# AjayAlluri/realtime-fraud-detection

Measured on AMD Instinct MI355X. Metric: scored transactions/sec (whole node), higher is better.
Workload: dtype f32 (features f64, forests f32/f64, blend f64)

## Files before the change

include/fdengine.h:

```cpp
#ifndef FDENGINE_H
#define FDENGINE_H

#include <stddef.h>
#include <stdint.h>

#ifdef __cplusplus
extern "C" {
#endif

#define FD_ABI_VERSION 15

enum fd_status {
  FD_OK = 0,
  FD_ERR_INVALID_ARG = 1,
  FD_ERR_HIP = 2,
  FD_ERR_NOT_LOADED = 3,
  FD_ERR_UNSUPPORTED = 4,
  FD_ERR_OOM = 5,
  FD_ERR_IO = 6,
};

enum fd_forest_kind {
  FD_FOREST_XGB_BINARY_LOGISTIC = 1,
  FD_FOREST_SKLEARN_IFOREST = 2,
  FD_FOREST_SKLEARN_PROBA = 3,
};

typedef struct fd_engine fd_engine;

typedef struct {
  int32_t n_trees;
  const int64_t* tree_offsets;
  const int32_t* left;
  const int32_t* right;
  const int32_t* feature;
  const double* threshold;
  const uint8_t* default_left;
  const double* leaf_value;
} fd_tree_arrays;

typedef struct {
  int32_t kind;
  int32_t num_feature;
  double base_score;
  double if_offset;
  double if_denominator;
} fd_forest_params;

#define FD_MAX_MODELS 8
enum fd_blend_strategy { FD_BLEND_WEIGHTED_AVERAGE = 0, FD_BLEND_VOTING = 1, FD_BLEND_STACKING = 2 };
enum fd_decision { FD_APPROVE = 0, FD_REVIEW = 1, FD_DECLINE = 2, FD_APPROVE_WITH_MONITORING = 3 };
enum fd_risk { FD_VERY_LOW = 0, FD_LOW = 1, FD_MEDIUM = 2, FD_HIGH = 3, FD_CRITICAL = 4 };
typedef struct {
  int32_t n_models;
  int32_t strategy;
  double weight[FD_MAX_MODELS];
  double conf_mult[FD_MAX_MODELS];
  double fraud_threshold;
  double confidence_threshold;
} fd_blend_params;

const char* fd_last_error(void);
int fd_abi_version(void);
const char* fd_build_id(void);
int fd_device_count(int* out);
int fd_engine_create(int device, fd_engine** out);
int fd_engine_destroy(fd_engine* eng);
int fd_engine_set_stream(fd_engine* eng, void* hip_stream);
int fd_engine_reset_stream(fd_engine* eng);
int fd_engine_sync(fd_engine* eng);

int fd_load_forest(fd_engine* eng, int slot, const fd_forest_params* params, const fd_tree_arrays* trees);
int fd_unload_forest(fd_engine* eng, int slot);

int fd_load_xgboost_json(fd_engine* eng, int slot, const char* path);

int fd_xgboost_json_read(const char* path, fd_forest_params* params, int32_t* n_trees, int64_t* n_nodes,
                         fd_tree_arrays* trees);
int fd_forest_info(fd_engine* eng, int slot, int32_t* n_trees, int32_t* depth, int32_t* num_feature);

int fd_forest_predict_device(fd_engine* eng, int slot, const float* d_X, int64_t n, int32_t ld,
                             double* d_prob, double* d_raw, int32_t* d_leaf);
int fd_forest_predict_host(fd_engine* eng, int slot, const float* X, int64_t n, int32_t ld,
                           double* prob, double* raw, int32_t* leaf);

typedef struct {
  int32_t n_trees;
  int32_t n_chunks;
  int32_t chunk;
  int32_t depth;
  int64_t tree_bytes;
  int64_t chunk_stride;
  int64_t blob_bytes;
  int64_t n_leaf_ids;
  float base_margin;
  int32_t layout;
  int64_t n_thresholds;
  int32_t bin_steps;
} fd_pack_info;
int fd_pack_forest_host(const fd_forest_params* params, const fd_tree_arrays* trees, void* blob,
                        int64_t blob_cap, int32_t* leaf_ids, int64_t ids_cap, fd_pack_info* info);
int fd_pack_forest_binned_host(const fd_forest_params* params, const fd_tree_arrays* trees, void* blob,
                               int64_t blob_cap, float* thresholds, int64_t thr_cap, int32_t* offsets,
                               fd_pack_info* info);

int fd_contract_forest_host(const fd_forest_params* params, const fd_tree_arrays* trees, int64_t* n_nodes,
                            fd_tree_arrays* out, int32_t* depths, int64_t* n_pruned);

typedef struct {
  int32_t kind;
  int32_t n_trees;
  int32_t depth;
  int32_t leaf_bytes;
  int64_t n_nodes;
  int64_t n_leaves;
  float base_margin;
  int32_t pad;
} fd_sparse_info;
int fd_pack_forest_sparse_host(const fd_forest_params* params, const fd_tree_arrays* trees, void* nodes,
                               int64_t nodes_cap, void* leaf_values, int64_t values_cap, int32_t* leaf_ids,
                               int64_t ids_cap, fd_sparse_info* info);

int fd_blend_device(fd_engine* eng, const fd_blend_params* params, int64_t n,
                    const double* const* d_probs, const uint8_t* present,
                    double* d_fraud_prob, double* d_confidence, uint8_t* d_decision, uint8_t* d_risk);
int fd_blend_host(fd_engine* eng, const fd_blend_params* params, int64_t n,
                  const double* const* probs, const uint8_t* present,
                  double* fraud_prob, double* confidence, uint8_t* decision, uint8_t* risk);

enum fd_window_mode {
  FD_WINDOW_REDIS_COMPAT = 0,
  FD_WINDOW_SLIDING = 1
};
#define FD_RAW_FEATURES 16
#define FD_VECTOR_WIDTH 64
#define FD_MAX_SEQ_LEN 16
typedef struct {
  int64_t capacity;
  int32_t window_mode;
  int32_t ring_k;
  int32_t seq_len;
} fd_state_params;
int fd_state_init(fd_engine* eng, const fd_state_params* params);
int fd_state_clear(fd_engine* eng);
int fd_state_info(fd_engine* eng, int64_t* capacity, int64_t* cards);
typedef struct {
  int64_t n;
  const uint64_t* key;
  const double* avg_amount;
  const int32_t* account_age_days;
  const uint64_t* device_fp;
} fd_users;
int fd_state_load_users_host(fd_engine* eng, const fd_users* users);
typedef struct {
  int64_t n;
  const double* fraud_rate;
  const double* risk_multiplier;
} fd_merchants;
int fd_load_merchants_host(fd_engine* eng, const fd_merchants* merchants);
typedef struct {
  const uint64_t* card_key;
  const int64_t* ts_ms;
  const int64_t* amount_cents;
  const int32_t* merchant;
  const uint64_t* device_fp;
  const uint8_t* ip_class;
  const uint8_t* hour;
  const uint8_t* weekend;
} fd_txn_batch;
int fd_features_device(fd_engine* eng, const fd_txn_batch* txns, int64_t n, float* d_vectors, double* d_raw);
int fd_features_host(fd_engine* eng, const fd_txn_batch* txns, int64_t n, float* vectors, double* raw);

#define FD_FEATURE_MAP_WIDTH 64
#define FD_CODE_UNKNOWN 254
typedef struct {
  const double* geo_lat;
  const double* geo_lon;
  const double* merchant_lat;
  const double* merchant_lon;
  const uint8_t* payment_method;
  const uint8_t* transaction_type;
  const uint8_t* card_type;
  const uint8_t* user_agent_flag;
  const double* fraud_score;
} fd_txn_context;
typedef struct {
  double tp_score;
  double fe_score;
  uint8_t tp_decision;
  uint8_t tp_risk;
  uint8_t fe_decision;
  uint8_t fe_risk;
  uint8_t pad[4];
} fd_rule_scores;
typedef struct {
  int64_t n;
  const uint64_t* key;
  const double* risk_score;
  const uint8_t* kyc_status;
  const uint8_t* verified;
  const int8_t* pref_start;
  const int8_t* pref_end;
  const double* weekend_activity;
  const double* online_preference;
  const double* intl_preference;
  const int32_t* txn_frequency;
  const uint8_t* has_patterns;
} fd_users_ext;
typedef struct {
  int64_t n;
  const double* avg_amount;
  const uint8_t* risk_level;
  const uint8_t* blacklisted;
  const uint8_t* category;
  const uint8_t* high_risk_category;
  const uint8_t* open_hour;
  const uint8_t* close_hour;
  const uint8_t* suspicious_name;
} fd_merchants_ext;
int fd_state_load_users_ext_host(fd_engine* eng, const fd_users_ext* users);
int fd_load_merchants_ext_host(fd_engine* eng, const fd_merchants_ext* merchants);
int fd_load_vocab_host(fd_engine* eng, const uint8_t* payment_high_risk, const uint8_t* type_is_refund);
int fd_features_full_device(fd_engine* eng, const fd_txn_batch* txns, const fd_txn_context* ctx, int64_t n,
                            float* d_vectors, double* d_raw, double* d_fmap, fd_rule_scores* d_rules);

typedef struct {
  int32_t input_size;
  int32_t hidden;
  int32_t n_out;
  const float* w_ih;
  const float* w_hh;
  const float* b_ih;
  const float* b_hh;
  const float* w_out;
  const float* b_out;
} fd_lstm_params;
int fd_load_lstm(fd_engine* eng, const fd_lstm_params* params);
int fd_unload_lstm(fd_engine* eng);
int fd_lstm_predict_device(fd_engine* eng, const float* d_seq, int64_t n, int32_t T, double* d_prob);
int fd_lstm_predict_host(fd_engine* eng, const float* seq, int64_t n, int32_t T, double* prob);
#define FD_SLOT_LSTM 64
int fd_features_seq_device(fd_engine* eng, const fd_txn_batch* txns, int64_t n, float* d_vectors, double* d_raw,
                           float* d_seq);

typedef struct {
  int32_t n_layers;
  int32_t dims[9];
  const float* weight[8];
  const float* bias[8];
} fd_mlp_params;
int fd_load_mlp(fd_engine* eng, const fd_mlp_params* params);
int fd_unload_mlp(fd_engine* eng);
int fd_mlp_info(fd_engine* eng, int32_t* n_layers, int32_t* in_dim, int32_t* hidden);
int fd_mlp_predict_device(fd_engine* eng, const float* d_X, int64_t n, int32_t ld, double* d_prob);
int fd_mlp_predict_host(fd_engine* eng, const float* X, int64_t n, int32_t ld, double* prob);
int fd_pack_mlp_host(const fd_mlp_params* params, void* blob, int64_t cap, int64_t* bytes);
#define FD_SLOT_MLP 65

#define FD_GRAPH_FEATURES 5
typedef struct {
// ... 249 lines not shown
```

realtime-fraud-detection_amd/csrc/engine.hip:

```cpp
#include <algorithm>
#include <chrono>
#include <mutex>
#include <cstring>
#include <string>

#include "blend_row.h"
#include "abtest_row.h"
#include "fd_internal.h"
#include "graph_row.h"
#include "host_stage.h"
#include "ingest_parse.h"
#include "text_row.h"

namespace fd {

static thread_local std::string g_last_error;

void set_error(const std::string& msg) { g_last_error = msg; }

Engine::Timed* Engine::next_event_pair(int kind) {
  if (timing_every > 1 && kind >= 0 && kind < 16 && (timing_seq[kind]++ % (unsigned)timing_every) != 0)
    return nullptr;
  if (events_used == events.size()) {
    hipEvent_t a, b;
// ... 367 lines not shown
    for (auto* b : {&f.split.bins, &f.split.nan, &f.split.leaves}) b->release();
    f.blob.release();
    f.leaf_ids.release();
    f.b_blob.release();
    f.b_thr.release();
    f.b_thr_off.release();
  }
  e.stage.release();
  e.scratch_probs.release();
  e.feat_vec.release();
  fd::windows_release(e);
  fd::sink_release(e);
  fd::graph_release(e);
  fd::text_release(e);
  fd::ab_release(e);
  for (auto* b : {&e.route_blk, &e.route_blk_stream, &e.route_out, &e.route_err, &e.seq_buf, &e.seq_desc, &e.lstm.wpk, &e.lstm.wpk4, &e.lstm.bias,
                  &e.lstm.wout, &e.lstm.bout, &e.state.seq, &e.mlp.blob})
    b->release();
  if (e.aux_stream) {
    (void)hipStreamSynchronize(e.aux_stream);
    (void)hipStreamDestroy(e.aux_stream);
    (void)hipEventDestroy(e.fork_ev);
    (void)hipEventDestroy(e.join_ev);
  }
  if (e.aux2_stream) {
    (void)hipStreamSynchronize(e.aux2_stream);
    (void)hipStreamDestroy(e.aux2_stream);
    (void)hipEventDestroy(e.join2_ev);
  }
  try {
    fd::comm_destroy(e);
  } catch (...) {
  }
  for (hipStream_t st : e.pipe_stream)
    if (st) {
      (void)hipStreamSynchronize(st);
      (void)hipStreamDestroy(st);
    }
  if (e.pipe_slot_stream) {
    (void)hipStreamSynchronize(e.pipe_slot_stream);
    (void)hipStreamDestroy(e.pipe_slot_stream);
  }
  if (e.pipe_entry_ev) (void)hipEventDestroy(e.pipe_entry_ev);
  for (int k = 0; k < Engine::kPipeSlots; ++k) {
    if (e.pipe_slot_ev[k]) (void)hipEventDestroy(e.pipe_slot_ev[k]);
    if (e.pipe_feat_ev[k]) (void)hipEventDestroy(e.pipe_feat_ev[k]);
    if (e.pipe_copy_ev[k]) (void)hipEventDestroy(e.pipe_copy_ev[k]);
    e.pipe_vec[k].release();
    e.pipe_out[k].release();
    e.pipe_seq[k].release();
  }
  for (int k = 0; k < Engine::kSplitRing; ++k) {
    if (e.pipe_done_ev[k]) (void)hipEventDestroy(e.pipe_done_ev[k]);
    e.pipe_split[k].release();
  }
  for (auto* b : {&e.state.uext, &e.state.mext, &e.state.vocab, &e.feat_ext}) b->release();
  for (auto& P1 : e.ens1)
    for (auto* b : {&P1.nodes[0], &P1.nodes[1], &P1.thr}) b->release();
  for (auto* b : {&e.ens.nodes[0], &e.ens.nodes[1], &e.ens.thr})
    b->release();
  {
    fd::IngestTables& t = e.ingest;
    for (auto* b : {&t.mkeys, &t.mvals}) b->release();
    for (int w = 0; w < 3; ++w) {
      t.vkeys[w].release();
      t.vvals[w].release();
    }
  }
  for (auto* b : {&e.state.pages, &e.state.keys, &e.state.merchants, &e.state.err, &e.state.sat,
                  &e.state.bucket_scr})
    b->release();
  for (auto& g : e.state.gs)
    for (auto* b : {&g.slot, &g.bucket_fill, &g.pairs, &g.ovf_cnt, &g.ovf_key, &g.ovf_b, &g.prep}) b->release();
  for (auto& ev : e.events) {
    (void)hipEventDestroy(ev.a);
    (void)hipEventDestroy(ev.b);
    if (ev.c) (void)hipEventDestroy(ev.c);
    if (ev.d) (void)hipEventDestroy(ev.d);
  }
  if (e.own_stream) (void)hipStreamDestroy(e.own_stream);
  delete eng;
  FD_API_END
}

static void rebind_stream(Engine& e, hipStream_t s) {
  for (int k = 0; k < Engine::kDoneRing; ++k)
    if (e.pipe_done_live[k] && s != e.stream) FD_HIP(hipStreamWaitEvent(s, e.pipe_done_ev[k], 0));
  e.stream = s;
}

int fd_engine_set_stream(fd_engine* eng, void* hip_stream) {
  FD_API_BEGIN
  FD_ENGINE_LOCK(eng);
  Engine& e = E(eng);
  rebind_stream(e, static_cast<hipStream_t>(hip_stream));
  FD_API_END
}

int fd_engine_reset_stream(fd_engine* eng) {
  FD_API_BEGIN
  FD_ENGINE_LOCK(eng);
  Engine& e = E(eng);
  rebind_stream(e, e.own_stream);
  FD_API_END
}

int fd_engine_sync(fd_engine* eng) {
  FD_API_BEGIN
  FD_ENGINE_LOCK(eng);
  Engine& e = E(eng);
  if (e.comm.aborted) {
    bool ok = fd::comm_sync_stream(e, e.comm.x_fwd);
    ok = fd::comm_sync_stream(e, e.stream) && ok;
    for (hipStream_t st : e.pipe_stream) ok = fd::comm_sync_stream(e, st) && ok;
    for (hipStream_t st : {e.pipe_slot_stream, e.aux_stream, e.aux2_stream}) ok = fd::comm_sync_stream(e, st) && ok;
    FD_REQUIRE(ok, FD_ERR_HIP, "streams still busy " + std::to_string(e.comm.timeout_ms) +
                                   " ms after the communicators were aborted (" + e.comm.abort_reason + ")");
  }
  FD_HIP(hipStreamSynchronize(e.stream));
  if (e.comm.x_fwd) FD_HIP(hipStreamSynchronize(e.comm.x_fwd));
  for (hipStream_t st : e.pipe_stream)
    if (st) FD_HIP(hipStreamSynchronize(st));
  if (e.pipe_slot_stream) FD_HIP(hipStreamSynchronize(e.pipe_slot_stream));
  if (e.aux_stream) FD_HIP(hipStreamSynchronize(e.aux_stream));
  if (e.aux2_stream) FD_HIP(hipStreamSynchronize(e.aux2_stream));
  fd::route_check(e);
  FD_API_END
}

int fd_engine_set_timing(fd_engine* eng, int enable) {
  FD_API_BEGIN
  FD_ENGINE_LOCK(eng);
  Engine& e = E_quiet(eng);
  e.timing = enable != 0;
  FD_API_END
}

int fd_engine_get_counter(fd_engine* eng, const char* key, int64_t* value) {
  FD_API_BEGIN
  FD_ENGINE_LOCK(eng);
  Engine& e = E_quiet(eng);
  FD_REQUIRE(key && value, FD_ERR_INVALID_ARG, "null key/value");
  const std::string k(key);
  if (k == "pipelined_batches") {
    *value = (int64_t)e.pipe_iter_total;
  } else if (k == "ensemble_single_launches") {
    *value = (int64_t)e.ens_single_total;
  } else if (k == "ensemble_contracted_launches") {
    *value = (int64_t)e.ens_contract_total;
  } else if (k == "ensemble_nodes_pruned") {
    *value = e.ens.valid ? (int64_t)e.ens.nodes_pruned : 0;
  } else if (k == "ensemble_node_steps_per_txn") {
    *value = (int64_t)e.ens_steps_last;
  } else if (k == "forest_sparse_launches") {
    *value = (int64_t)e.sparse_total;
  } else if (k == "mlp_launches") {
    *value = (int64_t)e.mlp_total;
  } else if (k == "graph_steps") {
    *value = (int64_t)e.graph.steps;
  } else if (k == "text_calls") {
    *value = (int64_t)e.text.calls;
  } else if (k == "text_nonascii_rows") {
    *value = fd::text_nonascii_rows(e);
  } else if (k == "latency_prebinned_batches") {
    *value = (int64_t)e.prebin_total;
  } else if (k == "pipelined_split_batches") {
    *value = (int64_t)e.pipe_split_total;
  } else if (k == "pipelined_compact_batches") {
    *value = (int64_t)e.pipe_compact_total;
  } else if (k == "pipelined_host_ns") {
    *value = (int64_t)e.pipe_host_ns;
  } else if (k == "pipelined_slot_stream_batches") {
    *value = (int64_t)e.pipe_slot_stream_total;
  } else if (k == "window_saturated") {
    FD_REQUIRE(e.state.ready, FD_ERR_NOT_LOADED, "card state not initialised (fd_state_init)");
    FD_HIP(hipStreamSynchronize(e.stream));
    for (hipStream_t st : e.pipe_stream)
      if (st) FD_HIP(hipStreamSynchronize(st));
    unsigned long long v = 0;
    FD_HIP(hipMemcpy(&v, e.state.sat.ptr, 8, hipMemcpyDeviceToHost));
    *value = (int64_t)v;
  } else if (k == "sharded_steps") {
    *value = (int64_t)e.comm.steps.load();
  } else if (k == "rccl_ops") {
    *value = (int64_t)e.comm.ops.load();
  } else if (k.rfind("sharded_host_ns_", 0) == 0) {
    int i = 0;
    while (i < fd::ShardComm::kHostPhases && k.compare(16, std::string::npos, fd::kShardHostPhase[i]) != 0) ++i;
    FD_REQUIRE(i < fd::ShardComm::kHostPhases, FD_ERR_INVALID_ARG, "unknown counter: " + k);
    *value = (int64_t)e.comm.host_ns[i].load();
  } else {
    FD_REQUIRE(false, FD_ERR_INVALID_ARG, "unknown counter: " + k);
  }
  FD_API_END
}

int fd_engine_set_option(fd_engine* eng, const char* key, int64_t value) {
  FD_API_BEGIN
  FD_ENGINE_LOCK(eng);
  Engine& e = E_quiet(eng);
  FD_REQUIRE(key, FD_ERR_INVALID_ARG, "null key");
  const std::string k(key);
  if (k == "forest_kernel") {
    FD_REQUIRE(value == 0 || value == 1 || value == 2 || value == 3 || value == 6 || value == 8 || value == 11,
               FD_ERR_INVALID_ARG, "forest_kernel must be 0, 1, 2, 3, 6, 8 or 11");
    e.forest_variant = (int)value;
  } else if (k == "ensemble") {
    FD_REQUIRE(value == 0 || value == 1, FD_ERR_INVALID_ARG, "ensemble must be 0 or 1");
    e.ensemble_on = value != 0;
  } else if (k == "ensemble_owner") {
    FD_REQUIRE(value == 0 || value == 1, FD_ERR_INVALID_ARG, "ensemble_owner must be 0 or 1");
    e.ens_owner_fixed = value != 0;
  } else if (k == "ensemble_prio") {
    FD_REQUIRE(value == 0 || value == 1, FD_ERR_INVALID_ARG, "ensemble_prio must be 0 or 1");
    e.ens_prio = value != 0;
  } else if (k == "ensemble_chunks") {
    FD_REQUIRE(value >= 0 && value <= 2, FD_ERR_INVALID_ARG, "ensemble_chunks must be 0, 1 or 2");
    e.ens_chunks = (int)value;
  } else if (k == "ensemble_contract") {
    FD_REQUIRE(value >= 0 && value <= 2, FD_ERR_INVALID_ARG, "ensemble_contract must be 0, 1 or 2");
    if ((int)value != e.ens_contract) {
      e.activate();
      FD_HIP(hipDeviceSynchronize());
    }
    e.ens_contract = (int)value;
  } else if (k == "compact_vectors") {
    FD_REQUIRE(value >= 0 && value <= 2, FD_ERR_INVALID_ARG, "compact_vectors must be 0, 1 or 2");
    e.compact_vectors = (int)value;
  } else if (k == "latency_fused") {
    FD_REQUIRE(value == 0 || value == 1, FD_ERR_INVALID_ARG, "latency_fused must be 0 or 1");
    e.latency_fused = value != 0;
  } else if (k == "pipeline_lean") {
    FD_REQUIRE(value == 0 || value == 1, FD_ERR_INVALID_ARG, "pipeline_lean must be 0 or 1");
    e.pipe_lean = value != 0;
  } else if (k == "pipeline_gather") {
    FD_REQUIRE(value == 0 || value == 1, FD_ERR_INVALID_ARG, "pipeline_gather must be 0 or 1");
    e.pipe_gather = value != 0;
  } else if (k == "latency_prebin") {
    FD_REQUIRE(value >= 0 && value <= 3, FD_ERR_INVALID_ARG, "latency_prebin must be 0, 1, 2 or 3");
    e.latency_prebin = value != 0;
    if (value) e.latency_prebin_mode = (int)value;
  } else if (k == "small_streams") {
    FD_REQUIRE(value >= 0 && value <= 2, FD_ERR_INVALID_ARG, "small_streams must be 0, 1 or 2");
    e.small_streams = (int)value;
  } else if (k == "count_exchange") {
    FD_REQUIRE(value >= -1 && value <= 1, FD_ERR_INVALID_ARG, "count_exchange must be -1, 0 or 1");
    FD_REQUIRE(!e.comm.pending, FD_ERR_INVALID_ARG, "count_exchange: a prefetched batch's counts are in flight");
    e.comm.count_mode = (int)value;
    e.comm.count_gather = value == 1 || (value < 0 && e.comm.world >= 4);
  } else if (k == "comm_timeout_ms") {
    FD_REQUIRE(value >= 1, FD_ERR_INVALID_ARG, "comm_timeout_ms must be >= 1");
    e.comm.timeout_ms = value;
  } else if (k == "stream_priority") {
    FD_REQUIRE(value >= 0 && value <= 3, FD_ERR_INVALID_ARG, "stream_priority must be in 0..3");
    FD_REQUIRE(!e.pipe_stream[0] && !e.comm.x_fwd, FD_ERR_INVALID_ARG,
               "stream_priority: set before the first pipelined call and fd_comm_init");
    e.stream_prio = (int)value;
  } else if (k == "bucket_keys") {
    FD_REQUIRE(value == 0 || (value >= 8 && value <= 512 && (value & (value - 1)) == 0), FD_ERR_INVALID_ARG,
               "bucket_keys must be 0 or a power of two in 8..512");
    e.state.bucket_keys = (int)value;
  } else if (k == "ensemble_bin_global") {
    FD_REQUIRE(value == 0 || value == 1, FD_ERR_INVALID_ARG, "ensemble_bin_global must be 0 or 1");
    e.ens_bin_global = value != 0;
  } else if (k == "lean_group") {
    FD_REQUIRE(value >= 0 && value <= 2, FD_ERR_INVALID_ARG, "lean_group must be 0, 1 or 2");
    e.state.lean_group = (int)value;
  } else if (k == "slot_gather") {
    FD_REQUIRE(value == 0 || value == 1, FD_ERR_INVALID_ARG, "slot_gather must be 0 or 1");
    e.state.slot_gather = value != 0;
  } else if (k == "slot_stream") {
    FD_REQUIRE(value >= -1 && value <= 2, FD_ERR_INVALID_ARG, "slot_stream must be -1, 0, 1 or 2");
    FD_REQUIRE(!e.pipe_slot_stream || (int)value == e.pipe_slot_mode, FD_ERR_INVALID_ARG,
               "slot_stream: set before the first pipelined call");
    e.pipe_slot_mode = (int)value;
  } else if (k == "slot_prio") {
    FD_REQUIRE(value == 0 || value == 1, FD_ERR_INVALID_ARG, "slot_prio must be 0 or 1");
    e.state.slot_prio = value != 0;
  } else if (k == "feature_prio") {
    FD_REQUIRE(value == 0 || value == 1, FD_ERR_INVALID_ARG, "feature_prio must be 0 or 1");
    e.state.feat_prio = value != 0;
  } else if (k == "bucket_spread") {
    FD_REQUIRE(value == 0 || value == 1, FD_ERR_INVALID_ARG, "bucket_spread must be 0 or 1");
    e.state.bucket_spread = value != 0;
  } else if (k == "timing_every") {
    FD_REQUIRE(value >= 1 && value <= 1000000, FD_ERR_INVALID_ARG, "timing_every must be >= 1");
    e.timing_every = (int)value;
    for (auto& q : e.timing_seq) q = 0;
  } else if (k == "seq_ring_lstm") {
    FD_REQUIRE(value == 0 || value == 1, FD_ERR_INVALID_ARG, "seq_ring_lstm must be 0 or 1");
    e.seq_ring_lstm = value != 0;
  } else if (k == "lstm_rows") {
    FD_REQUIRE(value == 0 || value == 4 || value == 16, FD_ERR_INVALID_ARG, "lstm_rows must be 0, 4 or 16");
    e.lstm_rows = (int)value;
  } else if (k == "mlp_form") {
    FD_REQUIRE(value == 0 || value == 1, FD_ERR_INVALID_ARG, "mlp_form must be 0 or 1");
    e.mlp_form = (int)value;
  } else if (k == "mlp_wgs_per_cu") {
    FD_REQUIRE(value >= 0 && value <= 8, FD_ERR_INVALID_ARG, "mlp_wgs_per_cu must be in 0..8");
    e.mlp_wgs_per_cu = (int)value;
  } else if (k == "ingest_stop_after") {
    FD_REQUIRE(value >= 0 && value <= 3, FD_ERR_INVALID_ARG, "ingest_stop_after must be in 0..3");
    e.ingest.stop_after = (int)value;
  } else if (k == "rule_fraud_threshold_permille") {
    FD_REQUIRE(value >= 0 && value <= 1000, FD_ERR_INVALID_ARG, "rule_fraud_threshold_permille must be in 0..1000");
    e.state.tp_threshold = (double)value / 1000.0;
  } else {
    throw fd::Error(FD_ERR_INVALID_ARG, "unknown option: " + k);
  }
  FD_API_END
}

int fd_timing_read(fd_engine* eng, int kind, double* total_ms, int64_t* launches) {
  FD_API_BEGIN
  FD_ENGINE_LOCK(eng);
  Engine& e = E_quiet(eng);
  double tot = 0.0;
  int64_t cnt = 0;
  for (size_t i = 0; i < e.events_used; ++i) {
    if (kind >= 0 && e.events[i].kind != kind) continue;
    FD_HIP(hipEventSynchronize(e.events[i].b));
    float ms = 0.f;
    FD_HIP(hipEventElapsedTime(&ms, e.events[i].a, e.events[i].b));
    tot += ms;
    if (e.events[i].split) {
      FD_HIP(hipEventSynchronize(e.events[i].d));
      FD_HIP(hipEventElapsedTime(&ms, e.events[i].c, e.events[i].d));
      tot += ms;
    }
    ++cnt;
  }
  if (total_ms) *total_ms = tot;
  if (launches) *launches = cnt;
  FD_API_END
}

int fd_timing_reset(fd_engine* eng) {
  FD_API_BEGIN
  FD_ENGINE_LOCK(eng);
  Engine& e = E_quiet(eng);
  for (size_t i = 0; i < e.events_used; ++i) {
    FD_HIP(hipEventSynchronize(e.events[i].b));
    if (e.events[i].split) FD_HIP(hipEventSynchronize(e.events[i].d));
  }
  e.events_used = 0;
  FD_API_END
}

int fd_load_forest(fd_engine* eng, int slot, const fd_forest_params* params, const fd_tree_arrays* trees) {
  FD_API_BEGIN
  FD_ENGINE_LOCK(eng);
  Engine& e = E(eng);
  FD_REQUIRE(params && trees, FD_ERR_INVALID_ARG, "null params/trees");
  fd::PackedForest& pf = slot_of(e, slot);
  FD_HIP(hipStreamSynchronize(e.stream));
  pf.loaded = false;
  fd::repack_forest(pf, *params, *trees);
  FD_API_END
}

int fd_pack_forest_host(const fd_forest_params* params, const fd_tree_arrays* trees, void* blob,
                        int64_t blob_cap, int32_t* leaf_ids, int64_t ids_cap, fd_pack_info* info) {
  FD_API_BEGIN
  FD_REQUIRE(params && trees && info, FD_ERR_INVALID_ARG, "null params/trees/info");
  const fd::HostPack hp = fd::pack_forest_host(*params, *trees);
  info->n_trees = hp.n_trees;
  info->n_chunks = hp.n_chunks;
  info->chunk = hp.chunk;
  info->depth = hp.depth;
  info->tree_bytes = (int64_t)hp.tree_bytes;
  info->chunk_stride = (int64_t)hp.chunk_stride;
  info->blob_bytes = (int64_t)hp.blob.size();
  info->n_leaf_ids = (int64_t)hp.leaf_ids.size();
  info->base_margin = hp.base_margin;
  info->layout = 0;
  info->n_thresholds = (int64_t)hp.b_thr.size();
  info->bin_steps = hp.bin_steps;
  if (blob) {
    FD_REQUIRE(blob_cap >= (int64_t)hp.blob.size(), FD_ERR_INVALID_ARG, "blob buffer too small");
    std::memcpy(blob, hp.blob.data(), hp.blob.size());
  }
  if (leaf_ids) {
    FD_REQUIRE(ids_cap >= (int64_t)hp.leaf_ids.size(), FD_ERR_INVALID_ARG, "leaf id buffer too small");
    std::memcpy(leaf_ids, hp.leaf_ids.data(), hp.leaf_ids.size() * sizeof(int32_t));
  }
  FD_API_END
}

int fd_contract_forest_host(const fd_forest_params* params, const fd_tree_arrays* trees, int64_t* n_nodes,
                            fd_tree_arrays* out, int32_t* depths, int64_t* n_pruned) {
  FD_API_BEGIN
  FD_REQUIRE(params && trees, FD_ERR_INVALID_ARG, "null params/trees");
  const fd::ContractedForest c = fd::contract_forest_host(*params, *trees);
  const int32_t T = (int32_t)c.off.size() - 1;
  const int64_t M = (int64_t)c.left.size();
  if (n_nodes) *n_nodes = M;
  if (n_pruned) *n_pruned = (int64_t)c.pruned;
  if (depths) std::memcpy(depths, c.depth.data(), (size_t)T * 4);
  if (out) {
    FD_REQUIRE(out->tree_offsets && out->left && out->right && out->feature && out->threshold && out->default_left &&
                   out->leaf_value,
               FD_ERR_INVALID_ARG, "incomplete output arrays");
    out->n_trees = T;
    std::memcpy(const_cast<int64_t*>(out->tree_offsets), c.off.data(), (size_t)(T + 1) * 8);
    std::memcpy(const_cast<int32_t*>(out->left), c.left.data(), (size_t)M * 4);
    std::memcpy(const_cast<int32_t*>(out->right), c.right.data(), (size_t)M * 4);
    std::memcpy(const_cast<int32_t*>(out->feature), c.feature.data(), (size_t)M * 4);
    std::memcpy(const_cast<double*>(out->threshold), c.threshold.data(), (size_t)M * 8);
    std::memcpy(const_cast<uint8_t*>(out->default_left), c.dleft.data(), (size_t)M);
    std::memcpy(const_cast<double*>(out->leaf_value), c.leaf.data(), (size_t)M * 8);
  }
  FD_API_END
}

int fd_pack_forest_binned_host(const fd_forest_params* params, const fd_tree_arrays* trees, void* blob,
                               int64_t blob_cap, float* thresholds, int64_t thr_cap, int32_t* offsets,
                               fd_pack_info* info) {
  FD_API_BEGIN
  FD_REQUIRE(params && trees && info, FD_ERR_INVALID_ARG, "null params/trees/info");
  const fd::HostPack hp = fd::pack_forest_host(*params, *trees);
  FD_REQUIRE(hp.binned, FD_ERR_UNSUPPORTED,
             "forest has no binned layout (depth > 8 or > 65534 distinct thresholds in a feature)");
  info->n_trees = hp.n_trees;
  info->n_chunks = hp.b_n_chunks;
  info->chunk = hp.b_chunk;
  info->depth = hp.depth;
  info->tree_bytes = (int64_t)hp.b_tree_bytes;
  info->chunk_stride = (int64_t)hp.b_chunk_stride;
  info->blob_bytes = (int64_t)hp.b_blob.size();
  info->n_leaf_ids = (int64_t)hp.leaf_ids.size();
  info->base_margin = hp.base_margin;
  info->layout = 1;
  info->n_thresholds = (int64_t)hp.b_thr.size();
  info->bin_steps = hp.bin_steps;
  if (blob) {
    FD_REQUIRE(blob_cap >= (int64_t)hp.b_blob.size(), FD_ERR_INVALID_ARG, "blob buffer too small");
    std::memcpy(blob, hp.b_blob.data(), hp.b_blob.size());
  }
  if (thresholds) {
    FD_REQUIRE(thr_cap >= (int64_t)hp.b_thr.size(), FD_ERR_INVALID_ARG, "threshold buffer too small");
    std::memcpy(thresholds, hp.b_thr.data(), hp.b_thr.size() * sizeof(float));
  }
  if (offsets) std::memcpy(offsets, hp.b_thr_off.data(), hp.b_thr_off.size() * sizeof(int32_t));
  FD_API_END
}

int fd_pack_forest_sparse_host(const fd_forest_params* params, const fd_tree_arrays* trees, void* nodes,
                               int64_t nodes_cap, void* leaf_values, int64_t values_cap, int32_t* leaf_ids,
                               int64_t ids_cap, fd_sparse_info* info) {
  FD_API_BEGIN
  FD_REQUIRE(params && trees && info, FD_ERR_INVALID_ARG, "null params/trees/info");
  const fd::SparsePack sp = fd::pack_forest_sparse_host(*params, *trees);
  *info = fd_sparse_info{};
  info->kind = sp.kind;
  info->n_trees = sp.n_trees;
  info->depth = sp.depth;
  info->leaf_bytes = sp.leaf_bytes;
  info->n_nodes = sp.n_nodes;
  info->n_leaves = sp.n_leaves;
  info->base_margin = sp.base_margin;
  if (nodes) {
    FD_REQUIRE(nodes_cap >= sp.n_nodes, FD_ERR_INVALID_ARG, "node buffer too small");
    std::memcpy(nodes, sp.nodes.data(), sp.nodes.size() * sizeof(uint32_t));
  }
  if (leaf_values) {
    FD_REQUIRE(values_cap >= sp.n_leaves, FD_ERR_INVALID_ARG, "leaf value buffer too small");
    std::memcpy(leaf_values, sp.leaf_val.data(), sp.leaf_val.size());
  }
  if (leaf_ids) {
    FD_REQUIRE(ids_cap >= sp.n_leaves, FD_ERR_INVALID_ARG, "leaf id buffer too small");
    std::memcpy(leaf_ids, sp.leaf_ids.data(), sp.leaf_ids.size() * sizeof(int32_t));
  }
  FD_API_END
}

int fd_load_xgboost_json(fd_engine* eng, int slot, const char* path) {
  FD_API_BEGIN
  FD_ENGINE_LOCK(eng);
  Engine& e = E(eng);
  fd::PackedForest& pf = slot_of(e, slot);
  fd::XgbModel m;
  fd::read_xgboost_json(path, m);
  fd_forest_params p{};
  p.kind = FD_FOREST_XGB_BINARY_LOGISTIC;
  p.num_feature = m.num_feature;
  p.base_score = m.base_score;
  fd_tree_arrays t{};
  t.n_trees = (int32_t)(m.offsets.size() - 1);
  t.tree_offsets = m.offsets.data();
  t.left = m.left.data();
  t.right = m.right.data();
  t.feature = m.feature.data();
  t.threshold = m.threshold.data();
  t.default_left = m.default_left.data();
  t.leaf_value = m.leaf_value.data();
  FD_REQUIRE(t.n_trees > 0, FD_ERR_INVALID_ARG, "xgboost json: no trees");
  FD_HIP(hipStreamSynchronize(e.stream));
  pf.loaded = false;
  fd::repack_forest(pf, p, t);
  FD_API_END
}

int fd_xgboost_json_read(const char* path, fd_forest_params* params, int32_t* n_trees, int64_t* n_nodes,
                         fd_tree_arrays* trees) {
  FD_API_BEGIN
  fd::XgbModel m;
  fd::read_xgboost_json(path, m);
  const int32_t T = (int32_t)(m.offsets.size() - 1);
  const int64_t M = (int64_t)m.left.size();
  if (params) {
    *params = fd_forest_params{};
    params->kind = FD_FOREST_XGB_BINARY_LOGISTIC;
    params->num_feature = m.num_feature;
    params->base_score = m.base_score;
  }
  if (n_trees) *n_trees = T;
  if (n_nodes) *n_nodes = M;
  if (trees) {
    FD_REQUIRE(trees->tree_offsets && trees->left && trees->right && trees->feature && trees->threshold &&
                   trees->default_left && trees->leaf_value,
               FD_ERR_INVALID_ARG, "incomplete output arrays");
    trees->n_trees = T;
    std::memcpy(const_cast<int64_t*>(trees->tree_offsets), m.offsets.data(), (size_t)(T + 1) * 8);
    std::memcpy(const_cast<int32_t*>(trees->left), m.left.data(), (size_t)M * 4);
    std::memcpy(const_cast<int32_t*>(trees->right), m.right.data(), (size_t)M * 4);
    std::memcpy(const_cast<int32_t*>(trees->feature), m.feature.data(), (size_t)M * 4);
    std::memcpy(const_cast<double*>(trees->threshold), m.threshold.data(), (size_t)M * 8);
    std::memcpy(const_cast<uint8_t*>(trees->default_left), m.default_left.data(), (size_t)M);
    std::memcpy(const_cast<double*>(trees->leaf_value), m.leaf_value.data(), (size_t)M * 8);
  }
  FD_API_END
}

int fd_unload_forest(fd_engine* eng, int slot) {
  FD_API_BEGIN
  FD_ENGINE_LOCK(eng);
  Engine& e = E(eng);
  fd::PackedForest& pf = slot_of(e, slot);
  FD_HIP(hipStreamSynchronize(e.stream));
  pf.blob.release();
  pf.leaf_ids.release();
  pf.b_blob.release();
  pf.b_thr.release();
  pf.b_thr_off.release();
  for (auto* b : {&pf.split.bins, &pf.split.nan, &pf.split.leaves}) b->release();
  for (auto* b : {&pf.sp.nodes, &pf.sp.leaf_val, &pf.sp.leaf_ids}) b->release();
  pf.sp.gen = 0;
  pf.sparse_only = false;
  pf.binned = false;
  pf.loaded = false;
  pf.gen = 0;
  FD_API_END
}

int fd_forest_info(fd_engine* eng, int slot, int32_t* n_trees, int32_t* depth, int32_t* num_feature) {
  FD_API_BEGIN
  FD_ENGINE_LOCK(eng);
  Engine& e = E(eng);
  fd::PackedForest& pf = slot_of(e, slot);
  FD_REQUIRE(pf.loaded, FD_ERR_NOT_LOADED, "Model in slot " + std::to_string(slot) + " not loaded");
  if (n_trees) *n_trees = pf.n_trees;
  if (depth) *depth = pf.depth;
  if (num_feature) *num_feature = pf.num_feature;
  FD_API_END
}

int fd_forest_predict_device(fd_engine* eng, int slot, const float* d_X, int64_t n, int32_t ld,
// ... 1375 lines not shown
```

realtime-fraud-detection_amd/csrc/ensemble.hip:

```cpp
#include <algorithm>
#include <atomic>
#include <cstring>

#include "blend_row.h"
#include "walk_common.h"

namespace fd {

static std::atomic<uint64_t> g_forest_gen{0};

void forest_loaded(PackedForest& pf, const fd_forest_params& p, const fd_tree_arrays& t) {
  pf.gen = ++g_forest_gen;
  pf.params = p;
  const int64_t m = t.tree_offsets[t.n_trees];
  pf.t_off.assign(t.tree_offsets, t.tree_offsets + t.n_trees + 1);
  pf.t_left.assign(t.left, t.left + m);
  pf.t_right.assign(t.right, t.right + m);
  pf.t_feature.assign(t.feature, t.feature + m);
  pf.t_threshold.assign(t.threshold, t.threshold + m);
  pf.t_leaf.assign(t.leaf_value, t.leaf_value + m);
  if (t.default_left)
    pf.t_dleft.assign(t.default_left, t.default_left + m);
  else
    pf.t_dleft.assign((size_t)m, 0);
}

ContractedForest contract_forest_host(const fd_forest_params& p, const fd_tree_arrays& t) {
  FD_REQUIRE(p.kind == FD_FOREST_XGB_BINARY_LOGISTIC || p.kind == FD_FOREST_SKLEARN_IFOREST, FD_ERR_INVALID_ARG,
             "contraction: XGBoost binary:logistic or IsolationForest trees");
  FD_REQUIRE(p.num_feature > 0 && p.num_feature <= kMaxFeatures, FD_ERR_UNSUPPORTED, "num_feature must be in [1, 64]");
  FD_REQUIRE(forest_depth_probe(t) >= 0, FD_ERR_INVALID_ARG, "incomplete tree arrays or a tree that is not a tree");
  const bool xgb = p.kind == FD_FOREST_XGB_BINARY_LOGISTIC;
  ContractedForest c;
  c.off.push_back(0);
  struct Item {
    int32_t o, lo, ro;
    int depth;
  };
  std::vector<Item> st, keep;
  std::vector<int32_t> remap;
  for (int i = 0; i < t.n_trees; ++i) {
    const int64_t a = t.tree_offsets[i], m = t.tree_offsets[i + 1] - a;
    const int32_t *L = t.left + a, *R = t.right + a, *F = t.feature + a;
    auto resolve = [&](int32_t o) {
      while (L[o] >= 0) {
        FD_REQUIRE(F[o] >= 0 && F[o] < p.num_feature, FD_ERR_INVALID_ARG, "split feature outside [0, num_feature)");
        const int src = compact_src(F[o]);
        if (src >= 0) break;
        const float val = src == -2 ? 0.5f : 0.0f;
        const float thr = xgb ? (float)t.threshold[a + o] : sklearn_threshold_to_lt(t.threshold[a + o]);
        o = val < thr ? L[o] : R[o];
      }
      return o;
    };
    const int64_t base = (int64_t)c.left.size();
    auto emit = [&](int32_t l, int32_t r, int32_t f, double thr, uint8_t dl, double leaf) {
      c.left.push_back(l);
      c.right.push_back(r);
      c.feature.push_back(f);
      c.threshold.push_back(thr);
      c.dleft.push_back(dl);
      c.leaf.push_back(leaf);
      return (int32_t)((int64_t)c.left.size() - 1 - base);
    };
    int64_t splits_in = 0, splits_out = 0;
    for (int64_t o = 0; o < m; ++o) splits_in += L[o] >= 0 ? 1 : 0;
    int depth = 0;
    const int32_t root = resolve(0);
    if (L[root] < 0 && L[0] >= 0) {
      emit(1, 2, 0, 0.0, 0, 0.0);
      emit(-1, -1, 0, 0.0, 0, t.leaf_value[a + root]);
      emit(-1, -1, 0, 0.0, 0, t.leaf_value[a + root]);
      depth = 1;
    } else {
      st.clear();
      st.push_back({root, 0, 0});
      keep.clear();
      while (!st.empty()) {
        Item it = st.back();
        st.pop_back();
        depth = std::max(depth, it.depth);
        if (L[it.o] >= 0) {
          it.lo = resolve(L[it.o]);
          it.ro = resolve(R[it.o]);
          st.push_back({it.ro, 0, 0, it.depth + 1});
          st.push_back({it.lo, 0, 0, it.depth + 1});
        }
        keep.push_back(it);
      }
      std::sort(keep.begin() + 1, keep.end(), [](const Item& x, const Item& y) { return x.o < y.o; });
      remap.assign((size_t)m, -1);
      for (size_t k = 0; k < keep.size(); ++k) remap[(size_t)keep[k].o] = (int32_t)k;
      for (const Item& it : keep) {
        const int32_t o = it.o;
        if (L[o] < 0) {
          emit(-1, -1, F[o], t.threshold[a + o], t.default_left ? t.default_left[a + o] : 0, t.leaf_value[a + o]);
        } else {
          ++splits_out;
          emit(remap[(size_t)it.lo], remap[(size_t)it.ro], F[o], t.threshold[a + o],
               t.default_left ? t.default_left[a + o] : 0, t.leaf_value[a + o]);
        }
      }
    }
    c.pruned += splits_in - splits_out;
    c.depth.push_back(std::max(depth, 1));
    c.off.push_back((int64_t)c.left.size());
  }
  return c;
}

namespace {

constexpr int kEnsWG = 1024;
constexpr int kMaxPass = 64;

template <bool WIDE>
struct EnsCfg {
  static constexpr int CHA = WIDE ? 24 : 20;
  static constexpr int CHB = WIDE ? 16 : 12;
  static constexpr uint32_t BUF = (uint32_t)(CHA * (1024 + 256 * 4) > CHB * (1024 + 256 * 8) ? CHA * (1024 + 256 * 4)
                                                                                             : CHB * (1024 + 256 * 8));
};
inline uint32_t ens_buf(bool wide) { return wide ? EnsCfg<true>::BUF : EnsCfg<false>::BUF; }
constexpr uint32_t kEnsTile = 4u * kTile * 8u;

__host__ __device__ constexpr uint32_t ens_xs_bytes(int nf) { return (uint32_t)((nf + 1) / 2) * 1024u; }

size_t ens_lds(int nf, bool wide) {
  return (size_t)ens_xs_bytes(nf) + 2 * (size_t)ens_buf(wide) + 2 * (size_t)kEnsTile + kTile * 4 + kTile * 8 + 128 +
         1024;
}

struct EnsArgs {
  const float* X;
  int64_t n;
  int ld, nf;
  const float* thr;
  int vec4;
  int compact;
  int owner_fixed;
  int prio;
  int n_pass;
  int ldepth;
  unsigned long long pass_global;
  const char* img;
  const char* nodes[2];
  int n_chunks[2];
  int stride[2];
  float base_margin;
  int pad1;
  double if_offset, if_denom;
  int pos[2];
  int mcol[2];
  double* mp;
  double* fp;
  double* conf;
  uint8_t* dec;
  uint8_t* risk;
  const RouteRecord* rec;
  ResultRecord* res;
  int pass_f[kMaxPass + 1];
  int img_off[kMaxPass + 1];
  int thr_off[kMaxFeatures + 1];
  uint16_t cbin[kMaxFeatures];
  alignas(4) uint16_t lut[8 * 32];
  BlendConsts blend;
#ifdef FD_FOREST_PROFILE
  int prof_slot;
  int clk_slot;
#endif
};

constexpr uint32_t kLinkMask = 0x3F8u;

template <int D, int TPG, bool NAN_AWARE>
__device__ __forceinline__ void walk_ens(uint32_t buf, int t0, uint32_t lane4, uint32_t (&leaf)[TPG]) {
  uint32_t tb[TPG], node[TPG], kl[TPG], kr[TPG], xw[TPG];
#pragma unroll
  for (int j = 0; j < TPG; ++j) {
    tb[j] = buf + (uint32_t)(t0 + j) * 1024u;
    asm volatile("" : "+v"(tb[j]));
    node[j] = lds_load<uint32_t>(tb[j] + 4u);
  }
#pragma unroll
  for (int j = 0; j < TPG; ++j) {
    xw[j] = lds_load<uint16_t>((node[j] & 0xFC02u) | lane4);
    if (D > 1) {
      const u32x2 k = lds_load<u32x2>(tb[j] + 8u);
      kl[j] = k.x;
      kr[j] = k.y;
    }
  }
#pragma unroll
  for (int l = 0; l < D; ++l) {
#pragma unroll
    for (int j = 0; j < TPG; ++j) {
      bool right = xw[j] > (node[j] >> 16);
      if (NAN_AWARE) {
        if (xw[j] == 0xFFFFu) right = (node[j] & 1u) == 0u;
      }
      if (l + 1 < D) {
        uint32_t a = kl[j], b = kr[j];
        asm volatile("" : "+v"(a), "+v"(b));
        node[j] = right ? b : a;
        xw[j] = lds_load<uint16_t>((node[j] & 0xFC02u) | lane4);
        if (l + 2 < D) {
          const u32x2 k = lds_load<u32x2>((node[j] & kLinkMask) | tb[j]);
          kl[j] = k.x;
          kr[j] = k.y;
        }
      } else {
        leaf[j] = ((node[j] & kLinkMask) >> 2) + (right ? 1u : 0u);
      }
    }
  }
}

template <int D, int TPG>
__device__ __forceinline__ unsigned long long walk_pack(uint32_t cur, int gg, uint32_t lane4, bool tile_nan) {
  static_assert(TPG <= 8, "a byte per tree in a u64");
  uint32_t leaf[TPG];
  if (tile_nan)
    walk_ens<D, TPG, true>(cur, gg * TPG, lane4, leaf);
  else
    walk_ens<D, TPG, false>(cur, gg * TPG, lane4, leaf);
  uint32_t lo = 0, hi = 0;
#pragma unroll
  for (int j = 0; j < TPG; ++j) {
    if (j < 4) lo |= leaf[j] << (8 * j);
    else hi |= leaf[j] << (8 * (j - 4));
  }
  return ((unsigned long long)hi << 32) | lo;
}

template <int TPG, bool NAN_AWARE>
__device__ __forceinline__ void walk_ens_var(uint32_t buf, int t0, uint32_t lane4, const int (&d)[TPG],
                                             uint32_t (&leaf)[TPG]) {
  uint32_t tb[TPG], node[TPG], kl[TPG], kr[TPG], xw[TPG];
  int dw = 1;
#pragma unroll
  for (int j = 0; j < TPG; ++j) {
    tb[j] = buf + (uint32_t)(t0 + j) * 1024u;
    asm volatile("" : "+v"(tb[j]));
    node[j] = lds_load<uint32_t>(tb[j] + 4u);
    dw = max(dw, d[j]);
    leaf[j] = 0u;
  }
#pragma unroll
  for (int j = 0; j < TPG; ++j) {
    xw[j] = lds_load<uint16_t>((node[j] & 0xFC02u) | lane4);
    const u32x2 k = lds_load<u32x2>(tb[j] + 8u);
    kl[j] = k.x;
    kr[j] = k.y;
  }
#pragma unroll
  for (int l = 0; l < 8; ++l) {
    if (l >= dw) break;
#pragma unroll
    for (int j = 0; j < TPG; ++j) {
      bool right = xw[j] > (node[j] >> 16);
      if (NAN_AWARE) {
        if (xw[j] == 0xFFFFu) right = (node[j] & 1u) == 0u;
      }
      const uint32_t at = ((node[j] & kLinkMask) >> 2) + (right ? 1u : 0u);
      leaf[j] = (l + 1 == d[j]) ? at : leaf[j];
      node[j] = right ? kr[j] : kl[j];
    }
    if (l + 1 >= dw) break;
#pragma unroll
    for (int j = 0; j < TPG; ++j) {
      if (l + 1 < d[j]) {
        xw[j] = lds_load<uint16_t>((node[j] & 0xFC02u) | lane4);
        if (l + 2 < d[j]) {
          const u32x2 k = lds_load<u32x2>((node[j] & kLinkMask) | tb[j]);
          kl[j] = k.x;
          kr[j] = k.y;
        }
      }
    }
  }
}

template <int VD, int TPG>
__device__ __forceinline__ unsigned long long walk_pack_var(uint32_t cur, int gg, uint32_t lane4, bool tile_nan) {
  static_assert(TPG <= 8, "a byte per tree in a u64");
  uint32_t leaf[TPG];
  int d[TPG];
#pragma unroll
  for (int j = 0; j < TPG; ++j)
    d[j] = __builtin_amdgcn_readfirstlane((int)lds_load<uint32_t>(cur + (uint32_t)(gg * TPG + j) * 1024u)) & 0xFF;
  if (VD == 1) {
    if (tile_nan)
      walk_ens_var<TPG, true>(cur, gg * TPG, lane4, d, leaf);
    else
      walk_ens_var<TPG, false>(cur, gg * TPG, lane4, d, leaf);
  } else {
#define FD_WALK_DEPTH(K)                                          \
  case K:                                                         \
    if (tile_nan)                                                 \
      walk_ens<K, TPG, true>(cur, gg * TPG, lane4, leaf);         \
    else                                                          \
      walk_ens<K, TPG, false>(cur, gg * TPG, lane4, leaf);        \
    break;
    switch (d[0]) {
      FD_WALK_DEPTH(1)
      FD_WALK_DEPTH(2)
      FD_WALK_DEPTH(3)
      FD_WALK_DEPTH(4)
      FD_WALK_DEPTH(5)
      FD_WALK_DEPTH(6)
      FD_WALK_DEPTH(7)
      default:
        if (tile_nan)
          walk_ens<8, TPG, true>(cur, gg * TPG, lane4, leaf);
        else
          walk_ens<8, TPG, false>(cur, gg * TPG, lane4, leaf);
        break;
    }
#undef FD_WALK_DEPTH
  }
  uint32_t lo = 0, hi = 0;
#pragma unroll
  for (int j = 0; j < TPG; ++j) {
    if (j < 4) lo |= leaf[j] << (8 * j);
    else hi |= leaf[j] << (8 * (j - 4));
  }
  return ((unsigned long long)hi << 32) | lo;
}

template <int D, int TPG, int CH, typename LeafT>
__device__ __forceinline__ void owner_sum(uint32_t buf, uint32_t tile, uint32_t acc, int txn, const int NL = 1 << D) {
  unsigned long long w[4];
#pragma unroll
  for (int q = 0; q < 4; ++q) w[q] = lds_load<unsigned long long>(tile + (uint32_t)(q * kTile + txn) * 8u);
  LeafT v[CH];
#pragma unroll
  for (int t = 0; t < CH; ++t) {
    const uint32_t idx = (uint32_t)(w[t / TPG] >> (8 * (t % TPG))) & 0xFFu;
    v[t] = lds_load<LeafT>(buf + (uint32_t)(CH * 1024) + ((uint32_t)(t * NL) + idx) * (uint32_t)sizeof(LeafT));
  }
  LeafT s = lds_load<LeafT>(acc + (uint32_t)txn * (uint32_t)sizeof(LeafT));
#pragma unroll
  for (int t = 0; t < CH; ++t) s += v[t];
  lds_store<LeafT>(acc + (uint32_t)txn * (uint32_t)sizeof(LeafT), s);
}

__device__ __forceinline__ void stage_pieces(const char* __restrict__ src, uint32_t dst, int bytes, int nparts,
                                             int part) {
  const int lane = threadIdx.x & 63;
  const int pieces = bytes >> 10;
  for (int p = part; p < pieces; p += nparts) {
    const char* g = src + (p << 10) + lane * 16;
    const uint32_t m0 = __builtin_amdgcn_readfirstlane(dst + ((uint32_t)p << 10));
    asm volatile(
        "s_mov_b32 m0, %0\n\t"
        "s_nop 0\n\t"
        "global_load_lds_dwordx4 %1, off"
        :
        : "s"(m0), "v"(g)
        : "memory", "m0");
  }
}

__host__ __device__ __forceinline__ int thr_pad(int g) { return g + (g >> 5); }

#ifdef FD_FOREST_PROFILE
constexpr int kEprofSlots = 4;
__device__ unsigned long long g_eprof[kEprofSlots * 256 * 16 * 16];
static int g_eprof_next = 0;
constexpr int kEclkSlots = 1024;
__device__ unsigned long long g_eclk[kEclkSlots * 4 * 4];
static int g_eclk_next = 0;
#define FD_ESTAMP(var) const unsigned long long var = __builtin_amdgcn_s_memtime()
#else
#define FD_ESTAMP(var)
#endif

template <int L>
__device__ __forceinline__ void search_lockstep(const float (&vv)[L], const int (&o)[L], const int (&cnt)[L],
                                                int (&pos)[L], int steps, bool glob, uint32_t tl, int o0,
                                                const float* __restrict__ thr) {
  if (!glob) {
    for (int st = steps; st > 0; st >>= 1) {
      float t[L];
#pragma unroll
      for (int k = 0; k < L; ++k) {
        const int np = pos[k] + st;
        const int idx = np <= cnt[k] ? np - 1 : 0;
        t[k] = lds_load<float>(tl + (uint32_t)thr_pad(o[k] - o0 + idx) * 4u);
      }
#pragma unroll
      for (int k = 0; k < L; ++k) {
        const int np = pos[k] + st;
        pos[k] = (np <= cnt[k] && t[k] <= vv[k]) ? np : pos[k];
      }
    }
  } else {
    for (int st = steps; st > 0; st >>= 1) {
      float t[L];
#pragma unroll
      for (int k = 0; k < L; ++k) {
        const int np = pos[k] + st;
        t[k] = thr[o[k] + (np <= cnt[k] ? np - 1 : 0)];
      }
#pragma unroll
      for (int k = 0; k < L; ++k) {
        const int np = pos[k] + st;
        pos[k] = (np <= cnt[k] && t[k] <= vv[k]) ? np : pos[k];
      }
    }
  }
}

template <int Q>
__device__ __forceinline__ void bin_compact_constants(const EnsArgs& a, uint16_t* Xs, int txn) {
  uint32_t* X32 = reinterpret_cast<uint32_t*>(Xs);
#pragma unroll
  for (int j = Q; j < kMaxFeatures / 2; j += 4) {
    const int f = 2 * j;
    const bool c0 = compact_src(f) < 0 && f < a.nf, c1 = compact_src(f + 1) < 0 && f + 1 < a.nf;
    if (c0 && c1)
      X32[j * 256 + txn] = (uint32_t)a.cbin[f] | ((uint32_t)a.cbin[f + 1] << 16);
    else if (c0)
      Xs[j * 512 + txn * 2] = a.cbin[f];
    else if (c1)
      Xs[j * 512 + txn * 2 + 1] = a.cbin[f + 1];
  }
}

constexpr int kLutN = 32;
static_assert(kIntSlots * kLutN == 8 * 32, "EnsArgs::lut");
constexpr int kIntOf[4][6] = {{-1, 2, -1, 6, -1, -1}, {-1, 3, 5, -1, -1, -1}, {0, 4, -1, -1, -1, -1},
                              {1, -1, -1, 7, -1, -1}};
constexpr int kNSearched[4] = {4, 4, 3, 3};
constexpr int kSearched[4][4] = {{0, 2, 4, 5}, {0, 3, 4, 5}, {2, 3, 4, 0}, {1, 2, 4, 0}};
constexpr bool int_tables_agree() {
  for (int q = 0; q < 4; ++q) {
    int ns = 0;
    for (int i = 0; i < 6; ++i) {
      const int ci = q + 4 * i;
      const int want = ci < kCompactSlots ? int_slot(ci) : -1;
      if (kIntOf[q][i] != want) return false;
      if (ci < kCompactSlots && want < 0) {
        if (ns >= 4 || kSearched[q][ns] != i) return false;
        ++ns;
      }
    }
    if (ns != kNSearched[q]) return false;
  }
  return true;
}
static_assert(int_tables_agree(), "kIntOf / kSearched must follow kIntCompact and kCompactSlot");

template <int Q>
__device__ __forceinline__ void load_compact(const float* __restrict__ xr, float (&v)[16]) {
  const unsigned long long ib = *reinterpret_cast<const unsigned long long*>(xr + 14);
#pragma unroll
  for (int i = 0; i < 6; ++i) {
    const int ci = Q + 4 * i;
    if (ci >= kCompactSlots) {
      v[i] = 0.f;
    } else if (int_slot(ci) >= 0) {
      v[i] = (float)(unsigned)((ib >> (8 * int_slot(ci))) & 0xFFull);
    } else {
      v[i] = xr[compact_word(ci)];
    }
  }
}

template <int Q>
__device__ __forceinline__ void load_split(const uint4* __restrict__ ra, const uint4* __restrict__ rb,
                                           float (&v)[16]) {
  const uint4 a0 = ra[0], a1 = ra[1], b0 = rb[0], b1 = rb[1];
  const unsigned fa = a1.w >> 24;
  const int na = (fa & 1u) ? 1 : 0;
  const int nu = ((b1.z >> 8) & 1u) ? 1 : 0;
  const int nc = ((b1.y >> 8) & 0xFFu) ? 1 : 0;
  const int n2 = na + nu + nc;
  auto byte = [](unsigned w, int k) { return (float)((w >> (8 * k)) & 0xFFu); };
#pragma unroll
  for (int i = 0; i < 6; ++i) {
    const int ci = Q + 4 * i;
    float x = 0.f;
    switch (ci) {
      case 0: x = __uint_as_float(a0.x); break;
      case 1: x = __uint_as_float(a0.y); break;
      case 2: x = byte(a1.w, 0); break;
      case 3: x = byte(a1.w, 1); break;
      case 4: x = byte(a1.w, 2); break;
      case 5: x = byte(b1.y, 0); break;
      case 6: x = byte(b1.y, 1); break;
      case 7: x = __uint_as_float(b0.x); break;
      case 8: x = __uint_as_float(b0.y); break;
      case 9: x = byte(b1.y, 2); break;
      case 10: x = __uint_as_float(a0.w); break;
      case 11: x = __uint_as_float(a1.x); break;
      case 12: x = byte(b1.y, 3); break;
      case 13: x = __uint_as_float(a1.y); break;
      case 14: x = __uint_as_float(b0.z); break;
      case 15: x = byte(b1.z, 0); break;
      default:
        if (ci < kCompactSlots) {
          const int k = ci - 16;
          const float first = (na && k == 0) ? __uint_as_float(a0.z)
                                             : ((nu && k == na) ? __uint_as_float(b0.w) : __uint_as_float(b1.x));
          const int t = k - n2;
          x = k < n2 ? first
                     : (t == 0 ? __uint_as_float(a1.z)
                               : (t == 1 ? ((fa & 2u) ? 1.f : 0.f) : (t == 2 ? ((fa & 4u) ? 1.f : 0.f) : 0.f)));
        }
        break;
    }
    v[i] = x;
  }
}

template <int Q, int L, bool LUT>
__device__ __forceinline__ void bin_compact_pass(const EnsArgs& a, const float (&v)[16], uint16_t* Xs,
                                                 int txn, int f0, int f1, bool glob, uint32_t tl, int o0,
                                                 int& anynan, uint32_t lut) {
  constexpr int NV = (kCompactSlots - Q + 3) / 4;
  constexpr int NS = LUT ? kNSearched[Q] : NV;
#pragma unroll
  for (int i = 0; i < NV; ++i) {
    const int ks = LUT ? kIntOf[Q][i] : -1;
    if (ks < 0) continue;
    const int f = kCompactSlot[Q + 4 * i];
    if (!(f >= f0 && f < f1 && f < a.nf)) continue;
    const float x = v[i];
    uint16_t bin;
    if (x != x) {
      anynan = 1;
      bin = (uint16_t)0xFFFFu;
    } else if (x >= 0.f && x < (float)kLutN && x == truncf(x)) {
      bin = lds_load<uint16_t>(lut + (uint32_t)(ks * kLutN + (int)x) * 2u);
    } else {
      const int o = a.thr_off[f], cnt = a.thr_off[f + 1] - o;
      int pos = 0;
#pragma unroll
      for (int st = 1 << 15; st > 0; st >>= 1)
        if (pos + st <= cnt && a.thr[o + pos + st - 1] <= x) pos += st;
      bin = (uint16_t)pos;
    }
    Xs[(f >> 1) * 512 + txn * 2 + (f & 1)] = bin;
  }
#pragma unroll
  for (int g0 = 0; g0 < NS; g0 += L) {
    float vv[L];
    int o[L], cnt[L], pos[L];
    bool act[L];
    int steps = 0;
#pragma unroll
    for (int k = 0; k < L; ++k) {
      const int i = LUT ? kSearched[Q][g0 + k < NS ? g0 + k : 0] : (g0 + k < NS ? g0 + k : 0);
      const int f = kCompactSlot[Q + 4 * i];
      act[k] = g0 + k < NS && f >= f0 && f < f1 && f < a.nf;
      vv[k] = act[k] ? v[i] : 0.f;
      o[k] = act[k] ? a.thr_off[f] : o0;
      cnt[k] = act[k] ? a.thr_off[f + 1] - o[k] : 0;
      pos[k] = 0;
      steps = max(steps, lift_steps(cnt[k]));
    }
    search_lockstep<L>(vv, o, cnt, pos, steps, glob, tl, o0, a.thr);
#pragma unroll
    for (int k = 0; k < L; ++k) {
      const int i = LUT ? kSearched[Q][g0 + k < NS ? g0 + k : 0] : (g0 + k < NS ? g0 + k : 0);
      const int f = kCompactSlot[Q + 4 * i];
      if (act[k]) {
        const bool nan = vv[k] != vv[k];
        anynan |= nan ? 1 : 0;
        Xs[(f >> 1) * 512 + txn * 2 + (f & 1)] = nan ? (uint16_t)0xFFFFu : (uint16_t)pos[k];
      }
    }
  }
}

template <int D, int OUT, bool WIDE, bool LUT = true, int VD = 0>
__global__ void __launch_bounds__(kEnsWG) ensemble_kernel(EnsArgs a) {
  constexpr int kCHA = EnsCfg<WIDE>::CHA, kCHB = EnsCfg<WIDE>::CHB;
  constexpr uint32_t kEnsBuf = EnsCfg<WIDE>::BUF;
  constexpr int TPGA = kCHA / 4, TPGB = kCHB / 4;
  extern __shared__ __attribute__((aligned(16))) char smem[];
  const uint32_t sdyn = (uint32_t)(size_t)((lds_char*)smem);
  const uint32_t s0 = (sdyn + 1023u) & ~1023u;
  char* const lbase = smem + (s0 - sdyn);
  const int tid = threadIdx.x, wave = tid >> 6, lane = tid & 63;
  const int gg = __builtin_amdgcn_readfirstlane(wave >> 2);
  const int txn = ((wave & 3) << 6) + lane;
  const uint32_t lane4 = s0 + (uint32_t)txn * 4u;
  const uint32_t bufA = s0 + ens_xs_bytes(a.nf), bufB = bufA + kEnsBuf;
  const uint32_t tile0 = bufB + kEnsBuf, tile1 = tile0 + kEnsTile;
  const uint32_t accA = tile1 + kEnsTile, accB = accA + kTile * 4;
  const uint32_t flags = accB + kTile * 8, owner_cnt = flags + 64;
  const int64_t row = (int64_t)blockIdx.x * kTile + txn;
  const bool valid = row < a.n;
  const int nA = a.n_chunks[0], G = nA + a.n_chunks[1];
  const int NL = VD ? 1 << a.ldepth : 1 << D;

#ifdef FD_FOREST_PROFILE
  unsigned long long pr_top = 0, pr_walk = 0, pr_sync = 0, pr_dma = 0, pr_st[8] = {0, 0, 0, 0, 0, 0, 0, 0};
#endif
  FD_ESTAMP(pr_t0);
#ifdef FD_FOREST_PROFILE
  const unsigned long long pr_rt0 = __builtin_amdgcn_s_memrealtime();
#endif
  {
    const int k_prio = a.prio, k_compact = a.compact, k_npass = a.n_pass, k_vec4 = a.vec4, k_ld = a.ld;
    const unsigned long long k_pg = a.pass_global;
    const float* k_x = a.X;
    const char* k_img = a.img;
    const int k_i0 = a.img_off[0], k_i1 = a.img_off[1], k_f1 = a.pass_f[1];
    asm volatile("" ::"s"(k_prio), "s"(k_compact), "s"(k_npass), "s"(k_vec4), "s"(k_ld), "s"(k_pg), "s"(k_x),
                 "s"(k_img), "s"(k_i0), "s"(k_i1), "s"(k_f1), "s"(nA), "s"(G), "s"(a.n));
  }
  if (a.prio) __builtin_amdgcn_s_setprio(2);
  int anynan = 0;
  const bool early0 = G > 0 && a.n_pass == 1 && (a.pass_global & 1ull) != 0;
  {
    uint16_t* Xs = reinterpret_cast<uint16_t*>(lbase);
    const int q = __builtin_amdgcn_readfirstlane(tid >> 8);
    const int fq = q * 16;
    float v[16];
    if (valid && a.compact == 2) {
      const uint4* ra = reinterpret_cast<const uint4*>(a.X) + 2 * row;
      const uint4* rb = reinterpret_cast<const uint4*>(a.X) + 2 * (a.n + row);
      switch (q) {
        case 0: load_split<0>(ra, rb, v); bin_compact_constants<0>(a, Xs, txn); break;
        case 1: load_split<1>(ra, rb, v); bin_compact_constants<1>(a, Xs, txn); break;
        case 2: load_split<2>(ra, rb, v); bin_compact_constants<2>(a, Xs, txn); break;
        default: load_split<3>(ra, rb, v); bin_compact_constants<3>(a, Xs, txn); break;
      }
    } else if (valid && a.compact) {
      const float* xr = a.X + row * (int64_t)kCompactWidth;
      switch (q) {
        case 0: load_compact<0>(xr, v); bin_compact_constants<0>(a, Xs, txn); break;
        case 1: load_compact<1>(xr, v); bin_compact_constants<1>(a, Xs, txn); break;
        case 2: load_compact<2>(xr, v); bin_compact_constants<2>(a, Xs, txn); break;
        default: load_compact<3>(xr, v); bin_compact_constants<3>(a, Xs, txn); break;
      }
    } else if (valid) {
      const float* xr = a.X + row * (int64_t)a.ld;
      const int ncopy = a.ld < a.nf ? a.ld : a.nf;
      if (a.vec4 && fq + 16 <= ncopy) {
        const float4* x4 = reinterpret_cast<const float4*>(xr + fq);
#pragma unroll
        for (int k = 0; k < 4; ++k) {
          const float4 t = x4[k];
          v[4 * k] = t.x;
          v[4 * k + 1] = t.y;
          v[4 * k + 2] = t.z;
          v[4 * k + 3] = t.w;
        }
      } else {
#pragma unroll
        for (int k = 0; k < 16; ++k) v[k] = fq + k < ncopy ? xr[fq + k] : __builtin_nanf("");
      }
    }
    if (a.n_pass > 0 && !(a.pass_global & 1ull))
      stage_pieces(a.img + a.img_off[0], bufA, a.img_off[1] - a.img_off[0], kEnsWG / 64, wave);
    if (early0) stage_chunk_asm(nA > 0 ? a.nodes[0] : a.nodes[1], bufA, nA > 0 ? a.stride[0] : a.stride[1], kEnsWG / 64);
#ifdef FD_FOREST_PROFILE
    pr_st[0] = __builtin_amdgcn_s_memtime();
#endif
    if (LUT && a.compact && tid < kIntSlots * kLutN / 2)
      lds_store<uint32_t>(accA + (uint32_t)tid * 4u, reinterpret_cast<const uint32_t*>(a.lut)[tid]);
    constexpr int kLock = 4;
    for (int p = 0; p < a.n_pass; ++p) {
      const int f0 = a.pass_f[p], f1 = a.pass_f[p + 1];
      const bool glob = (a.pass_global >> p) & 1ull;
      const int o0 = a.thr_off[f0];
      const uint32_t tl = bufA;
      if (!glob) {
        if (p > 0)
          stage_pieces(a.img + a.img_off[p], bufA, a.img_off[p + 1] - a.img_off[p], kEnsWG / 64, wave);
        dma_wait();
        __syncthreads();
      } else if (LUT && a.compact && p == 0) {
        __syncthreads();
      }
#ifdef FD_FOREST_PROFILE
      if (p < 3) pr_st[1 + 2 * p] = __builtin_amdgcn_s_memtime();
#endif
      if (LUT && valid && a.compact) {
        switch (q) {
          case 0: bin_compact_pass<0, kLock, true>(a, v, Xs, txn, f0, f1, glob, tl, o0, anynan, accA); break;
          case 1: bin_compact_pass<1, kLock, true>(a, v, Xs, txn, f0, f1, glob, tl, o0, anynan, accA); break;
          case 2: bin_compact_pass<2, kLock, true>(a, v, Xs, txn, f0, f1, glob, tl, o0, anynan, accA); break;
          default: bin_compact_pass<3, kLock, true>(a, v, Xs, txn, f0, f1, glob, tl, o0, anynan, accA); break;
        }
      } else if (valid && a.compact) {
        switch (q) {
          case 0: bin_compact_pass<0, kLock, false>(a, v, Xs, txn, f0, f1, glob, tl, o0, anynan, accA); break;
          case 1: bin_compact_pass<1, kLock, false>(a, v, Xs, txn, f0, f1, glob, tl, o0, anynan, accA); break;
          case 2: bin_compact_pass<2, kLock, false>(a, v, Xs, txn, f0, f1, glob, tl, o0, anynan, accA); break;
          default: bin_compact_pass<3, kLock, false>(a, v, Xs, txn, f0, f1, glob, tl, o0, anynan, accA); break;
        }
      } else if (valid) {
#pragma unroll
        for (int kk = 0; kk < 16; kk += kLock) {
          const int fb = fq + kk;
          if (fb + kLock - 1 < f0 || fb >= f1) continue;
          float vv[kLock];
          int o[kLock], cnt[kLock], pos[kLock];
          bool act[kLock];
          int steps = 0;
#pragma unroll
          for (int k = 0; k < kLock; ++k) {
            const int f = fb + k;
            act[k] = f >= f0 && f < f1;
            vv[k] = act[k] ? v[kk + k] : 0.f;
            o[k] = act[k] ? a.thr_off[f] : o0;
            cnt[k] = act[k] ? a.thr_off[f + 1] - o[k] : 0;
            pos[k] = 0;
            steps = max(steps, lift_steps(cnt[k]));
          }
          if (!glob) {
            for (int st = steps; st > 0; st >>= 1) {
              float t[kLock];
#pragma unroll
              for (int k = 0; k < kLock; ++k) {
                const int np = pos[k] + st;
                const int idx = np <= cnt[k] ? np - 1 : 0;
                t[k] = lds_load<float>(tl + (uint32_t)thr_pad(o[k] - o0 + idx) * 4u);
              }
#pragma unroll
              for (int k = 0; k < kLock; ++k) {
                const int np = pos[k] + st;
                pos[k] = (np <= cnt[k] && t[k] <= vv[k]) ? np : pos[k];
              }
            }
          } else {
            for (int st = steps; st > 0; st >>= 1) {
              float t[kLock];
#pragma unroll
              for (int k = 0; k < kLock; ++k) {
                const int np = pos[k] + st;
                t[k] = a.thr[o[k] + (np <= cnt[k] ? np - 1 : 0)];
              }
#pragma unroll
              for (int k = 0; k < kLock; ++k) {
                const int np = pos[k] + st;
                pos[k] = (np <= cnt[k] && t[k] <= vv[k]) ? np : pos[k];
              }
            }
          }
#pragma unroll
          for (int k = 0; k < kLock; ++k) {
            const int f = fb + k;
            if (act[k]) {
              const bool nan = vv[k] != vv[k];
              anynan |= nan ? 1 : 0;
              Xs[(f >> 1) * 512 + txn * 2 + (f & 1)] = nan ? (uint16_t)0xFFFFu : (uint16_t)pos[k];
            }
          }
        }
      }
      __syncthreads();
#ifdef FD_FOREST_PROFILE
      if (p < 3) pr_st[2 + 2 * p] = __builtin_amdgcn_s_memtime();
#endif
    }
  }
  if (G > 0 && !early0)
    stage_pieces(nA > 0 ? a.nodes[0] : a.nodes[1], bufA, nA > 0 ? a.stride[0] : a.stride[1], kEnsWG / 64, wave);
  if (gg == 0) {
    lds_store<float>(accA + txn * 4, a.base_margin);
    lds_store<double>(accB + txn * 8, 0.0);
  }
  if (tid == 0) lds_store<uint32_t>(owner_cnt, 0u);
  dma_wait();
  const bool tile_nan = tile_any(anynan, reinterpret_cast<uint32_t*>(lbase + (flags - s0)), kEnsWG / 64);

  FD_ESTAMP(pr_t1);
  for (int g = 0; g < G; ++g) {
    FD_ESTAMP(q0);
    const bool owner = gg == (a.owner_fixed ? 0 : ((g - 1) & 3));
    if (owner) {
      if (g > 0) {
        const int c = g - 1;
        const uint32_t bp = (c & 1) ? bufB : bufA, tp = (c & 1) ? tile1 : tile0;
        if (c < nA) owner_sum<D, TPGA, kCHA, float>(bp, tp, accA, txn, NL);
        else owner_sum<D, TPGB, kCHB, double>(bp, tp, accB, txn, NL);
        if (lane == 0)
          __hip_atomic_fetch_add(reinterpret_cast<uint32_t*>(lbase + (owner_cnt - s0)), 1u, __ATOMIC_RELAXED,
                                 __HIP_MEMORY_SCOPE_WORKGROUP);
        while (__hip_atomic_load(reinterpret_cast<uint32_t*>(lbase + (owner_cnt - s0)), __ATOMIC_RELAXED,
                                 __HIP_MEMORY_SCOPE_WORKGROUP) < 4u * (uint32_t)g)
          __builtin_amdgcn_s_sleep(1);
      }
      if (g + 1 < G) {
        const int h = g + 1, fb = h >= nA ? 1 : 0;
        stage_pieces(a.nodes[fb] + (size_t)(fb ? h - nA : h) * a.stride[fb], (g & 1) ? bufA : bufB, a.stride[fb], 4,
                  wave & 3);
      }
    }
    const uint32_t cur = (g & 1) ? bufB : bufA, tw = (g & 1) ? tile1 : tile0;
    FD_ESTAMP(q1);
    unsigned long long w;
    if (VD)
      w = g < nA ? walk_pack_var<VD, TPGA>(cur, gg, lane4, tile_nan) : walk_pack_var<VD, TPGB>(cur, gg, lane4, tile_nan);
    else
      w = g < nA ? walk_pack<D, TPGA>(cur, gg, lane4, tile_nan) : walk_pack<D, TPGB>(cur, gg, lane4, tile_nan);
    lds_store<unsigned long long>(tw + (uint32_t)(gg * kTile + txn) * 8u, w);
    FD_ESTAMP(q2);
    if (owner) dma_wait();
#ifdef FD_FOREST_PROFILE
    const unsigned long long q2d = __builtin_amdgcn_s_memtime();
#endif
    __syncthreads();
#ifdef FD_FOREST_PROFILE
    const unsigned long long q3 = __builtin_amdgcn_s_memtime();
    pr_top += q1 - q0;
    pr_walk += q2 - q1;
    pr_dma += q2d - q2;
    pr_sync += q3 - q2;
#endif
  }
  if (G > 0 && gg == (a.owner_fixed ? 0 : ((G - 1) & 3))) {
    const int c = G - 1;
    const uint32_t bp = (c & 1) ? bufB : bufA, tp = (c & 1) ? tile1 : tile0;
    if (c < nA) owner_sum<D, TPGA, kCHA, float>(bp, tp, accA, txn, NL);
    else owner_sum<D, TPGB, kCHB, double>(bp, tp, accB, txn, NL);
  }
  __syncthreads();
#ifdef FD_FOREST_PROFILE
  if (lane == 0 && blockIdx.x < 256) {
    unsigned long long* o = g_eprof + (size_t)a.prof_slot * 256 * 16 * 16 + ((size_t)blockIdx.x * 16 + wave) * 16;
    for (int k = 0; k < 7; ++k) o[6 + k] = pr_st[k] ? pr_st[k] - pr_t0 : 0;
    o[0] = pr_t1 - pr_t0;
    o[1] = pr_top;
    o[2] = pr_walk;
    o[3] = pr_sync;
    o[13] = pr_dma;
    o[4] = pr_t0;
    o[5] = __builtin_amdgcn_s_memtime();
    o[14] = pr_rt0;
    o[15] = __builtin_amdgcn_s_memrealtime();
    if (wave == 0 && (blockIdx.x & 63) == 0) {
      unsigned long long* c = g_eclk + ((size_t)a.clk_slot * 4 + (blockIdx.x >> 6)) * 4;
      c[0] = pr_t0;
      c[1] = o[5];
      c[2] = pr_rt0;
      c[3] = o[15];
    }
  }
#endif
  if (gg != 0 || !valid) return;

  double pa, pb;
  {
    const float mg = lds_load<float>(accA + txn * 4);
    const float xm = fminf(-mg, 88.7f);
    const float denom = expf(xm) + 1.0f + 1e-16f;
    pa = (double)(1.0f / denom);
  }
  {
    const double d = lds_load<double>(accB + txn * 8);
    const double qd = (a.if_denom != 0.0) ? d / a.if_denom : 1.0;
    const double score = pow(2.0, -qd);
    const double decision = -score - a.if_offset;
    pb = 1.0 / (1.0 + exp(decision));
  }
  if (OUT == 2) {
    a.fp[row] = nA > 0 ? pa : pb;
    if (a.mp) a.mp[row] = nA > 0 ? (double)lds_load<float>(accA + txn * 4) : lds_load<double>(accB + txn * 8);
    return;
  }
  double raw[FD_MAX_MODELS];
#pragma unroll
  for (int m = 0; m < FD_MAX_MODELS; ++m) raw[m] = m == a.pos[0] ? pa : (m == a.pos[1] ? pb : 0.0);
  if (a.mp) {
    a.mp[(size_t)a.mcol[0] * a.n + row] = pa;
    a.mp[(size_t)a.mcol[1] * a.n + row] = pb;
  }
  double fp, conf;
  uint8_t dec, risk;
  blend_row(a.blend, raw, fp, conf, dec, risk);
  if (OUT == 0) {
    a.fp[row] = fp;
    if (a.conf) a.conf[row] = conf;
    if (a.dec) a.dec[row] = dec;
    if (a.risk) a.risk[row] = risk;
  } else {
    ResultRecord r;
    r.fraud_prob = fp;
    r.confidence = conf;
    r.seq = a.rec[row].seq;
    r.decision = dec;
    r.risk = risk;
    r.pad = 0;
    a.res[row] = r;
  }
}

template <int OUT, bool WIDE>
const void* pick_ensemble(int D) {
  switch (D) {
    case 1: return (const void*)ensemble_kernel<1, OUT, WIDE>;
    case 2: return (const void*)ensemble_kernel<2, OUT, WIDE>;
    case 3: return (const void*)ensemble_kernel<3, OUT, WIDE>;
    case 4: return (const void*)ensemble_kernel<4, OUT, WIDE>;
    case 5: return (const void*)ensemble_kernel<5, OUT, WIDE>;
    case 6: return (const void*)ensemble_kernel<6, OUT, WIDE>;
    case 7: return (const void*)ensemble_kernel<7, OUT, WIDE>;
    case 8: return (const void*)ensemble_kernel<8, OUT, WIDE>;
    default: return nullptr;
  }
}

const void* pick_ensemble(int out, bool wide, int D) {
  if (wide) return out == 1 ? pick_ensemble<1, true>(D) : out == 2 ? pick_ensemble<2, true>(D) : pick_ensemble<0, true>(D);
  return out == 1 ? pick_ensemble<1, false>(D) : out == 2 ? pick_ensemble<2, false>(D) : pick_ensemble<0, false>(D);
}

const void* pick_ensemble_var(int out, bool wide, int vd) {
  if (vd == 2) {
    if (wide) return out == 1 ? (const void*)ensemble_kernel<8, 1, true, true, 2> : (const void*)ensemble_kernel<8, 0, true, true, 2>;
    return out == 1 ? (const void*)ensemble_kernel<8, 1, false, true, 2> : (const void*)ensemble_kernel<8, 0, false, true, 2>;
  }
  if (wide) return out == 1 ? (const void*)ensemble_kernel<8, 1, true, true, 1> : (const void*)ensemble_kernel<8, 0, true, true, 1>;
  return out == 1 ? (const void*)ensemble_kernel<8, 1, false, true, 1> : (const void*)ensemble_kernel<8, 0, false, true, 1>;
}

fd_tree_arrays arrays_of(const PackedForest& f) {
  fd_tree_arrays t{};
  t.n_trees = f.n_trees;
  t.tree_offsets = f.t_off.data();
  t.left = f.t_left.data();
  t.right = f.t_right.data();
  t.feature = f.t_feature.data();
  t.threshold = f.t_threshold.data();
  t.default_left = f.t_dleft.data();
  t.leaf_value = f.t_leaf.data();
  return t;
}

void plan_passes(const std::vector<float>& thr, const std::vector<int32_t>& off, int nf, bool wide, EnsPassSet& ps,
                 std::vector<float>& img) {
  const size_t stage_floats = (2 * (size_t)ens_buf(wide) + 2 * (size_t)kEnsTile) / 4;
  ps = EnsPassSet{};
  ps.f.push_back(0);
  ps.img_off.push_back((int)(img.size() * 4));
  int f = 0;
  while (f < nf) {
    int g = f;
    while (g < nf && (size_t)(off[g + 1] - off[f]) + (size_t)(off[g + 1] - off[f]) / 32 + 1 <= stage_floats) ++g;
    const int np = (int)ps.f.size() - 1;
    FD_REQUIRE(np < kMaxPass, FD_ERR_UNSUPPORTED, "ensemble binning plan too long");
    if (g == f) {
      ps.glob |= 1ull << np;
      g = f + 1;
    } else {
      const int cnt = off[g] - off[f];
      const size_t words = cnt > 0 ? (size_t)thr_pad(cnt - 1) + 1 : 0;
      const size_t base = img.size();
      img.resize(base + (words + 255) / 256 * 256, 0.f);
      for (int i = 0; i < cnt; ++i) img[base + (size_t)thr_pad(i)] = thr[(size_t)off[f] + i];
    }
    ps.f.push_back(g);
    ps.img_off.push_back((int)(img.size() * 4));
    f = g;
  }
}

bool build_plan(Engine& e, EnsemblePlan& P, int sa, int sb, bool wide, int contract = 0) {
  P.valid = false;
  const PackedForest* F[2] = {sa >= 0 ? &e.forests[sa] : nullptr, sb >= 0 ? &e.forests[sb] : nullptr};
  if (!F[0] && !F[1]) return false;
  int D = 0, nf = -1;
  for (const PackedForest* f : F) {
    if (!f) continue;
    if (f->sparse_only || !f->binned || f->t_off.empty() || (nf >= 0 && f->num_feature != nf)) return false;
    nf = f->num_feature;
    D = std::max(D, f->depth);
  }
  if (D > 8) return false;
  if (ens_lds(nf, wide) > kLdsBudget) return false;
  HostPack hp[2];
  for (int k = 0; k < 2; ++k) {
    if (!F[k]) continue;
    hp[k] = pack_forest_host(F[k]->params, arrays_of(*F[k]), D);
    if (!hp[k].binned || hp[k].depth != D) return false;
  }
  std::vector<std::vector<float>> merged(nf);
  for (int f = 0; f < nf; ++f) {
    for (int k = 0; k < 2; ++k) {
      if (!F[k]) continue;
      const HostPack& h = hp[k];
      merged[f].insert(merged[f].end(), h.b_thr.begin() + h.b_thr_off[f], h.b_thr.begin() + h.b_thr_off[f + 1]);
    }
    std::sort(merged[f].begin(), merged[f].end());
    merged[f].erase(std::unique(merged[f].begin(), merged[f].end()), merged[f].end());
    if (merged[f].size() > (size_t)kMaxBins) return false;
  }
  std::vector<float> thr;
  std::vector<int32_t> off(nf + 1, 0);
  int maxc = 0;
  for (int f = 0; f < nf; ++f) {
    thr.insert(thr.end(), merged[f].begin(), merged[f].end());
    off[f + 1] = (int32_t)thr.size();
    maxc = std::max(maxc, (int)merged[f].size());
  }
  const int NL = 1 << D;
  const int CH[2] = {wide ? EnsCfg<true>::CHA : EnsCfg<false>::CHA, wide ? EnsCfg<true>::CHB : EnsCfg<false>::CHB};
  const size_t leaf_sz[2] = {sizeof(float), sizeof(double)};
  for (int k = 0; k < 2; ++k) {
    if (!F[k]) {
      P.n_trees[k] = P.n_chunks[k] = 0;
      P.CH[k] = CH[k];
      P.stride[k] = 0;
      continue;
    }
    const HostPack& h = hp[k];
    const int T = h.n_trees, nc = (T + CH[k] - 1) / CH[k];
    const size_t leaf_bytes = (size_t)CH[k] * NL * leaf_sz[k];
    const size_t stride = ((size_t)CH[k] * 1024 + leaf_bytes + 1023) / 1024 * 1024;
    FD_REQUIRE(stride <= ens_buf(wide), FD_ERR_UNSUPPORTED, "ensemble chunk exceeds its LDS buffer");
    std::vector<char> blob((size_t)nc * stride, 0);
    for (int i = 0; i < T; ++i) {
      const char* src = h.b_blob.data() + (size_t)(i / h.b_chunk) * h.b_chunk_stride + (size_t)(i % h.b_chunk) *
                                                                                          h.b_tree_bytes;
      char* chunk = blob.data() + (size_t)(i / CH[k]) * stride;
      uint32_t* dst = reinterpret_cast<uint32_t*>(chunk + (size_t)(i % CH[k]) * 1024);
      for (int s = 1; s < NL; ++s) {
        uint32_t w;
        std::memcpy(&w, src + (size_t)s * 4, 4);
        const uint32_t f = (w >> 10) & 63u;
        if (!h.pad[(size_t)i * NL + s]) {
          const int j = (int)(w >> 16);
          const float t = h.b_thr[h.b_thr_off[f] + j];
          const uint32_t jm = (uint32_t)(std::lower_bound(merged[f].begin(), merged[f].end(), t) - merged[f].begin());
          w = (jm << 16) | (w & 0xFFFFu);
        }
        const uint32_t link = s < (NL >> 1) ? (uint32_t)s : (uint32_t)(s - (NL >> 1));
        dst[s] = (w & 0xFFFF0001u) | ((f >> 1) << 10) | (link << 3) | ((f & 1u) << 1);
      }
      std::memcpy(chunk + (size_t)CH[k] * 1024 + (size_t)(i % CH[k]) * NL * leaf_sz[k], src + (size_t)NL * 4,
                  (size_t)NL * leaf_sz[k]);
    }
    P.nodes[k].ensure(blob.size());
    FD_HIP(hipMemcpy(P.nodes[k].ptr, blob.data(), blob.size(), hipMemcpyHostToDevice));
    P.n_trees[k] = T;
    P.CH[k] = CH[k];
    P.n_chunks[k] = nc;
    P.stride[k] = stride;
  }
  P.contract = contract;
  P.contracted = false;
  P.nodes_pruned = 0;
  P.steps_full = P.steps_c = 0;
  for (int k = 0; k < 2 && contract; ++k) {
    if (!F[k]) continue;
    const bool xgb = F[k]->params.kind == FD_FOREST_XGB_BINARY_LOGISTIC;
    const ContractedForest c = contract_forest_host(F[k]->params, arrays_of(*F[k]));
    const int T = hp[k].n_trees, nc = P.n_chunks[k], ch = CH[k], tpg = ch / 4;
    const size_t nb = (size_t)nc * ch;
    std::vector<int> dw(nb, 1);
    for (int i = 0; i < T; ++i) dw[i] = std::min(c.depth[i], D);
    if (contract == 1)
      for (size_t g0 = 0; g0 < nb; g0 += tpg) {
        const int mx = *std::max_element(dw.begin() + g0, dw.begin() + g0 + tpg);
        std::fill(dw.begin() + g0, dw.begin() + g0 + tpg, mx);
      }
    std::vector<char> blob((size_t)nc * P.stride[k], 0);
    std::vector<int32_t> cur(2 * NL);
    for (size_t i = 0; i < nb; ++i) {
      char* chunk = blob.data() + (i / ch) * P.stride[k];
      uint32_t* dst = reinterpret_cast<uint32_t*>(chunk + (i % ch) * 1024);
      dst[0] = (uint32_t)dw[i];
      const int nl = 1 << dw[i];
      if ((int)i >= T) {
        for (int s = 1; s < nl; ++s) dst[s] = (s < (nl >> 1) ? (uint32_t)s : (uint32_t)(s - (nl >> 1))) << 3;
        continue;
      }
      P.steps_c += dw[i];
      const int64_t a = c.off[i];
      cur[1] = 0;
      for (int s = 1; s < nl; ++s) {
        const int32_t o = cur[s];
        const uint32_t link = s < (nl >> 1) ? (uint32_t)s : (uint32_t)(s - (nl >> 1));
        if (c.left[a + o] < 0) {
          dst[s] = link << 3;
          cur[2 * s] = cur[2 * s + 1] = o;
          continue;
        }
        const uint32_t f = (uint32_t)c.feature[a + o];
        const float thr = xgb ? (float)c.threshold[a + o] : sklearn_threshold_to_lt(c.threshold[a + o]);
        const uint32_t jm = (uint32_t)(std::lower_bound(merged[f].begin(), merged[f].end(), thr) - merged[f].begin());
        dst[s] = (jm << 16) | ((f >> 1) << 10) | (link << 3) | ((f & 1u) << 1) | (c.dleft[a + o] ? 1u : 0u);
        cur[2 * s] = c.left[a + o];
        cur[2 * s + 1] = c.right[a + o];
      }
      char* leaves = chunk + (size_t)ch * 1024 + (i % ch) * NL * leaf_sz[k];
      for (int s = 0; s < nl; ++s) {
        const double v = c.leaf[a + cur[nl + s]];
        if (k == 0) {
          const float vf = (float)v;
          std::memcpy(leaves + (size_t)s * 4, &vf, 4);
        } else {
          std::memcpy(leaves + (size_t)s * 8, &v, 8);
        }
      }
    }
    P.nodes_c[k].ensure(blob.size());
    FD_HIP(hipMemcpy(P.nodes_c[k].ptr, blob.data(), blob.size(), hipMemcpyHostToDevice));
    P.nodes_pruned += c.pruned;
  }
  for (int k = 0; k < 2; ++k) P.steps_full += F[k] ? (long long)hp[k].n_trees * D : 0;
  P.contracted = contract != 0 && P.steps_c < P.steps_full;
  P.thr.ensure(std::max<size_t>(4, thr.size() * sizeof(float)));
  if (!thr.empty()) FD_HIP(hipMemcpy(P.thr.ptr, thr.data(), thr.size() * sizeof(float), hipMemcpyHostToDevice));
  P.h_thr_off = off;
  P.h_cbin.assign(kMaxFeatures, 0);
  for (int f = 0; f < nf && f < kMaxFeatures; ++f) {
    const int src = compact_src(f);
    if (src >= 0) continue;
    const float val = src == -2 ? 0.5f : 0.0f;
    P.h_cbin[f] = (uint16_t)(std::upper_bound(merged[f].begin(), merged[f].end(), val) - merged[f].begin());
  }
  {
    std::vector<uint16_t> lut((size_t)kIntSlots * kLutN, 0);
    for (int k = 0; k < kIntSlots; ++k) {
      const int f = kCompactSlot[kIntCompact[k]];
      if (f >= nf) continue;
      for (int x = 0; x < kLutN; ++x)
        lut[(size_t)k * kLutN + x] =
            (uint16_t)(std::upper_bound(merged[f].begin(), merged[f].end(), (float)x) - merged[f].begin());
    }
    P.h_lut = lut;
  }
  {
    std::vector<float> img;
    plan_passes(thr, off, nf, wide, P.passes, img);
    P.img.ensure(std::max<size_t>(1024, img.size() * sizeof(float)));
    if (!img.empty()) FD_HIP(hipMemcpy(P.img.ptr, img.data(), img.size() * sizeof(float), hipMemcpyHostToDevice));
  }
  P.max_feature_thr = maxc;
  P.slot[0] = sa;
  P.slot[1] = sb;
  P.gen[0] = F[0] ? F[0]->gen : 0;
  P.gen[1] = F[1] ? F[1]->gen : 0;
  P.n_forests = (F[0] ? 1 : 0) + (F[1] ? 1 : 0);
  P.D = D;
  P.nf = nf;
  P.wide = wide;
  P.kind[0] = FD_FOREST_XGB_BINARY_LOGISTIC;
  P.kind[1] = FD_FOREST_SKLEARN_IFOREST;
  P.base_margin = F[0] ? hp[0].base_margin : 0.f;
  P.if_offset = F[1] ? F[1]->if_offset : 0.0;
  P.if_denominator = F[1] ? F[1]->if_denominator : 0.0;
  P.valid = true;
  return true;
}

bool plan_current(const Engine& e, const EnsemblePlan& P, int sa, int sb, bool wide, int contract = 0) {
  return P.valid && P.wide == wide && P.contract == contract && P.slot[0] == sa && P.slot[1] == sb &&
         P.gen[0] == (sa >= 0 ? e.forests[sa].gen : 0) && P.gen[1] == (sb >= 0 ? e.forests[sb].gen : 0);
}

bool want_wide(const Engine& e) { return e.ens_chunks == 1 || (e.ens_chunks == 0 && !e.comm.ready); }

}

#ifdef FD_FOREST_PROFILE
extern "C" __attribute__((visibility("default"))) int fd_debug_ens_profile(unsigned long long* out, int n) {
  return (int)hipMemcpyFromSymbol(out, HIP_SYMBOL(g_eprof), sizeof(unsigned long long) * (size_t)n);
}
extern "C" __attribute__((visibility("default"))) int fd_debug_ens_profile_next(void) { return g_eprof_next; }
extern "C" __attribute__((visibility("default"))) int fd_debug_ens_clock(unsigned long long* out, int n) {
  return (int)hipMemcpyFromSymbol(out, HIP_SYMBOL(g_eclk), sizeof(unsigned long long) * (size_t)n);
}
extern "C" __attribute__((visibility("default"))) int fd_debug_ens_clock_next(void) { return g_eclk_next; }
#endif

namespace {
struct Pair {
  int sa = -1, sb = -1, pa = -1, pb = -1, ma = -1, mb = -1;
};

bool select_pair(Engine& e, const fd_blend_params& p, const int32_t* slots, const uint8_t* present, int64_t n,
                 Pair& q) {
  if (!e.ensemble_on || e.forest_variant != 0 || n <= 0) return false;
  if ((n + kTile - 1) / kTile < kSplitTiles) return false;
  int k = 0;
  for (int m = 0; m < p.n_models; ++m) {
    if (present && !present[m]) continue;
    const int s = slots[m];
    if (s < 0 || s >= kMaxSlots || !e.forests[s].loaded || e.forests[s].sparse_only) return false;
    const int kind = e.forests[s].kind;
    if (kind == FD_FOREST_XGB_BINARY_LOGISTIC && q.sa < 0) {
      q.sa = s;
      q.pa = k;
      q.ma = m;
    } else if (kind == FD_FOREST_SKLEARN_IFOREST && q.sb < 0) {
      q.sb = s;
      q.pb = k;
      q.mb = m;
    } else {
      return false;
    }
    ++k;
  }
  if (q.sa < 0 || q.sb < 0) return false;
  const bool wide = want_wide(e);
  if (!plan_current(e, e.ens, q.sa, q.sb, wide, e.ens_contract) &&
      !build_plan(e, e.ens, q.sa, q.sb, wide, e.ens_contract))
    return false;
  return true;
}
}

namespace {
void plan_args(const EnsemblePlan& P, const float* dX, int64_t n, int32_t ld, bool owner_fixed, EnsArgs& a) {
  a.X = dX;
  a.n = n;
  a.ld = ld;
  a.nf = P.nf;
  a.thr = P.thr.as<const float>();
  FD_REQUIRE(P.nf <= kMaxFeatures, FD_ERR_UNSUPPORTED, "ensemble: more than 64 features");
  for (int f = 0; f <= P.nf; ++f) a.thr_off[f] = P.h_thr_off[f];
  a.owner_fixed = owner_fixed ? 1 : 0;
  for (int f = 0; f < kMaxFeatures; ++f) a.cbin[f] = f < (int)P.h_cbin.size() ? P.h_cbin[f] : 0;
  for (size_t k = 0; k < P.h_lut.size() && k < sizeof(a.lut) / sizeof(a.lut[0]); ++k) a.lut[k] = P.h_lut[k];
  a.vec4 = (ld % 4 == 0 && (reinterpret_cast<uintptr_t>(dX) & 15u) == 0) ? 1 : 0;
  const EnsPassSet& ps = P.passes;
  a.n_pass = (int)ps.f.size() - 1;
  for (int p = 0; p <= a.n_pass; ++p) {
    a.pass_f[p] = ps.f[p];
    a.img_off[p] = ps.img_off[p];
  }
  a.pass_global = ps.glob;
  a.img = P.img.as<const char>();
  for (int q = 0; q < 2; ++q) {
    a.nodes[q] = P.nodes[q].as<const char>();
    a.n_chunks[q] = P.n_chunks[q];
    a.stride[q] = (int)P.stride[q];
  }
  a.base_margin = P.base_margin;
  a.if_offset = P.if_offset;
  a.if_denom = P.if_denominator;
}

bool run_plan(Engine& e, const EnsemblePlan& P, EnsArgs& a, int out, int timing_kind, int vd = 0) {
  const void* fn = vd && out != 2 ? pick_ensemble_var(out, P.wide, vd) : pick_ensemble(out, P.wide, P.D);
  if (!fn) return false;
  const size_t lds = ens_lds(P.nf, P.wide);
  FD_HIP(hipFuncSetAttribute(fn, hipFuncAttributeMaxDynamicSharedMemorySize, (int)lds));
  const int64_t blocks = (a.n + kTile - 1) / kTile;
  Engine::Timed* ev = e.timing ? e.next_event_pair(timing_kind) : nullptr;
  if (ev) FD_HIP(hipEventRecord(ev->a, e.stream));
#ifdef FD_FOREST_PROFILE
  a.prof_slot = g_eprof_next;
  g_eprof_next = (g_eprof_next + 1) % kEprofSlots;
  a.clk_slot = g_eclk_next;
  g_eclk_next = (g_eclk_next + 1) % kEclkSlots;
#endif
  void* args[] = {&a};
  FD_HIP(hipLaunchKernel(fn, dim3((unsigned)blocks), dim3(kEnsWG), args, lds, e.stream));
  if (ev) FD_HIP(hipEventRecord(ev->b, e.stream));
  return true;
}
}

bool ensemble_applies(Engine& e, const fd_blend_params& p, const int32_t* slots, const uint8_t* present, int64_t n) {
  Pair q;
  return select_pair(e, p, slots, present, n, q);
}

bool launch_ensemble(Engine& e, const fd_blend_params& p, const int32_t* slots, const uint8_t* present,
                     const float* dX, int64_t n, int32_t ld, double* dMP, double* dfp, double* dconf, uint8_t* ddec,
                     uint8_t* drisk, const RouteRecord* records, ResultRecord* results, int compact) {
  Pair q;
  if (!select_pair(e, p, slots, present, n, q)) return false;
  const int pa = q.pa, pb = q.pb, ma = q.ma, mb = q.mb;
  EnsArgs a{};
  plan_args(e.ens, dX, n, compact ? kCompactWidth : ld, e.ens_owner_fixed, a);
  a.compact = compact;
  if (compact && e.ens_bin_global) {
    a.n_pass = 1;
    a.pass_f[0] = 0;
    a.pass_f[1] = e.ens.nf;
    a.pass_global = 1ull;
  }
  a.prio = e.ens_prio ? 1 : 0;
  a.pos[0] = pa;
  a.pos[1] = pb;
  a.mcol[0] = ma;
  a.mcol[1] = mb;
  a.blend = blend_consts(p, present);
  a.mp = dMP;
  a.fp = dfp;
  a.conf = dconf;
  a.dec = ddec;
  a.risk = drisk;
  a.rec = records;
  a.res = results;
  const int out = results ? 1 : 0;
  FD_REQUIRE(out == 1 || dfp != nullptr, FD_ERR_INVALID_ARG, "null output");
  const int vd = (compact && e.ens.contracted) ? (e.ens.contract == 1 ? 2 : 1) : 0;
  if (vd) {
    for (int k = 0; k < 2; ++k) a.nodes[k] = e.ens.nodes_c[k].as<const char>();
    a.ldepth = e.ens.D;
  }
  if (!run_plan(e, e.ens, a, out, FD_TIMING_ENSEMBLE, vd)) return false;
  if (vd) ++e.ens_contract_total;
  e.ens_steps_last = vd ? e.ens.steps_c : e.ens.steps_full;
  return true;
}

bool launch_ensemble_single(Engine& e, int slot, const float* dX, int64_t n, int32_t ld, double* dprob,
                            double* draw, hipStream_t stream) {
  if (!e.ensemble_on || e.forest_variant != 0 || n <= 0) return false;
  if ((n + kTile - 1) / kTile < kSplitTiles) return false;
  if (slot < 0 || slot >= kMaxSlots || !e.forests[slot].loaded || e.forests[slot].sparse_only) return false;
  const bool xgb = e.forests[slot].kind == FD_FOREST_XGB_BINARY_LOGISTIC;
  const int sa = xgb ? slot : -1, sb = xgb ? -1 : slot;
  EnsemblePlan& P = e.ens1[slot];
  const bool wide = want_wide(e);
  if (!plan_current(e, P, sa, sb, wide) && !build_plan(e, P, sa, sb, wide)) return false;
  EnsArgs a{};
  plan_args(P, dX, n, ld, e.ens_owner_fixed, a);
  a.prio = e.ens_prio ? 1 : 0;
  a.fp = dprob;
  a.mp = draw;
  const hipStream_t saved = e.stream;
  if (stream) e.stream = stream;
  bool ok = false;
  try {
    ok = run_plan(e, P, a, 2, xgb ? FD_TIMING_XGB : FD_TIMING_IFOREST);
  } catch (...) {
    e.stream = saved;
    throw;
  }
  e.stream = saved;
  if (ok) ++e.ens_single_total;
  return ok;
}


}
```

realtime-fraud-detection_amd/csrc/fd_internal.h:

```cpp
#pragma once

#include <hip/hip_runtime.h>

#include <atomic>
#include <chrono>
#include <condition_variable>
#include <cstddef>
#include <cstdint>
#include <mutex>
#include <stdexcept>
#include <string>
#include <thread>
#include <vector>

#include "fdengine.h"
#include "key_hash.h"

namespace fd {

constexpr int kMaxSlots = 8;
constexpr int kTile = 256;
constexpr int kGatherBatchMax = 4096;
constexpr int kMaxFeatures = 64;
constexpr int kCompactWidth = 16;
// ... 24 lines not shown
constexpr int64_t kSparseMaxNodes = 1ll << 24;
constexpr size_t kLdsBudget = 160 * 1024;
constexpr int kMaxBins = 65534;
constexpr int kSplitTiles = 128;
constexpr int kSeqInput = 16;
constexpr unsigned long long kSeqMaterialized = 1ull << 63;
constexpr int kLstmHidden = 128;

#ifdef FD_FOREST_PROFILE
constexpr int kTlKernels = 8;
#define FD_TL_BUF(name) __device__ unsigned long long name[fd::kTlKernels * 1024 * 4]
#define FD_TL(buf, kid, k)                                                                            \
  do {                                                                                                \
    const unsigned tl_b = blockIdx.x + blockIdx.y * gridDim.x;                                        \
    if (threadIdx.x == 0 && tl_b < 1024u) buf[((kid) * 1024 + tl_b) * 4 + (k)] = __builtin_amdgcn_s_memrealtime(); \
  } while (0)
#else
#define FD_TL(buf, kid, k) \
  do {                     \
  } while (0)
#endif

struct Error : std::runtime_error {
  int code;
  Error(int c, const std::string& m) : std::runtime_error(m), code(c) {}
};

void set_error(const std::string& msg);

#define FD_HIP(call)                                                                       \
  do {                                                                                     \
    hipError_t _e = (call);                                                                \
    if (_e != hipSuccess)                                                                  \
      throw ::fd::Error(FD_ERR_HIP, std::string(#call) + ": " + hipGetErrorString(_e));    \
  } while (0)

#define FD_REQUIRE(cond, code, msg)              \
  do {                                           \
    if (!(cond)) throw ::fd::Error((code), (msg)); \
  } while (0)


struct DeviceBuffer {
  void* ptr = nullptr;
  size_t bytes = 0;
  void ensure(size_t need) {
    if (need <= bytes) return;
    release();
    FD_HIP(hipMalloc(&ptr, need));
    bytes = need;
  }
  void ensure_headroom(size_t need) {
    if (need > bytes) ensure(need + need / 4);
  }
  void release() {
    if (ptr) (void)hipFree(ptr);
    ptr = nullptr;
    bytes = 0;
  }
  template <class T>
  T* as() const { return static_cast<T*>(ptr); }
};

struct SplitScratch {
  DeviceBuffer bins, nan, leaves;
};

struct PreBin {
  const float* thr[2] = {};
  const int32_t* thr_off[2] = {};
  uint32_t* bins[2] = {};
  uint32_t* nan[2] = {};
  int nf[2] = {};
  int64_t n = 0, n_pad = 0;
  int ld = 0;
  int steps[2] = {};
  bool thr_nonempty = false;
  const void* fx = nullptr;
  const void* ff = nullptr;
  const float* X = nullptr;
  bool want = false, done = false;
};

struct SparseImage {
  DeviceBuffer nodes, leaf_val, leaf_ids;
  int64_t n_nodes = 0, n_leaves = 0;
  uint64_t gen = 0;
};

struct PackedForest {
  bool loaded = false;
  bool sparse_only = false;
  mutable SparseImage sp;
  int kind = 0;
  int n_trees = 0;
  int n_chunks = 0;
  int chunk = 0;
  int depth = 0;
  int num_feature = 0;
  size_t tree_bytes = 0;
  size_t chunk_stride = 0;
  float base_margin = 0.f;
  double if_offset = 0.0;
  double if_denominator = 0.0;
  DeviceBuffer blob;
  DeviceBuffer leaf_ids;
  bool binned = false;
  int b_chunk = 0, b_n_chunks = 0, bin_steps = 0;
  size_t b_tree_bytes = 0, b_chunk_stride = 0;
  DeviceBuffer b_blob;
  DeviceBuffer b_thr;
  DeviceBuffer b_thr_off;
  int b_n_thr = 0;
  int n_chunk = 0, n_n_chunks = 0;
  size_t n_chunk_stride = 0;
  DeviceBuffer n_blob;
  DeviceBuffer n_leaves;
  mutable SplitScratch split;
  uint64_t gen = 0;
  fd_forest_params params{};
  std::vector<int64_t> t_off;
  std::vector<int32_t> t_left, t_right, t_feature;
  std::vector<double> t_threshold, t_leaf;
  std::vector<uint8_t> t_dleft;
};

struct EnsPassSet {
  std::vector<int> f, img_off;
  unsigned long long glob = 0;
};

struct EnsemblePlan {
  bool valid = false;
  bool wide = true;
  int slot[2] = {-1, -1};
  uint64_t gen[2] = {0, 0};
  int n_forests = 0, D = 0, nf = 0;
  int kind[2] = {0, 0}, n_trees[2] = {0, 0}, CH[2] = {0, 0}, n_chunks[2] = {0, 0};
  size_t stride[2] = {0, 0};
  float base_margin = 0.f;
  double if_offset = 0.0, if_denominator = 0.0;
  DeviceBuffer nodes[2], thr;
  std::vector<int32_t> h_thr_off;
  std::vector<uint16_t> h_cbin;
  std::vector<uint16_t> h_lut;
  DeviceBuffer img;
  EnsPassSet passes;
  int max_feature_thr = 0;
  DeviceBuffer nodes_c[2];
  int contract = 0;
  bool contracted = false;
  long long nodes_pruned = 0;
  long long steps_full = 0, steps_c = 0;
};

struct ContractedForest {
  std::vector<int64_t> off;
  std::vector<int32_t> left, right, feature, depth;
  std::vector<double> threshold, leaf;
  std::vector<uint8_t> dleft;
  long long pruned = 0;
  fd_tree_arrays arrays() const {
    fd_tree_arrays t{};
    t.n_trees = (int32_t)off.size() - 1;
    t.tree_offsets = off.data();
    t.left = left.data();
    t.right = right.data();
    t.feature = feature.data();
    t.threshold = threshold.data();
    t.default_left = dleft.data();
    t.leaf_value = leaf.data();
    return t;
  }
};
ContractedForest contract_forest_host(const fd_forest_params& p, const fd_tree_arrays& t);

struct __attribute__((aligned(16))) RouteRecord {
  unsigned long long key;
  long long ts;
  long long cents;
  unsigned long long dfp;
  int merchant;
  unsigned seq;
  unsigned char ipc, hour, wk;
  unsigned char pm;
  unsigned flags;
};
struct __attribute__((aligned(8))) ResultRecord {
  double fraud_prob;
  double confidence;
  unsigned seq;
  unsigned char decision, risk;
  unsigned short pad;
};

struct LstmModel {
  bool loaded = false;
  int input_size = 0, n_out = 0;
  DeviceBuffer wpk, wpk4, bias, wout, bout;
  bool hh_finite = false;
};

constexpr int kGraphChunk = 16384;
struct GraphState {
  bool ready = false;
  int H = 0;
  int cap = 0;
  int cur = 0;
  int64_t total = 0;
  int64_t base = 0;
  DeviceBuffer log[2];
  DeviceBuffer dm;
  unsigned long long steps = 0;
};

constexpr int kTextChunk = 65536;
struct TextState {
  DeviceBuffer acc;
  DeviceBuffer count;
  unsigned long long calls = 0;
};

struct AbTest {
  bool live = false;
  uint64_t salt = 0;
  double threshold = 0.0;
};
struct AbState {
  AbTest tests[FD_AB_MAX_TESTS];
  DeviceBuffer state;
  DeviceBuffer partials;
  DeviceBuffer part;
  DeviceBuffer index;
  DeviceBuffer rows;
};
struct AbScatter {
  const int32_t* idx;
  int64_t n;
  int64_t count[2];
  int models[2];
  int m_max;
  const double *p_fp, *p_conf;
  const uint8_t *p_dec, *p_risk;
  const double* p_mp[2];
  double *fp, *conf;
  uint8_t *dec, *risk;
  double* mp;
};

struct MlpModel {
  bool loaded = false;
  bool hot = false;
  int n_layers = 0;
  int dims[9] = {};
  int words = 0;
  int cus = 0, occ_ref = 1, occ_lds = 1;
  DeviceBuffer blob;
};

struct __attribute__((aligned(128))) CardHeader {
  long long last_ts;
  unsigned char ring_n, ring_head;
  unsigned char unsorted;
  unsigned char pad0;
  unsigned char wc[3], pad1;
  unsigned flags;
  int rc_cnt;
  long long ws[3];
  unsigned wod[3];
  unsigned pad2;
  unsigned long long key;
  double avg;
  int age;
  int pad3;
  unsigned long long fp[3];
  long long pad4[2];
};
static_assert(sizeof(CardHeader) == 128, "CardHeader must be one 128-B line");
static_assert(offsetof(CardHeader, key) == 64 && offsetof(CardHeader, wod) + sizeof(unsigned) * 3 <= 64,
              "the mutable fields in bytes 0-63, the key at 64 (snapshot.hip reads it there)");
constexpr int kCardHeaderBytes = (int)sizeof(CardHeader);

struct __attribute__((aligned(16))) RingEvent {
  long long ts;
  long long cents;
};

struct CardPages {
  char* base;
  long long stride;
  __host__ __device__ __forceinline__ CardHeader* hdr(long long s) const {
    return reinterpret_cast<CardHeader*>(base + s * stride);
  }
  __host__ __device__ __forceinline__ RingEvent* ring(long long s) const {
    return reinterpret_cast<RingEvent*>(base + s * stride + kCardHeaderBytes);
  }
};

#ifdef __HIP_DEVICE_COMPILE__
#define FD_CARD_SLOT_QUAL __device__ __forceinline__
#else
#define FD_CARD_SLOT_QUAL __device__ inline
#endif
FD_CARD_SLOT_QUAL long long card_slot(unsigned long long* keys, CardPages pg, long long mask, unsigned long long key) {
  if (key == 0ull) key = 1ull;
  long long h = (long long)(fmix64(key) & (unsigned long long)mask);
  if (mask >= 7) {
    long long g = h & ~7ll;
    int j0 = (int)(h & 7);
    for (long long p = 0; p <= mask + 8; p += 8) {
      const uint4* q = reinterpret_cast<const uint4*>(keys + g);
      uint4 w[4];
#pragma unroll
      for (int u = 0; u < 4; ++u) w[u] = q[u];
#pragma unroll
      for (int j = 0; j < 8; ++j) {
        if (j < j0) continue;
        const uint4 v = w[j >> 1];
        const unsigned long long k = (j & 1) ? (((unsigned long long)v.w << 32) | v.z)
                                             : (((unsigned long long)v.y << 32) | v.x);
        if (k == key) return g + j;
        if (k == 0ull) {
          const unsigned long long old = atomicCAS(&keys[g + j], 0ull, key);
          if (old == 0ull) {
            pg.hdr(g + j)->key = key;
            return g + j;
          }
          if (old == key) return g + j;
// ... 51 lines not shown
struct WindowState {
  bool ready = false;
  int64_t cap = 0, cand_cap = 0;
  int64_t ooo = 10000;
  int64_t wm = INT64_MIN;
  int64_t min_seen = INT64_MAX;
  int64_t max_seen = INT64_MIN;
  bool observed = false;
  DeviceBuffer ulog[2], mlog[2];
  int ucur = 0, mcur = 0;
  int64_t ucount = 0, mcount = 0;
  DeviceBuffer keys, vals, sort_tmp, uout, mout, scalars;
};

struct SinkState {
  bool ready = false;
  unsigned long long cap = 0, ucap = 0;
  DeviceBuffer table, users, err;
};

struct IngestTables {
  DeviceBuffer mkeys, mvals, vkeys[3], vvals[3];
  unsigned long long mmask = 0, vmask[3] = {0, 0, 0};
  bool mloaded = false, vloaded[3] = {false, false, false};
  int stop_after = 0;
};

struct ShardComm {
  bool ready = false;
  bool aborted = false;
  std::string abort_reason;
  int rank = 0, world = 1;
  const void* api = nullptr;
  void* fwd = nullptr;
  void* back = nullptr;
  hipStream_t x_fwd = nullptr;
  DeviceBuffer rec[2], cnt[2], back_buf;
  static constexpr int kInbox = 3;
  DeviceBuffer inbox[kInbox];
  DeviceBuffer res[kInbox];
  hipEvent_t in_ev[kInbox] = {}, inbox_ev[kInbox] = {};
  bool inbox_live[kInbox] = {};
  int inbox_next = 0;
  int inbox_of[2] = {0, 0};
  DeviceBuffer route_blk;
  int64_t* h_cnt[2] = {nullptr, nullptr};
  int64_t* d_hcnt[2] = {nullptr, nullptr};
  unsigned long long cnt_seq[2] = {0, 0};
  bool pending = false;
  unsigned long long pending_id = 0;
  int64_t pending_n = 0;
  int pending_slot = 0, next_slot = 0;
  int64_t split[2][2 * FD_MAX_SHARDS] = {};
  int64_t timeout_ms = 120000;
  int count_mode = -1;
  bool count_gather = false;
  int device = 0;
  static constexpr int kHostPhases = 8;
  std::atomic<unsigned long long> steps{0}, host_ns[kHostPhases] = {};
  std::atomic<unsigned long long> ops{0};
};
inline const char* const kShardHostPhase[ShardComm::kHostPhases] = {
    "wait", "partition", "counts", "count_copy", "records", "score", "back", "scatter"};
struct HostLaps {
  ShardComm& c;
  std::chrono::steady_clock::time_point t = std::chrono::steady_clock::now();
  void operator()(int ph) {
    const auto now = std::chrono::steady_clock::now();
    c.host_ns[ph].fetch_add((unsigned long long)std::chrono::duration_cast<std::chrono::nanoseconds>(now - t).count(),
                            std::memory_order_relaxed);
    t = now;
  }
};

inline int64_t floor_div_host(int64_t a, int64_t b) {
  int64_t q = a / b;
  if ((a % b != 0) && ((a < 0) != (b < 0))) --q;
  return q;
}

struct Engine {
  int device = 0;
  hipStream_t own_stream = nullptr;
  hipStream_t stream = nullptr;
  PackedForest forests[kMaxSlots];
  CardStore state;
  LstmModel lstm;
  MlpModel mlp;
  unsigned long long mlp_total = 0;
  GraphState graph;
  TextState text;
  AbState ab;
  WindowState windows;
  IngestTables ingest;
  SinkState sink;
  hipStream_t aux_stream = nullptr;
  hipEvent_t fork_ev = nullptr, join_ev = nullptr;
  hipStream_t aux2_stream = nullptr;
  hipEvent_t join2_ev = nullptr;
  DeviceBuffer seq_buf;
  DeviceBuffer seq_desc;
  DeviceBuffer feat_vec, feat_ext;
  static constexpr int kPipeSlots = 2;
  hipStream_t pipe_stream[2] = {nullptr, nullptr};
  static constexpr int kDoneRing = 4;
  hipEvent_t pipe_entry_ev = nullptr, pipe_feat_ev[kPipeSlots] = {}, pipe_done_ev[kDoneRing] = {};
  bool pipe_feat_live[kPipeSlots] = {}, pipe_done_live[kDoneRing] = {};
  bool pipe_dirty = true;
  int pipe_slot_mode = -1;
  hipStream_t pipe_slot_stream = nullptr;
  hipEvent_t pipe_slot_ev[kPipeSlots] = {};
  hipStream_t slot_pass_stream = nullptr;
  hipEvent_t slot_pass_ev = nullptr;
  unsigned long long pipe_iter = 0;
  unsigned long long pipe_iter_total = 0;
  unsigned long long sparse_total = 0;
  unsigned long long ens_single_total = 0;
  unsigned long long pipe_split_total = 0;
  unsigned long long pipe_compact_total = 0;
  unsigned long long pipe_host_ns = 0;
  unsigned long long pipe_slot_stream_total = 0;
  bool pipe_lean = true;
  bool pipe_gather = true;
  DeviceBuffer pipe_vec[kPipeSlots], pipe_seq[kPipeSlots];
  static constexpr int kSplitRing = 4;
  static_assert(kSplitRing == kDoneRing, "the split-row ring's buffers are released by the done events");
  DeviceBuffer pipe_split[kSplitRing];
  DeviceBuffer pipe_out[kPipeSlots];
  hipEvent_t pipe_copy_ev[kPipeSlots] = {};
  bool pipe_copy_live[kPipeSlots] = {};
  bool pipe_copy_vec[kPipeSlots] = {};
  int small_streams = 0;
  bool latency_fused = true;
  bool seq_ring_lstm = true;
  bool latency_prebin = true;
  int latency_prebin_mode = 3;
  PreBin prebin;
  unsigned long long prebin_total = 0;
  bool ens_prio = true;
  bool ens_bin_global = false;
  int compact_vectors = 2;
  int stream_prio = 3;
  DeviceBuffer stage;
  DeviceBuffer scratch_probs;
  DeviceBuffer route_blk, route_out, route_err;
  DeviceBuffer route_blk_stream;
  ShardComm comm;
  EnsemblePlan ens;
  EnsemblePlan ens1[kMaxSlots];
  bool route_err_live = false;
  int forest_variant = 0;
  bool ens_owner_fixed = true;
  int ens_chunks = 0;
  int ens_contract = 1;
  unsigned long long ens_contract_total = 0;
  long long ens_steps_last = 0;
  int mlp_form = 0;
  int mlp_wgs_per_cu = 0;
  int lstm_rows = 0;
  bool ensemble_on = true;
  bool timing = false;
  int timing_every = 1;
  unsigned long long timing_seq[16] = {};
  struct Timed {
    hipEvent_t a, b;
    int kind;
    hipEvent_t c = nullptr, d = nullptr;
    bool split = false;
  };
  std::vector<Timed> events;
  size_t events_used = 0;
  void activate() const { FD_HIP(hipSetDevice(device)); }
  Timed* next_event_pair(int kind);
};

struct HostPack {
  std::vector<char> blob;
  std::vector<int32_t> leaf_ids;
  int kind = 0, n_trees = 0, n_chunks = 0, chunk = 0, depth = 0, num_feature = 0;
  size_t tree_bytes = 0, chunk_stride = 0;
  float base_margin = 0.f;
  bool binned = false;
  std::vector<char> b_blob;
  std::vector<float> b_thr;
  std::vector<int32_t> b_thr_off;
  int b_chunk = 0, b_n_chunks = 0, bin_steps = 0;
  size_t b_tree_bytes = 0, b_chunk_stride = 0;
  std::vector<char> n_blob, n_leaves;
  int n_chunk = 0, n_n_chunks = 0;
  size_t n_chunk_stride = 0;
  std::vector<uint8_t> pad;
};
HostPack pack_forest_host(const fd_forest_params& p, const fd_tree_arrays& t, int min_depth = 0);
void repack_forest(PackedForest& pf, const fd_forest_params& p, const fd_tree_arrays& t);
float sklearn_threshold_to_lt(double thr);
struct SparsePack {
  std::vector<uint32_t> nodes;
  std::vector<char> leaf_val;
  std::vector<int32_t> leaf_ids;
  int kind = 0, n_trees = 0, depth = 0, num_feature = 0, leaf_bytes = 0;
  int64_t n_nodes = 0, n_leaves = 0;
  float base_margin = 0.f;
};
SparsePack pack_forest_sparse_host(const fd_forest_params& p, const fd_tree_arrays& t);
int forest_depth_probe(const fd_tree_arrays& t);
void load_forest_sparse(PackedForest& pf, const fd_forest_params& p, const fd_tree_arrays& t);
void launch_forest_sparse(Engine& e, const PackedForest& pf, const float* d_X, int64_t n, int32_t ld, double* d_prob,
                          double* d_raw, int32_t* d_leaf, hipStream_t stream);
bool launch_forest_pair(Engine& e, const PackedForest& pa, const PackedForest& pb, const float* d_X, int64_t n,
                        int32_t ld, double* d_prob_a, double* d_prob_b);
void launch_forest(Engine& e, const PackedForest& pf, const float* d_X, int64_t n, int32_t ld,
                   double* d_prob, double* d_raw, int32_t* d_leaf, hipStream_t stream = nullptr);
struct BlendConsts;
bool launch_forest_pair_blend(Engine& e, const PackedForest& p1, const PackedForest& p2, const float* d_X, int64_t n,
                              int32_t ld, const BlendConsts& bc, const double* const* cols, int pos1, int pos2,
                              double* dfp, double* dconf, uint8_t* ddec, uint8_t* drisk,
                              hipEvent_t before_blend = nullptr);
bool forest_pair_prebin(Engine& e, const PackedForest& p1, const PackedForest& p2, const float* d_X, int64_t n,
                        int32_t ld);
void windows_init(Engine& e, const fd_window_params& p);
void windows_step(Engine& e, const fd_txn_batch& t, const fd_window_inputs& in, int64_t n, bool flush,
                  fd_user_window* u_out, int64_t u_cap, int64_t* n_user, fd_merchant_window* m_out, int64_t m_cap,
                  int64_t* n_merch);
void windows_release(Engine& e);
void windows_observe(Engine& e, int64_t max_event_ts);
void merchant_windows_merge(const fd_merchant_window* p, int64_t n, fd_merchant_window* out, int64_t* n_out);
void ingest_set_vocab(Engine& e, int which, const uint8_t* bytes, const int64_t* offsets, int64_t n);
void ingest_set_merchants(Engine& e, const uint8_t* bytes, const int64_t* offsets, int64_t n);
void launch_ingest(Engine& e, const uint8_t* d_bytes, const int64_t* d_offsets, int64_t n, const fd_ingest_out& out);
void sink_init(Engine& e, const fd_sink_params& p);
void sink_update(Engine& e, const fd_txn_batch& t, const fd_window_inputs& in, int64_t n);
void sink_query(Engine& e, int kind, const int64_t* bucket, const int32_t* merchant, int64_t n, fd_aggregate* out);
void sink_evict_before(Engine& e, int64_t hour, int64_t* kept_entries, int64_t* kept_users);
void sink_release(Engine& e);
void state_snapshot(Engine& e, const char* path, int shard, int n_shards, int64_t* bytes_written);
void state_restore(Engine& e, const char* path, int shard, int n_shards, int flags, int64_t* cards_restored);
void state_init(Engine& e, const fd_state_params& p);
void state_clear(Engine& e);
int64_t state_count(Engine& e);
void load_users(Engine& e, const fd_users& u);
void load_merchants(Engine& e, const fd_merchants& m);
void launch_features(Engine& e, const fd_txn_batch& t, int64_t n, float* d_vec, double* d_raw,
                     float* d_seq = nullptr, double* d_vel5 = nullptr, hipStream_t stream = nullptr,
                     bool lean = false, int set = 0, hipEvent_t before_buckets = nullptr, int compact = 0,
                     unsigned long long* d_seq_desc = nullptr);
void launch_features_records(Engine& e, const void* d_records, int64_t n, float* d_vec, float* d_seq,
                             hipStream_t stream = nullptr, bool lean = false, int set = 0,
                             hipEvent_t before_buckets = nullptr, int compact = 0);
void load_users_ext(Engine& e, const fd_users_ext& u);
void load_merchants_ext(Engine& e, const fd_merchants_ext& m);
void load_vocab(Engine& e, const uint8_t* pay_high_risk, const uint8_t* type_refund);
void launch_features_full(Engine& e, const fd_txn_batch& t, const fd_txn_context& c, int64_t n, float* d_vec,
                          double* d_raw, double* d_fmap, fd_rule_scores* d_rules);
void features_check(Engine& e);
hipStream_t make_stream(int level);
unsigned shard_of_host(unsigned long long key, unsigned G);
void launch_route_partition(Engine& e, const fd_txn_batch& t, const fd_window_inputs* extra, int64_t n, int G,
                            void* d_records, int64_t* d_counts, hipStream_t stream = nullptr,
                            DeviceBuffer* scratch = nullptr, bool timed = true);
void launch_route_count(const fd_txn_batch& t, int64_t n, int G, int64_t* totals, hipStream_t st, DeviceBuffer& blk);
struct CountPublish {
  int64_t* cnt;
  int G;
  int gather_rank;
  int64_t* h;
  unsigned long long* h_seq;
  unsigned long long seq;
};
void launch_route_place(const fd_txn_batch& t, int64_t n, int G, void* d_records, hipStream_t st, DeviceBuffer& blk,
                        const CountPublish* pub = nullptr);
void launch_route_unpack(Engine& e, const void* d_records, const void* d_results, int64_t n, const fd_txn_batch& out,
                         uint8_t* pm, uint8_t* fraud, double* score);
void launch_result_pack(Engine& e, const double* fp, const double* conf, const uint8_t* dec, const uint8_t* risk,
                        const RouteRecord* records, int64_t n, void* d_results);
void launch_result_scatter(Engine& e, const void* d_results, int64_t n, double* fp, double* conf, uint8_t* dec,
                           uint8_t* risk);
void route_check(Engine& e);
void comm_unique_id(const char* rccl_path, uint8_t* out);
void comm_init(Engine& e, const char* rccl_path, int rank, int world, const uint8_t* id_fwd, const uint8_t* id_back);
void comm_destroy(Engine& e);
void comm_abort(Engine& e, const std::string& reason);
bool comm_sync_stream(Engine& e, hipStream_t st);
void comm_launch_counts(Engine& e, const fd_txn_batch& t, int64_t n, hipEvent_t ready, int slot, HostLaps& L);
void comm_wait_counts(Engine& e, int slot, int64_t n, HostLaps& L);
void comm_forward_group(Engine& e, int slot, const fd_txn_batch* next, int64_t next_n, hipEvent_t next_ready,
                        int next_slot, HostLaps& L);
void comm_exchange(Engine& e, bool back, hipStream_t st, const void* sendbuf, const int64_t* send, void* recvbuf,
                   const int64_t* recv, size_t elem);
void load_lstm(Engine& e, const fd_lstm_params& p);
void launch_lstm(Engine& e, hipStream_t stream, const float* d_seq, int64_t n, int T, double* d_prob,
                 const unsigned long long* d_desc = nullptr);
std::vector<uint32_t> pack_mlp_host(const fd_mlp_params& p);
void load_mlp(Engine& e, const fd_mlp_params& p);
void launch_mlp(Engine& e, hipStream_t stream, const float* d_X, int64_t n, int32_t ld, double* d_prob);
void graph_init(Engine& e, const fd_graph_params& p);
void graph_clear(Engine& e);
void graph_release(Engine& e);
void graph_info(Engine& e, int64_t* total, int64_t* held);
void graph_step(Engine& e, const fd_txn_batch& t, int64_t n, double* d_out);
void text_release(Engine& e);
int64_t text_nonascii_rows(Engine& e);
void text_features(Engine& e, const uint8_t* d_bytes, const int64_t* d_off, int64_t n, double* d_feat,
                   uint8_t* d_patterns, uint8_t* d_status);
const AbTest& ab_test(Engine& e, int id);
void ab_create(Engine& e, int id, const fd_ab_params& p);
void ab_destroy(Engine& e, int id);
void ab_clear(Engine& e, int id);
void ab_release(Engine& e);
// ... 29 lines not shown
```

realtime-fraud-detection_amd/fdengine/_native.py:

```python
from __future__ import annotations

import ctypes as C
import os
from pathlib import Path

PKG_ROOT = Path(__file__).resolve().parent.parent
REPO_ROOT = PKG_ROOT.parent
LIB_PATH = Path(os.environ.get("FDENGINE_LIB", PKG_ROOT / "lib" / "libfdengine.so"))

FD_OK = 0
FD_ERR_INVALID_ARG = 1
FD_ERR_HIP = 2
FD_ERR_NOT_LOADED = 3
FD_ERR_UNSUPPORTED = 4
FD_ERR_OOM = 5
FD_ERR_IO = 6
FD_RESTORE_SKIP_WINDOWS = 1
FD_RESTORE_SKIP_SINK = 2

FD_FOREST_XGB_BINARY_LOGISTIC = 1
FD_FOREST_SKLEARN_IFOREST = 2
FD_FOREST_SKLEARN_PROBA = 3

FD_MAX_MODELS = 8
FD_BLEND_WEIGHTED_AVERAGE = 0
FD_BLEND_VOTING = 1
FD_BLEND_STACKING = 2

DECISIONS = ("APPROVE", "REVIEW", "DECLINE", "APPROVE_WITH_MONITORING")
RISK_LEVELS = ("VERY_LOW", "LOW", "MEDIUM", "HIGH", "CRITICAL")


class fd_tree_arrays(C.Structure):
    _fields_ = [
        ("n_trees", C.c_int32),
        ("tree_offsets", C.POINTER(C.c_int64)),
        ("left", C.POINTER(C.c_int32)),
        ("right", C.POINTER(C.c_int32)),
        ("feature", C.POINTER(C.c_int32)),
        ("threshold", C.POINTER(C.c_double)),
        ("default_left", C.POINTER(C.c_uint8)),
        ("leaf_value", C.POINTER(C.c_double)),
    ]


class fd_forest_params(C.Structure):
    _fields_ = [
        ("kind", C.c_int32),
        ("num_feature", C.c_int32),
        ("base_score", C.c_double),
        ("if_offset", C.c_double),
        ("if_denominator", C.c_double),
    ]


class fd_blend_params(C.Structure):
    _fields_ = [
        ("n_models", C.c_int32),
        ("strategy", C.c_int32),
        ("weight", C.c_double * FD_MAX_MODELS),
        ("conf_mult", C.c_double * FD_MAX_MODELS),
        ("fraud_threshold", C.c_double),
        ("confidence_threshold", C.c_double),
    ]


class fd_pack_info(C.Structure):
    _fields_ = [
        ("n_trees", C.c_int32),
        ("n_chunks", C.c_int32),
        ("chunk", C.c_int32),
        ("depth", C.c_int32),
        ("tree_bytes", C.c_int64),
        ("chunk_stride", C.c_int64),
        ("blob_bytes", C.c_int64),
        ("n_leaf_ids", C.c_int64),
        ("base_margin", C.c_float),
        ("layout", C.c_int32),
        ("n_thresholds", C.c_int64),
        ("bin_steps", C.c_int32),
    ]


class fd_sparse_info(C.Structure):
    _fields_ = [
        ("kind", C.c_int32),
        ("n_trees", C.c_int32),
        ("depth", C.c_int32),
        ("leaf_bytes", C.c_int32),
        ("n_nodes", C.c_int64),
        ("n_leaves", C.c_int64),
        ("base_margin", C.c_float),
        ("pad", C.c_int32),
    ]


class fd_state_params(C.Structure):
    _fields_ = [("capacity", C.c_int64), ("window_mode", C.c_int32), ("ring_k", C.c_int32), ("seq_len", C.c_int32)]


class fd_txn_context(C.Structure):
    _fields_ = [("geo_lat", C.c_void_p), ("geo_lon", C.c_void_p), ("merchant_lat", C.c_void_p),
                ("merchant_lon", C.c_void_p), ("payment_method", C.c_void_p), ("transaction_type", C.c_void_p),
                ("card_type", C.c_void_p), ("user_agent_flag", C.c_void_p), ("fraud_score", C.c_void_p)]


class fd_users_ext(C.Structure):
    _fields_ = [("n", C.c_int64), ("key", C.c_void_p), ("risk_score", C.c_void_p), ("kyc_status", C.c_void_p),
                ("verified", C.c_void_p), ("pref_start", C.c_void_p), ("pref_end", C.c_void_p),
                ("weekend_activity", C.c_void_p), ("online_preference", C.c_void_p), ("intl_preference", C.c_void_p),
                ("txn_frequency", C.c_void_p), ("has_patterns", C.c_void_p)]


class fd_merchants_ext(C.Structure):
    _fields_ = [("n", C.c_int64), ("avg_amount", C.c_void_p), ("risk_level", C.c_void_p), ("blacklisted", C.c_void_p),
                ("category", C.c_void_p), ("high_risk_category", C.c_void_p), ("open_hour", C.c_void_p),
                ("close_hour", C.c_void_p), ("suspicious_name", C.c_void_p)]


CTX_FIELDS = ("geo_lat", "geo_lon", "merchant_lat", "merchant_lon", "payment_method", "transaction_type",
              "card_type", "user_agent_flag", "fraud_score")
USER_EXT_FIELDS = ("risk_score", "kyc_status", "verified", "pref_start", "pref_end", "weekend_activity",
                   "online_preference", "intl_preference", "txn_frequency", "has_patterns")
MERCHANT_EXT_FIELDS = ("avg_amount", "risk_level", "blacklisted", "category", "high_risk_category", "open_hour",
                       "close_hour", "suspicious_name")
FD_FEATURE_MAP_WIDTH = 64
FD_CODE_UNKNOWN = 254
RULE_DTYPE = [("tp_score", "<f8"), ("fe_score", "<f8"), ("tp_decision", "u1"), ("tp_risk", "u1"),
              ("fe_decision", "u1"), ("fe_risk", "u1"), ("pad", "u1", 4)]


class fd_lstm_params(C.Structure):
    _fields_ = [("input_size", C.c_int32), ("hidden", C.c_int32), ("n_out", C.c_int32), ("w_ih", C.c_void_p),
                ("w_hh", C.c_void_p), ("b_ih", C.c_void_p), ("b_hh", C.c_void_p), ("w_out", C.c_void_p),
                ("b_out", C.c_void_p)]


class fd_mlp_params(C.Structure):
    _fields_ = [("n_layers", C.c_int32), ("dims", C.c_int32 * 9), ("weight", C.c_void_p * 8),
                ("bias", C.c_void_p * 8)]


class fd_graph_params(C.Structure):
    _fields_ = [("max_history", C.c_int32)]


class fd_text_batch(C.Structure):
    _fields_ = [("bytes", C.c_void_p), ("off", C.c_void_p)]


class fd_ab_params(C.Structure):
    _fields_ = [("salt", C.c_uint64), ("threshold", C.c_double)]


class fd_ab_moments(C.Structure):
    _fields_ = [("sum_hi", C.c_double), ("sum_lo", C.c_double), ("m2_hi", C.c_double), ("m2_lo", C.c_double)]


class fd_ab_variant_state(C.Structure):
    _fields_ = [("rows", C.c_int64), ("decisions", C.c_int64 * 4), ("labeled", C.c_int64), ("tp", C.c_int64),
                ("fp", C.c_int64), ("tn", C.c_int64), ("fn", C.c_int64), ("prediction", fd_ab_moments),
                ("time_ms", fd_ab_moments)]


class fd_ab_state(C.Structure):
    _fields_ = [("variant", fd_ab_variant_state * 2)]


class fd_ab_model_set(C.Structure):
    _fields_ = [("params", C.c_void_p), ("slots", C.c_void_p), ("ext_probs", C.c_void_p), ("present", C.c_void_p)]


class fd_users(C.Structure):
    _fields_ = [("n", C.c_int64), ("key", C.c_void_p), ("avg_amount", C.c_void_p),
                ("account_age_days", C.c_void_p), ("device_fp", C.c_void_p)]


class fd_merchants(C.Structure):
    _fields_ = [("n", C.c_int64), ("fraud_rate", C.c_void_p), ("risk_multiplier", C.c_void_p)]


class fd_txn_batch(C.Structure):
    _fields_ = [("card_key", C.c_void_p), ("ts_ms", C.c_void_p), ("amount_cents", C.c_void_p),
                ("merchant", C.c_void_p), ("device_fp", C.c_void_p), ("ip_class", C.c_void_p),
                ("hour", C.c_void_p), ("weekend", C.c_void_p)]


FD_TIMING_ALL, FD_TIMING_XGB, FD_TIMING_IFOREST, FD_TIMING_FEATURES, FD_TIMING_BLEND = -1, 0, 1, 2, 3
FD_TIMING_ROUTE = 4
FD_TIMING_LSTM = 5
FD_TIMING_WINDOWS = 6
FD_TIMING_INGEST = 7
FD_TIMING_ENSEMBLE = 8
FD_TIMING_MLP = 9
FD_TIMING_GRAPH = 10
FD_TIMING_TEXT = 11
FD_TIMING_ABTEST = 12

INGEST_FIELDS = (("card_key", "<u8"), ("ts_ms", "<i8"), ("amount_cents", "<i8"), ("merchant", "<i4"),
                 ("device_fp", "<u8"), ("ip_class", "u1"), ("hour", "u1"), ("weekend", "u1"), ("geo_lat", "<f8"),
                 ("geo_lon", "<f8"), ("merchant_lat", "<f8"), ("merchant_lon", "<f8"), ("payment_method", "u1"),
                 ("transaction_type", "u1"), ("card_type", "u1"), ("user_agent_flag", "u1"),
                 ("fraud_score", "<f8"), ("is_fraud", "u1"), ("txn_hash", "<u8"), ("status", "u1"))
FD_VOCAB_OTHER = 254
FD_VOCAB_PAYMENT_METHOD, FD_VOCAB_TRANSACTION_TYPE, FD_VOCAB_CARD_TYPE = 0, 1, 2
FD_INGEST_MALFORMED, FD_INGEST_TOO_LONG, FD_INGEST_UNKNOWN_VOCAB, FD_INGEST_INEXACT, FD_INGEST_MISSING = 1, 2, 4, 8, 16
FD_INGEST_INVALID = FD_INGEST_MALFORMED | FD_INGEST_TOO_LONG | FD_INGEST_MISSING


class fd_sink_params(C.Structure):
    _fields_ = [("capacity", C.c_int64), ("user_capacity", C.c_int64)]


FD_AGG_HOURLY, FD_AGG_DAILY, FD_AGG_MERCHANT = 1, 2, 3
AGGREGATE_DTYPE = [("total_count", "<i8"), ("fraud_count", "<i8"), ("high_risk_count", "<i8"),
                   ("unique_user_count", "<i8"), ("total_amount", "<f8"), ("fraud_rate", "<f8"),
                   ("avg_amount", "<f8"), ("found", "<i4"), ("pad", "<i4")]
# ... 30 lines not shown
GRAPH_COLUMNS = ("user_centrality", "merchant_centrality", "clustering_coefficient", "path_length_anomaly",
                 "community_anomaly")
FD_TEXT_FIELDS = 4
FD_TEXT_PATTERNS = 5
FD_TEXT_FEATURES = 14
FD_TEXT_NONASCII = 1
TEXT_FIELDS = ("merchant_name", "description", "category", "location")
TEXT_COLUMNS = ("merchant_name_length", "description_length", "total_text_length", "merchant_name_unique_chars",
                "merchant_name_char_diversity", "numbers_in_merchant", "numbers_in_description", "total_numbers",
                "special_chars_merchant", "special_chars_description", "total_special_chars", "merchant_word_count",
                "description_word_count", "total_word_count")
TEXT_PATTERNS = ("crypto_keywords", "gift_card_keywords", "urgent_language", "suspicious_merchant",
                 "known_scam_patterns")
FD_AB_MAX_TESTS = 8
FD_AB_NO_LABEL = 255
FD_SEQ_INPUT = 16
FD_MAX_SHARDS = 64
FD_ROUTE_RECORD_BYTES = 48
FD_RESULT_RECORD_BYTES = 24
FD_WINDOW_REDIS_COMPAT = 0
FD_WINDOW_SLIDING = 1
FD_RAW_FEATURES = 16
FD_VECTOR_WIDTH = 64
TXN_FIELDS = ("card_key", "ts_ms", "amount_cents", "merchant", "device_fp", "ip_class", "hour", "weekend")

_vp = C.c_void_p
_i32 = C.c_int32
_i64 = C.c_int64
_dp = C.POINTER(C.c_double)

SIGNATURES = {
    "fd_last_error": (C.c_char_p, []),
    "fd_build_id": (C.c_char_p, []),
    "fd_abi_version": (C.c_int, []),
    "fd_device_count": (C.c_int, [C.POINTER(C.c_int)]),
    "fd_engine_create": (C.c_int, [C.c_int, C.POINTER(_vp)]),
    "fd_engine_destroy": (C.c_int, [_vp]),
    "fd_engine_set_stream": (C.c_int, [_vp, _vp]),
    "fd_engine_reset_stream": (C.c_int, [_vp]),
    "fd_engine_sync": (C.c_int, [_vp]),
    "fd_load_forest": (C.c_int, [_vp, C.c_int, C.POINTER(fd_forest_params), C.POINTER(fd_tree_arrays)]),
    "fd_unload_forest": (C.c_int, [_vp, C.c_int]),
    "fd_load_xgboost_json": (C.c_int, [_vp, C.c_int, C.c_char_p]),
    "fd_xgboost_json_read": (C.c_int, [C.c_char_p, C.POINTER(fd_forest_params), C.POINTER(_i32), C.POINTER(_i64),
                                       C.POINTER(fd_tree_arrays)]),
    "fd_forest_info": (C.c_int, [_vp, C.c_int, C.POINTER(_i32), C.POINTER(_i32), C.POINTER(_i32)]),
    "fd_forest_predict_device": (C.c_int, [_vp, C.c_int, _vp, _i64, _i32, _vp, _vp, _vp]),
    "fd_forest_predict_host": (C.c_int, [_vp, C.c_int, _vp, _i64, _i32, _vp, _vp, _vp]),
    "fd_blend_device": (C.c_int, [_vp, C.POINTER(fd_blend_params), _i64, C.POINTER(_vp), _vp, _vp, _vp, _vp, _vp]),
    "fd_blend_host": (C.c_int, [_vp, C.POINTER(fd_blend_params), _i64, C.POINTER(_vp), _vp, _vp, _vp, _vp, _vp]),
    "fd_score_matrix_device": (C.c_int, [_vp, C.POINTER(fd_blend_params), _vp, C.POINTER(_vp), _vp, _vp, _i64, _i32,
                                         _vp, _vp, _vp, _vp, _vp]),
    "fd_score_matrix_host": (C.c_int, [_vp, C.POINTER(fd_blend_params), _vp, C.POINTER(_vp), _vp, _vp, _i64, _i32,
                                       _vp, _vp, _vp, _vp, _vp]),
    "fd_state_init": (C.c_int, [_vp, C.POINTER(fd_state_params)]),
    "fd_state_clear": (C.c_int, [_vp]),
    "fd_state_info": (C.c_int, [_vp, C.POINTER(_i64), C.POINTER(_i64)]),
    "fd_state_load_users_host": (C.c_int, [_vp, C.POINTER(fd_users)]),
    "fd_load_merchants_host": (C.c_int, [_vp, C.POINTER(fd_merchants)]),
    "fd_features_device": (C.c_int, [_vp, C.POINTER(fd_txn_batch), _i64, _vp, _vp]),
    "fd_features_host": (C.c_int, [_vp, C.POINTER(fd_txn_batch), _i64, _vp, _vp]),
    "fd_score_batch_device": (C.c_int, [_vp, C.POINTER(fd_blend_params), _vp, C.POINTER(_vp), _vp,
                                        C.POINTER(fd_txn_batch), _i64, _vp, _vp, _vp, _vp, _vp, _vp]),
    "fd_score_batch_pipelined": (C.c_int, [_vp, C.POINTER(fd_blend_params), _vp, C.POINTER(_vp), _vp,
                                           C.POINTER(fd_txn_batch), _i64, _vp, _vp, _vp, _vp, _vp, _vp, _vp]),
    "fd_state_load_users_ext_host": (C.c_int, [_vp, C.POINTER(fd_users_ext)]),
    "fd_load_merchants_ext_host": (C.c_int, [_vp, C.POINTER(fd_merchants_ext)]),
    "fd_load_vocab_host": (C.c_int, [_vp, _vp, _vp]),
    "fd_features_full_device": (C.c_int, [_vp, C.POINTER(fd_txn_batch), C.POINTER(fd_txn_context), _i64, _vp, _vp,
                                          _vp, _vp]),
    "fd_load_lstm": (C.c_int, [_vp, C.POINTER(fd_lstm_params)]),
    "fd_unload_lstm": (C.c_int, [_vp]),
    "fd_lstm_predict_device": (C.c_int, [_vp, _vp, _i64, _i32, _vp]),
    "fd_lstm_predict_host": (C.c_int, [_vp, _vp, _i64, _i32, _vp]),
    "fd_load_mlp": (C.c_int, [_vp, C.POINTER(fd_mlp_params)]),
    "fd_unload_mlp": (C.c_int, [_vp]),
    "fd_mlp_info": (C.c_int, [_vp, C.POINTER(_i32), C.POINTER(_i32), C.POINTER(_i32)]),
    "fd_mlp_predict_device": (C.c_int, [_vp, _vp, _i64, _i32, _vp]),
    "fd_mlp_predict_host": (C.c_int, [_vp, _vp, _i64, _i32, _vp]),
    "fd_pack_mlp_host": (C.c_int, [C.POINTER(fd_mlp_params), _vp, _i64, C.POINTER(_i64)]),
    "fd_graph_init": (C.c_int, [_vp, C.POINTER(fd_graph_params)]),
    "fd_graph_clear": (C.c_int, [_vp]),
    "fd_graph_info": (C.c_int, [_vp, C.POINTER(_i64), C.POINTER(_i64)]),
    "fd_graph_step_device": (C.c_int, [_vp, C.POINTER(fd_txn_batch), _i64, _vp]),
    "fd_graph_step_host": (C.c_int, [_vp, C.POINTER(fd_txn_batch), _i64, _vp]),
    "fd_graph_features_host": (C.c_int, [_vp, _vp, _vp, _i64, _i32, _vp]),
    "fd_text_features_device": (C.c_int, [_vp, C.POINTER(fd_text_batch), _i64, _vp, _vp, _vp]),
    "fd_text_features_host": (C.c_int, [_vp, C.POINTER(fd_text_batch), _i64, _vp, _vp, _vp]),
    "fd_text_features_ref_host": (C.c_int, [_vp, _vp, _i64, _vp, _vp, _vp]),
    "fd_ab_create": (C.c_int, [_vp, _i32, C.POINTER(fd_ab_params)]),
    "fd_ab_destroy": (C.c_int, [_vp, _i32]),
    "fd_ab_clear": (C.c_int, [_vp, _i32]),
    "fd_ab_assign_device": (C.c_int, [_vp, _i32, _vp, _i64, _vp]),
    "fd_ab_assign_host": (C.c_int, [_vp, _i32, _vp, _i64, _vp]),
    "fd_ab_partition_device": (C.c_int, [_vp, _vp, _i64, _vp, _vp]),
    "fd_ab_partition_host": (C.c_int, [_vp, _vp, _i64, _vp, _vp]),
    "fd_ab_score_matrix_device": (C.c_int, [_vp, _i32, C.POINTER(fd_ab_model_set), C.POINTER(fd_ab_model_set), _vp,
                                            _vp, _i64, _i32, _vp, _vp, _vp, _vp, _vp, _vp]),
    "fd_ab_score_matrix_host": (C.c_int, [_vp, _i32, C.POINTER(fd_ab_model_set), C.POINTER(fd_ab_model_set), _vp,
                                          _vp, _i64, _i32, _vp, _vp, _vp, _vp, _vp, _vp]),
    "fd_ab_record_device": (C.c_int, [_vp, _i32, _vp, _vp, _vp, _vp, C.c_double, _vp, _i64]),
    "fd_ab_record_host": (C.c_int, [_vp, _i32, _vp, _vp, _vp, _vp, C.c_double, _vp, _i64]),
    "fd_ab_state_host": (C.c_int, [_vp, _i32, C.POINTER(fd_ab_state)]),
    "fd_ab_state_merge_host": (C.c_int, [C.POINTER(fd_ab_state), C.POINTER(fd_ab_state), C.POINTER(fd_ab_state)]),
    "fd_ab_bucket_host": (C.c_int, [_vp, _i64, C.c_uint64, _vp]),
    "fd_ab_record_ref_host": (C.c_int, [_vp, _vp, _vp, _vp, C.c_double, _vp, _i64, C.POINTER(fd_ab_state)]),
    "fd_features_seq_device": (C.c_int, [_vp, C.POINTER(fd_txn_batch), _i64, _vp, _vp, _vp]),
    "fd_shard_of_host": (C.c_int, [_vp, _i64, _i32, _vp]),
    "fd_route_partition_device": (C.c_int, [_vp, C.POINTER(fd_txn_batch), _i64, _i32, _vp, _vp]),
    "fd_route_partition_ex_device": (C.c_int, [_vp, C.POINTER(fd_txn_batch), C.POINTER(fd_window_inputs), _i64, _i32,
                                               _vp, _vp]),
    "fd_route_unpack_device": (C.c_int, [_vp, _vp, _vp, _i64, C.POINTER(fd_txn_batch), _vp, _vp, _vp]),
    "fd_windows_observe": (C.c_int, [_vp, _i64]),
    "fd_merchant_windows_merge": (C.c_int, [_vp, _i64, _vp, C.POINTER(_i64)]),
    "fd_score_records_device": (C.c_int, [_vp, C.POINTER(fd_blend_params), _vp, _vp, _vp, _i64, _vp]),
    "fd_score_records_pipelined": (C.c_int, [_vp, C.POINTER(fd_blend_params), _vp, _vp, _vp, _i64, _vp, _vp]),
    "fd_comm_unique_id": (C.c_int, [C.c_char_p, _vp]),
    "fd_comm_init": (C.c_int, [_vp, C.c_char_p, _i32, _i32, _vp, _vp]),
    "fd_comm_destroy": (C.c_int, [_vp]),
    "fd_sharded_step": (C.c_int, [_vp, C.POINTER(fd_blend_params), _vp, _vp, C.POINTER(fd_txn_batch), _i64,
                                  C.c_uint64, _vp, C.POINTER(fd_txn_batch), _i64, C.c_uint64, _vp, _vp, _vp, _vp, _vp,
                                  _vp]),
    "fd_route_partition_stream": (C.c_int, [_vp, C.POINTER(fd_txn_batch), C.POINTER(fd_window_inputs), _i64, _i32,
                                            _vp, _vp, _vp]),
    "fd_route_scatter_results_device": (C.c_int, [_vp, _vp, _i64, _vp, _vp, _vp, _vp]),
    "fd_windows_init": (C.c_int, [_vp, C.POINTER(fd_window_params)]),
    "fd_windows_step_device": (C.c_int, [_vp, C.POINTER(fd_txn_batch), C.POINTER(fd_window_inputs), _i64, C.c_int,
                                         _vp, _i64, C.POINTER(_i64), _vp, _i64, C.POINTER(_i64)]),
    "fd_windows_step_host": (C.c_int, [_vp, C.POINTER(fd_txn_batch), C.POINTER(fd_window_inputs), _i64, C.c_int,
                                       _vp, _i64, C.POINTER(_i64), _vp, _i64, C.POINTER(_i64)]),
    "fd_windows_stats": (C.c_int, [_vp, C.POINTER(_i64), C.POINTER(_i64), C.POINTER(_i64)]),
    "fd_state_snapshot": (C.c_int, [_vp, C.c_char_p, _i32, _i32, C.POINTER(_i64)]),
    "fd_state_restore": (C.c_int, [_vp, C.c_char_p, _i32, _i32, _i32, C.POINTER(_i64)]),
    "fd_hash64": (C.c_int, [_vp, _i64, C.POINTER(C.c_uint64)]),
    "fd_sink_init": (C.c_int, [_vp, C.POINTER(fd_sink_params)]),
    "fd_sink_update_device": (C.c_int, [_vp, C.POINTER(fd_txn_batch), C.POINTER(fd_window_inputs), _i64]),
    "fd_sink_update_host": (C.c_int, [_vp, C.POINTER(fd_txn_batch), C.POINTER(fd_window_inputs), _i64]),
    "fd_sink_query_host": (C.c_int, [_vp, _i32, _vp, _vp, _i64, _vp]),
    "fd_sink_evict_before": (C.c_int, [_vp, _i64, C.POINTER(_i64), C.POINTER(_i64)]),
    "fd_ingest_set_vocab": (C.c_int, [_vp, _i32, _vp, _vp, _i64]),
    "fd_ingest_set_merchants": (C.c_int, [_vp, _vp, _vp, _i64]),
    "fd_ingest_json_device": (C.c_int, [_vp, _vp, _vp, _i64, C.POINTER(fd_ingest_out)]),
    "fd_ingest_json_host": (C.c_int, [_vp, _vp, _vp, _i64, C.POINTER(fd_ingest_out)]),
    "fd_ingest_scalar_host": (C.c_int, [_i32, _vp, _i32, _dp, C.POINTER(_i64), C.POINTER(_i32)]),
    "fd_engine_set_timing": (C.c_int, [_vp, C.c_int]),
    "fd_engine_set_option": (C.c_int, [_vp, C.c_char_p, _i64]),
    "fd_engine_get_counter": (C.c_int, [_vp, C.c_char_p, C.POINTER(_i64)]),
    "fd_timing_read": (C.c_int, [_vp, C.c_int, _dp, C.POINTER(_i64)]),
    "fd_timing_reset": (C.c_int, [_vp]),
    "fd_pack_forest_host": (C.c_int, [C.POINTER(fd_forest_params), C.POINTER(fd_tree_arrays), _vp, _i64, _vp, _i64,
                                      C.POINTER(fd_pack_info)]),
    "fd_contract_forest_host": (C.c_int, [C.POINTER(fd_forest_params), C.POINTER(fd_tree_arrays), C.POINTER(_i64),
                                          C.POINTER(fd_tree_arrays), C.POINTER(C.c_int32), C.POINTER(_i64)]),
    "fd_pack_forest_binned_host": (C.c_int, [C.POINTER(fd_forest_params), C.POINTER(fd_tree_arrays), _vp, _i64,
                                             _vp, _i64, _vp, C.POINTER(fd_pack_info)]),
    "fd_pack_forest_sparse_host": (C.c_int, [C.POINTER(fd_forest_params), C.POINTER(fd_tree_arrays), _vp, _i64,
                                             _vp, _i64, _vp, _i64, C.POINTER(fd_sparse_info)]),
}


class NativeError(RuntimeError):
    def __init__(self, code: int, fn: str, msg: str):
        super().__init__(f"{fn} failed ({code}): {msg}")
        self.code = code


def _preload_hip_runtime() -> None:
    if os.environ.get("FDENGINE_HIP_RUNTIME", "") == "system":
        return
    import importlib.util
    try:
        spec = importlib.util.find_spec("torch")
    except (ImportError, ValueError):
        spec = None
    if spec is None or not spec.origin:
        return
    cand = Path(spec.origin).parent / "lib" / "libamdhip64.so"
    if cand.exists():
        C.CDLL(str(cand), mode=C.RTLD_GLOBAL)


def _load() -> C.CDLL:
    _preload_hip_runtime()
    if not LIB_PATH.exists():
        raise ImportError(
            f"libfdengine.so not found at {LIB_PATH}. Build it with "
            "`python -c 'import __graft_entry__ as g; g.build()'` (hipcc --offload-arch=gfx950). "
            "There is no CPU fallback for the scoring path.")
    lib = C.CDLL(str(LIB_PATH))
    for name, (res, args) in SIGNATURES.items():
        fn = getattr(lib, name)
        fn.restype = res
        fn.argtypes = args
    from . import _buildid
    src_pkg = Path(os.environ.get("FDENGINE_SRC_ROOT", PKG_ROOT))
    src_repo = Path(os.environ.get("FDENGINE_SRC_REPO", src_pkg.parent))
    if (src_pkg / "csrc").is_dir():
        _buildid.check(lib.fd_build_id().decode(), src_pkg, src_repo)
    return lib


lib = _load()


def check(code: int, fn: str) -> None:
    if code != FD_OK:
        msg = lib.fd_last_error().decode("utf-8", "replace")
        if code == FD_ERR_NOT_LOADED:
            raise ValueError(msg)
        raise NativeError(code, fn, msg)


def call(fn: str, *args) -> None:
    check(getattr(lib, fn)(*args), fn)
```

realtime-fraud-detection_amd/fdengine/engine.py:

```python
from __future__ import annotations

import ctypes as C
import os
from typing import Dict, Optional, Sequence

import numpy as np

from . import _native as N
from .forest import ForestArrays


def _ptr(a: Optional[np.ndarray]):
    return None if a is None else C.c_void_p(a.ctypes.data)


class FraudEngine:
    def __init__(self, device: int = 0):
        h = C.c_void_p()
        N.call("fd_engine_create", int(device), C.byref(h))
        self._h = h
        self.device = int(device)
        self.forests: Dict[int, dict] = {}

    def close(self) -> None:
# ... 551 lines not shown
        wi = N.fd_window_inputs(*[int(extra_ptrs[f]) if extra_ptrs and extra_ptrs.get(f) else None
                                  for f in ("payment_method", "is_fraud")], None)
        N.call("fd_route_partition_stream", self._h, C.byref(b), C.byref(wi), int(n), int(n_shards),
               C.c_void_p(records_ptr) if records_ptr else None, C.c_void_p(counts_ptr),
               C.c_void_p(int(stream_ptr)) if stream_ptr else None)

    def route_unpack_device(self, records_ptr: int, results_ptr: int, n: int, out_ptrs: dict, pm_ptr: int = 0,
                            fraud_ptr: int = 0, score_ptr: int = 0) -> None:
        opt = lambda p: C.c_void_p(p) if p else None
        b = N.fd_txn_batch(*[int(out_ptrs.get(f) or 0) or None for f in N.TXN_FIELDS])
        N.call("fd_route_unpack_device", self._h, opt(records_ptr), opt(results_ptr), int(n), C.byref(b),
               opt(pm_ptr), opt(fraud_ptr), opt(score_ptr))

    def score_records_device(self, params: N.fd_blend_params, slots: Sequence[int], records_ptr: int, n: int,
                             results_ptr: int, present: Optional[Sequence[int]] = None) -> None:
        M = params.n_models
        sl = np.array(list(slots) + [-1] * (N.FD_MAX_MODELS - len(slots)), np.int32)
        pres = np.array([1] * M if present is None else list(present), np.uint8)
        N.call("fd_score_records_device", self._h, C.byref(params), _ptr(sl), _ptr(pres),
               C.c_void_p(records_ptr) if records_ptr else None, int(n),
               C.c_void_p(results_ptr) if results_ptr else None)

    def score_records_pipelined(self, params: N.fd_blend_params, slots: Sequence[int], records_ptr: int, n: int,
                                results_ptr: int, input_ready: int = 0, present: Optional[Sequence[int]] = None) -> None:
        M = params.n_models
        sl = np.array(list(slots) + [-1] * (N.FD_MAX_MODELS - len(slots)), np.int32)
        pres = np.array([1] * M if present is None else list(present), np.uint8)
        N.call("fd_score_records_pipelined", self._h, C.byref(params), _ptr(sl), _ptr(pres),
               C.c_void_p(records_ptr) if records_ptr else None, int(n),
               C.c_void_p(results_ptr) if results_ptr else None, C.c_void_p(input_ready) if input_ready else None)

    @staticmethod
    def comm_unique_id(rccl_path: str) -> bytes:
        buf = (C.c_uint8 * 128)()
        N.call("fd_comm_unique_id", os.fsencode(rccl_path), C.cast(buf, C.c_void_p))
        return bytes(buf)

    def comm_init(self, rccl_path: str, rank: int, world: int, id_fwd: bytes, id_back: bytes) -> None:
        a = (C.c_uint8 * 128).from_buffer_copy(id_fwd)
        b = (C.c_uint8 * 128).from_buffer_copy(id_back)
        N.call("fd_comm_init", self._h, os.fsencode(rccl_path), int(rank), int(world), C.cast(a, C.c_void_p),
               C.cast(b, C.c_void_p))

    def comm_destroy(self) -> None:
        N.call("fd_comm_destroy", self._h)

    def sharded_scorer(self, params: N.fd_blend_params, slots: Sequence[int],
                       present: Optional[Sequence[int]] = None) -> "ShardedStep":
        return ShardedStep(self, params, slots, present)

    def route_scatter_results_device(self, results_ptr: int, n: int, fp_ptr: int, conf_ptr: int = 0,
                                     dec_ptr: int = 0, risk_ptr: int = 0) -> None:
        opt = lambda p: C.c_void_p(p) if p else None
        N.call("fd_route_scatter_results_device", self._h, opt(results_ptr), int(n), opt(fp_ptr), opt(conf_ptr),
               opt(dec_ptr), opt(risk_ptr))

    @staticmethod
    def blend_params(weights: Sequence[float], conf_mult: Sequence[float], strategy: int = 0,
                     fraud_threshold: float = 0.5, confidence_threshold: float = 0.7) -> N.fd_blend_params:
        p = N.fd_blend_params()
        p.n_models = len(weights)
        p.strategy = int(strategy)
        for i, (w, m) in enumerate(zip(weights, conf_mult)):
            p.weight[i] = float(w)
            p.conf_mult[i] = float(m)
        p.fraud_threshold = float(fraud_threshold)
        p.confidence_threshold = float(confidence_threshold)
        return p

    def blend(self, params: N.fd_blend_params, probs: Sequence[Optional[np.ndarray]]):
        M = params.n_models
        assert len(probs) == M
        n = next((len(p) for p in probs if p is not None), 0)
        cols = [None if p is None else np.ascontiguousarray(p, dtype=np.float64) for p in probs]
        present = np.array([0 if c is None else 1 for c in cols], np.uint8)
        arr = (C.c_void_p * N.FD_MAX_MODELS)()
        for i, c in enumerate(cols):
            arr[i] = None if c is None else c.ctypes.data
        fp = np.empty(n, np.float64)
        conf = np.empty(n, np.float64)
        dec = np.empty(n, np.uint8)
        risk = np.empty(n, np.uint8)
        N.call("fd_blend_host", self._h, C.byref(params), n, arr, _ptr(present), _ptr(fp), _ptr(conf),
               _ptr(dec), _ptr(risk))
        return fp, conf, dec, risk

    def score_matrix(self, params: N.fd_blend_params, slots: Sequence[int], X: np.ndarray,
                     ext_probs: Optional[Sequence[Optional[np.ndarray]]] = None,
                     present: Optional[Sequence[int]] = None):
        X = np.ascontiguousarray(np.asarray(X, dtype=np.float32))
        n, ld = X.shape
        M = params.n_models
        sl = np.array(list(slots) + [-1] * (N.FD_MAX_MODELS - len(slots)), np.int32)
        pres = np.array([1] * M if present is None else list(present), np.uint8)
        ext = (C.c_void_p * N.FD_MAX_MODELS)()
        keep = []
        for m in range(M):
            if sl[m] < 0 and pres[m]:
                col = np.ascontiguousarray(ext_probs[m], dtype=np.float64)
                keep.append(col)
                ext[m] = col.ctypes.data
        mp = np.empty((M, n), np.float64)
        fp = np.empty(n, np.float64)
        conf = np.empty(n, np.float64)
        dec = np.empty(n, np.uint8)
        risk = np.empty(n, np.uint8)
        N.call("fd_score_matrix_host", self._h, C.byref(params), _ptr(sl), ext, _ptr(pres), _ptr(X), n, ld,
               _ptr(mp), _ptr(fp), _ptr(conf), _ptr(dec), _ptr(risk))
        return mp, fp, conf, dec, risk

    def blend_device(self, params: N.fd_blend_params, n: int, prob_ptrs: Sequence[Optional[int]],
                     fp_ptr: int, conf_ptr: int = 0, dec_ptr: int = 0, risk_ptr: int = 0) -> None:
        present = np.array([0 if p is None else 1 for p in prob_ptrs], np.uint8)
        arr = (C.c_void_p * N.FD_MAX_MODELS)()
        for i, p in enumerate(prob_ptrs):
            arr[i] = p if p else None
        N.call("fd_blend_device", self._h, C.byref(params), int(n), arr, _ptr(present), C.c_void_p(fp_ptr),
               C.c_void_p(conf_ptr) if conf_ptr else None, C.c_void_p(dec_ptr) if dec_ptr else None,
               C.c_void_p(risk_ptr) if risk_ptr else None)


def pack_forest_host(fa: ForestArrays):
    p, t, keep = fa.c_structs()
    info = N.fd_pack_info()
    N.call("fd_pack_forest_host", C.byref(p), C.byref(t), None, 0, None, 0, C.byref(info))
    blob = np.empty(info.blob_bytes, np.uint8)
    ids = np.empty(info.n_leaf_ids, np.int32)
    N.call("fd_pack_forest_host", C.byref(p), C.byref(t), C.c_void_p(blob.ctypes.data), info.blob_bytes,
           C.c_void_p(ids.ctypes.data), info.n_leaf_ids, C.byref(info))
    del keep
    return blob.tobytes(), ids, info


def contract_forest_host(fa: ForestArrays):
    p, t, keep = fa.c_structs()
    nn, pruned = C.c_int64(), C.c_int64()
    N.call("fd_contract_forest_host", C.byref(p), C.byref(t), C.byref(nn), None, None, None)
    T, M = fa.n_trees, nn.value
    out = ForestArrays(kind=fa.kind, num_feature=fa.num_feature, offsets=np.zeros(T + 1, np.int64),
                       left=np.zeros(M, np.int32), right=np.zeros(M, np.int32), feature=np.zeros(M, np.int32),
                       threshold=np.zeros(M, np.float64), default_left=np.zeros(M, np.uint8),
                       leaf_value=np.zeros(M, np.float64), base_score=fa.base_score, if_offset=fa.if_offset,
                       if_denominator=fa.if_denominator)
    _, to, ko = out.c_structs()
    depths = np.zeros(T, np.int32)
    N.call("fd_contract_forest_host", C.byref(p), C.byref(t), C.byref(nn), C.byref(to),
           depths.ctypes.data_as(C.POINTER(C.c_int32)), C.byref(pruned))
    del keep
    for name in ("offsets", "left", "right", "feature", "threshold", "default_left", "leaf_value"):
        setattr(out, name, ko[name])
    return out, depths, pruned.value


def pack_forest_binned_host(fa: ForestArrays):
    p, t, keep = fa.c_structs()
    info = N.fd_pack_info()
    N.call("fd_pack_forest_binned_host", C.byref(p), C.byref(t), None, 0, None, 0, None, C.byref(info))
    blob = np.empty(info.blob_bytes, np.uint8)
    thr = np.empty(info.n_thresholds, np.float32)
    off = np.empty(fa.num_feature + 1, np.int32)
    N.call("fd_pack_forest_binned_host", C.byref(p), C.byref(t), C.c_void_p(blob.ctypes.data), info.blob_bytes,
           C.c_void_p(thr.ctypes.data), info.n_thresholds, C.c_void_p(off.ctypes.data), C.byref(info))
    del keep
    return blob.tobytes(), thr, off, info


def pack_forest_sparse_host(fa: ForestArrays):
    p, t, keep = fa.c_structs()
    info = N.fd_sparse_info()
    N.call("fd_pack_forest_sparse_host", C.byref(p), C.byref(t), None, 0, None, 0, None, 0, C.byref(info))
    nodes = np.empty((info.n_nodes, 2), np.uint32)
    vals = np.empty(info.n_leaves, np.float32 if info.leaf_bytes == 4 else np.float64)
    ids = np.empty(info.n_leaves, np.int32)
    N.call("fd_pack_forest_sparse_host", C.byref(p), C.byref(t), C.c_void_p(nodes.ctypes.data), info.n_nodes,
           C.c_void_p(vals.ctypes.data), info.n_leaves, C.c_void_p(ids.ctypes.data), info.n_leaves, C.byref(info))
    del keep
    return nodes, vals, ids, info


def read_xgboost_json_native(path) -> ForestArrays:
    p = N.fd_forest_params()
    nt, nn = C.c_int32(), C.c_int64()
    N.call("fd_xgboost_json_read", os.fsencode(str(path)), C.byref(p), C.byref(nt), C.byref(nn), None)
    T, M = nt.value, nn.value
    fa = ForestArrays(kind=p.kind, num_feature=p.num_feature, offsets=np.zeros(T + 1, np.int64),
                      left=np.zeros(M, np.int32), right=np.zeros(M, np.int32), feature=np.zeros(M, np.int32),
                      threshold=np.zeros(M, np.float64), default_left=np.zeros(M, np.uint8),
                      leaf_value=np.zeros(M, np.float64), base_score=p.base_score)
    _, t, keep = fa.c_structs()
    N.call("fd_xgboost_json_read", os.fsencode(str(path)), C.byref(p), C.byref(nt), C.byref(nn), C.byref(t))
    out = ForestArrays(kind=fa.kind, num_feature=fa.num_feature, offsets=keep["offsets"], left=keep["left"],
                       right=keep["right"], feature=keep["feature"], threshold=keep["threshold"],
                       default_left=keep["default_left"], leaf_value=keep["leaf_value"], base_score=p.base_score)
    return out


def shard_of(keys, n_shards: int) -> np.ndarray:
    k = np.ascontiguousarray(keys, np.uint64)
    out = np.empty(len(k), np.int32)
    N.call("fd_shard_of_host", _ptr(k), len(k), int(n_shards), _ptr(out))
    return out


def device_count() -> int:
    c = C.c_int()
    rc = N.lib.fd_device_count(C.byref(c))
    return c.value if rc == N.FD_OK else 0


def merge_merchant_windows(parts) -> np.ndarray:
    a = np.concatenate([np.asarray(p, N.MERCHANT_WINDOW_DTYPE) for p in parts]) if len(parts) else \
        np.zeros(0, N.MERCHANT_WINDOW_DTYPE)
    a = np.ascontiguousarray(a)
    out = np.zeros(max(len(a), 1), N.MERCHANT_WINDOW_DTYPE)
    m = C.c_int64()
    N.call("fd_merchant_windows_merge", a.ctypes.data if len(a) else None, len(a), out.ctypes.data, C.byref(m))
    return out[:m.value].copy()


class PipelinedScorer:

    def __init__(self, eng: FraudEngine, params: N.fd_blend_params, slots: Sequence[int],
                 present: Optional[Sequence[int]] = None, pipelined: bool = True):
        M = params.n_models
        self.eng = eng
        self.params = params
        self._sl = np.array(list(slots) + [-1] * (N.FD_MAX_MODELS - len(slots)), np.int32)
        self._pres = np.array([1] * M if present is None else list(present), np.uint8)
        self._ext = (C.c_void_p * N.FD_MAX_MODELS)()
        self._batch = N.fd_txn_batch()
        self.pipelined = pipelined
        self._fn = N.lib.fd_score_batch_pipelined if pipelined else N.lib.fd_score_batch_device
        self._args = [C.byref(params), _ptr(self._sl), self._ext, _ptr(self._pres), C.byref(self._batch)]

    def __call__(self, txn_ptrs: dict, n: int, fp_ptr: int, conf_ptr: int = 0, dec_ptr: int = 0, risk_ptr: int = 0,
                 input_ready: int = 0, vec_ptr: int = 0, model_probs_ptr: int = 0) -> None:
        b = self._batch
        for f in N.TXN_FIELDS:
            setattr(b, f, txn_ptrs[f])
        if self.pipelined:
            rc = self._fn(self.eng._h, *self._args, int(n), vec_ptr or None, model_probs_ptr or None, fp_ptr,
                          conf_ptr or None, dec_ptr or None, risk_ptr or None, input_ready or None)
            N.check(rc, "fd_score_batch_pipelined")
        else:
            rc = self._fn(self.eng._h, *self._args, int(n), vec_ptr or None, model_probs_ptr or None, fp_ptr,
                          conf_ptr or None, dec_ptr or None, risk_ptr or None)
            N.check(rc, "fd_score_batch_device")


class ShardedStep:

    def __init__(self, eng: FraudEngine, params: N.fd_blend_params, slots: Sequence[int],
                 present: Optional[Sequence[int]] = None):
        M = params.n_models
        self.eng, self.params = eng, params
        self._sl = np.array(list(slots) + [-1] * (N.FD_MAX_MODELS - len(slots)), np.int32)
        self._pres = np.array([1] * M if present is None else list(present), np.uint8)
        self._cur, self._next = N.fd_txn_batch(), N.fd_txn_batch()
        self.split_sizes = np.zeros(2 * 64, np.int64)
        self._fn = N.lib.fd_sharded_step

    def __call__(self, txn_ptrs: dict, n: int, fp_ptr: int, conf_ptr: int, dec_ptr: int, risk_ptr: int,
                 input_ready: int = 0, next_ptrs: Optional[dict] = None, next_n: int = 0, next_ready: int = 0,
                 batch_id: int = 0, next_id: int = 0) -> None:
        for f in N.TXN_FIELDS:
            setattr(self._cur, f, txn_ptrs[f])
        nxt = None
        if next_ptrs is not None:
            for f in N.TXN_FIELDS:
                setattr(self._next, f, next_ptrs[f])
            nxt = C.byref(self._next)
        rc = self._fn(self.eng._h, C.byref(self.params), self._sl.ctypes.data, self._pres.ctypes.data,
                      C.byref(self._cur), int(n), int(batch_id), input_ready or None, nxt, int(next_n), int(next_id),
                      next_ready or None, fp_ptr or None, conf_ptr or None, dec_ptr or None, risk_ptr or None,
                      self.split_sizes.ctypes.data)
        N.check(rc, "fd_sharded_step")
```

Before: 848.0 million.

## Add dense chunked ensemble layout with per-chunk bundle tables and default to it

Adds a new dense forest layout (contract mode 3/4) that packs contracted trees into variable-length chunks. Each chunk carries its own bundle table of depths and node offsets plus a leaf-index table for owner summation. The kernel gains a DENSE variant that walks bundles per group from these tables and stages chunks with the table appended. It also bins only the compact slots with precomputed threshold ranges. The aim is to cut wasted per-tree 1KB slots and node steps on trees of mixed depth, at the cost of more complex indexing, runtime depth switches and a larger LDS tile.

After: 899.3 million (median of 6 runs). 1.06x the previous value.

```diff
diff --git a/include/fdengine.h b/include/fdengine.h
--- a/include/fdengine.h
+++ b/include/fdengine.h
@@ -106,6 +106,18 @@
 
 int fd_contract_forest_host(const fd_forest_params* params, const fd_tree_arrays* trees, int64_t* n_nodes,
                             fd_tree_arrays* out, int32_t* depths, int64_t* n_pruned);
+
+typedef struct fd_dense_tree {
+  int32_t chunk, bundle, group, depth;
+  int32_t node_offset, leaf_offset;
+} fd_dense_tree;
+typedef struct fd_dense_info {
+  int32_t n_chunks, s_max, trees_per_bundle, buf_bytes;
+  int64_t blob_bytes, n_thresholds, node_steps;
+} fd_dense_info;
+int fd_dense_layout_host(const fd_forest_params* params, const fd_tree_arrays* trees, int32_t wide, int32_t mode,
+                         int32_t owner_bias, fd_dense_info* info, void* blob, int64_t* chunk_offsets,
+                         int32_t* chunk_lengths, fd_dense_tree* tree_info, float* thresholds, int32_t* thr_offsets);
 
 typedef struct {
   int32_t kind;
diff --git a/realtime-fraud-detection_amd/csrc/engine.hip b/realtime-fraud-detection_amd/csrc/engine.hip
--- a/realtime-fraud-detection_amd/csrc/engine.hip
+++ b/realtime-fraud-detection_amd/csrc/engine.hip
@@ -543,6 +543,8 @@
     *value = e.ens.valid ? (int64_t)e.ens.nodes_pruned : 0;
   } else if (k == "ensemble_node_steps_per_txn") {
     *value = (int64_t)e.ens_steps_last;
+  } else if (k == "ensemble_dense_chunks") {
+    *value = (int64_t)e.ens_dense_chunks_last;
   } else if (k == "forest_sparse_launches") {
     *value = (int64_t)e.sparse_total;
   } else if (k == "mlp_launches") {
@@ -609,7 +611,7 @@
     FD_REQUIRE(value >= 0 && value <= 2, FD_ERR_INVALID_ARG, "ensemble_chunks must be 0, 1 or 2");
     e.ens_chunks = (int)value;
   } else if (k == "ensemble_contract") {
-    FD_REQUIRE(value >= 0 && value <= 2, FD_ERR_INVALID_ARG, "ensemble_contract must be 0, 1 or 2");
+    FD_REQUIRE(value >= 0 && value <= 4, FD_ERR_INVALID_ARG, "ensemble_contract must be 0 .. 4");
     if ((int)value != e.ens_contract) {
       e.activate();
       FD_HIP(hipDeviceSynchronize());
@@ -804,6 +806,45 @@
   FD_API_END
 }
 
+int fd_dense_layout_host(const fd_forest_params* params, const fd_tree_arrays* trees, int32_t wide, int32_t mode,
+                         int32_t owner_bias, fd_dense_info* info, void* blob, int64_t* chunk_offsets,
+                         int32_t* chunk_lengths, fd_dense_tree* tree_info, float* thresholds, int32_t* thr_offsets) {
+  FD_API_BEGIN
+  FD_REQUIRE(params && trees && info, FD_ERR_INVALID_ARG, "null params/trees/info");
+  const fd::ContractedForest c = fd::contract_forest_host(*params, *trees);
+  const bool xgb = params->kind == FD_FOREST_XGB_BINARY_LOGISTIC;
+  std::vector<std::vector<float>> tables((size_t)params->num_feature);
+  for (size_t o = 0; o < c.left.size(); ++o)
+    if (c.left[o] >= 0)
+      tables[(size_t)c.feature[o]].push_back(xgb ? (float)c.threshold[o] : fd::sklearn_threshold_to_lt(c.threshold[o]));
+  int64_t n_thr = 0;
+  for (std::vector<float>& t : tables) {
+    std::sort(t.begin(), t.end());
+    t.erase(std::unique(t.begin(), t.end()), t.end());
+    n_thr += (int64_t)t.size();
+  }
+  const fd::DenseLayout L = fd::dense_layout_host(c, xgb, tables, wide != 0, mode, owner_bias);
+  info->n_chunks = (int32_t)L.chunk_len.size();
+  info->s_max = fd::kDenseSMax;
+  info->trees_per_bundle = L.tpg;
+  info->buf_bytes = (int32_t)L.buf;
+  info->blob_bytes = (int64_t)L.blob.size();
+  info->n_thresholds = n_thr;
+  info->node_steps = L.steps;
+  if (blob) std::memcpy(blob, L.blob.data(), L.blob.size());
+  if (chunk_offsets) std::memcpy(chunk_offsets, L.chunk_off.data(), L.chunk_off.size() * 8);
+  if (chunk_lengths) std::memcpy(chunk_lengths, L.chunk_len.data(), L.chunk_len.size() * 4);
+  if (tree_info) std::memcpy(tree_info, L.tree.data(), L.tree.size() * sizeof(fd_dense_tree));
+  if (thr_offsets) thr_offsets[0] = 0;
+  int64_t at = 0;
+  for (size_t f = 0; f < tables.size(); ++f) {
+    if (thresholds) std::memcpy(thresholds + at, tables[f].data(), tables[f].size() * 4);
+    at += (int64_t)tables[f].size();
+    if (thr_offsets) thr_offsets[f + 1] = (int32_t)at;
+  }
+  FD_API_END
+}
+
 int fd_pack_forest_binned_host(const fd_forest_params* params, const fd_tree_arrays* trees, void* blob,
                                int64_t blob_cap, float* thresholds, int64_t thr_cap, int32_t* offsets,
                                fd_pack_info* info) {
diff --git a/realtime-fraud-detection_amd/csrc/ensemble.hip b/realtime-fraud-detection_amd/csrc/ensemble.hip
--- a/realtime-fraud-detection_amd/csrc/ensemble.hip
+++ b/realtime-fraud-detection_amd/csrc/ensemble.hip
@@ -131,6 +131,14 @@
          1024;
 }
 
+constexpr uint32_t kDenseTile = (uint32_t)kDenseSMax * kTile * 8u;
+constexpr uint32_t kDenseTab = 1024, kDenseGroupTab = 64, kDenseTreeTab = 576;
+constexpr int kDenseOwnerBias = 0;
+size_t ens_lds_dense(bool wide) {
+  return (size_t)ens_xs_bytes(kCompactSlots) + 2 * ((size_t)ens_buf(wide) + kDenseTab) + 2 * (size_t)kDenseTile +
+         kTile * 4 + kTile * 8 + 128 + 1024;
+}
+
 struct EnsArgs {
   const float* X;
   int64_t n;
@@ -163,6 +171,7 @@
   int img_off[kMaxPass + 1];
   int thr_off[kMaxFeatures + 1];
   uint16_t cbin[kMaxFeatures];
+  int cthr[2 * kCompactSlots];
   alignas(4) uint16_t lut[8 * 32];
   BlendConsts blend;
 #ifdef FD_FOREST_PROFILE
@@ -174,11 +183,10 @@
 constexpr uint32_t kLinkMask = 0x3F8u;
 
 template <int D, int TPG, bool NAN_AWARE>
-__device__ __forceinline__ void walk_ens(uint32_t buf, int t0, uint32_t lane4, uint32_t (&leaf)[TPG]) {
-  uint32_t tb[TPG], node[TPG], kl[TPG], kr[TPG], xw[TPG];
+__device__ __forceinline__ void walk_ens_at(uint32_t (&tb)[TPG], uint32_t lane4, uint32_t (&leaf)[TPG]) {
+  uint32_t node[TPG], kl[TPG], kr[TPG], xw[TPG];
 #pragma unroll
   for (int j = 0; j < TPG; ++j) {
-    tb[j] = buf + (uint32_t)(t0 + j) * 1024u;
     asm volatile("" : "+v"(tb[j]));
     node[j] = lds_load<uint32_t>(tb[j] + 4u);
   }
@@ -214,6 +222,14 @@
       }
     }
   }
+}
+
+template <int D, int TPG, bool NAN_AWARE>
+__device__ __forceinline__ void walk_ens(uint32_t buf, int t0, uint32_t lane4, uint32_t (&leaf)[TPG]) {
+  uint32_t tb[TPG];
+#pragma unroll
+  for (int j = 0; j < TPG; ++j) tb[j] = buf + (uint32_t)(t0 + j) * 1024u;
+  walk_ens_at<D, TPG, NAN_AWARE>(tb, lane4, leaf);
 }
 
 template <int D, int TPG>
@@ -328,6 +344,97 @@
   return ((unsigned long long)hi << 32) | lo;
 }
 
+template <int D, int TPG, bool NAN_AWARE>
+__device__ __forceinline__ unsigned long long walk_pack_at(uint32_t (&tb)[TPG], uint32_t lane4) {
+  uint32_t leaf[TPG];
+  walk_ens_at<D, TPG, NAN_AWARE>(tb, lane4, leaf);
+  uint32_t lo = 0, hi = 0;
+#pragma unroll
+  for (int j = 0; j < TPG; ++j) {
+    if (j < 4) lo |= leaf[j] << (8 * j);
+    else hi |= leaf[j] << (8 * (j - 4));
+  }
+  return ((unsigned long long)hi << 32) | lo;
+}
+
+template <int TPG>
+__device__ __forceinline__ void walk_dense(uint32_t cur, uint32_t tab, uint32_t tw, int gg, int txn, uint32_t lane4,
+                                           bool tile_nan, uint32_t counts) {
+  static_assert(TPG <= 6, "six block offsets per bundle entry");
+  const int nb = (int)((counts >> (8 * gg)) & 0xFFu);
+  const uint32_t ent = tab + kDenseGroupTab + (uint32_t)gg * 128u;
+  u32x4 e = lds_load<u32x4>(ent);
+  for (int s = 0; s < nb; ++s) {
+    const uint32_t e0 = __builtin_amdgcn_readfirstlane(e.x);
+    const uint32_t off[6] = {e.y & 0xFFFFu, e.y >> 16, e.z & 0xFFFFu, e.z >> 16, e.w & 0xFFFFu, e.w >> 16};
+    e = lds_load<u32x4>(ent + (uint32_t)(s + 1) * 16u);
+    uint32_t tb[TPG];
+#pragma unroll
+    for (int j = 0; j < TPG; ++j) tb[j] = cur + off[j];
+    unsigned long long w;
+#define FD_WALK_DEPTH(K)                                                                                        \
+  case K:                                                                                                       \
+    w = tile_nan ? walk_pack_at<K, TPG, true>(tb, lane4) : walk_pack_at<K, TPG, false>(tb, lane4);              \
+    break;
+    switch (e0 & 0xFFu) {
+      FD_WALK_DEPTH(1)
+      FD_WALK_DEPTH(2)
+      FD_WALK_DEPTH(3)
+      FD_WALK_DEPTH(4)
+      FD_WALK_DEPTH(5)
+      FD_WALK_DEPTH(6)
+      FD_WALK_DEPTH(7)
+      default:
+        w = tile_nan ? walk_pack_at<8, TPG, true>(tb, lane4) : walk_pack_at<8, TPG, false>(tb, lane4);
+        break;
+    }
+#undef FD_WALK_DEPTH
+    lds_store<unsigned long long>(tw + (((e0 >> 8) & 0xFFu) * (uint32_t)kTile + (uint32_t)txn) * 8u,
+                                  w);
+  }
+}
+
+template <typename LeafT>
+__device__ __forceinline__ void owner_sum_dense(uint32_t buf, uint32_t tab, uint32_t tile, uint32_t acc, int txn) {
+  const int n = (int)(__builtin_amdgcn_readfirstlane(lds_load<uint32_t>(tab)) & 0xFFu);
+  const uint32_t tx = tile + (uint32_t)txn * 8u, ent = tab + kDenseTreeTab;
+  u32x4 ea = lds_load<u32x4>(ent), eb = lds_load<u32x4>(ent + 16u);
+  u32x4 na = lds_load<u32x4>(ent + 32u), nb = lds_load<u32x4>(ent + 48u);
+  uint32_t i0 = lds_load<uint8_t>(tx + (ea.x & 0xFFFFu)), i1 = lds_load<uint8_t>(tx + (ea.y & 0xFFFFu)),
+           i2 = lds_load<uint8_t>(tx + (ea.z & 0xFFFFu)), i3 = lds_load<uint8_t>(tx + (ea.w & 0xFFFFu)),
+           i4 = lds_load<uint8_t>(tx + (eb.x & 0xFFFFu)), i5 = lds_load<uint8_t>(tx + (eb.y & 0xFFFFu)),
+           i6 = lds_load<uint8_t>(tx + (eb.z & 0xFFFFu)), i7 = lds_load<uint8_t>(tx + (eb.w & 0xFFFFu));
+  LeafT s = lds_load<LeafT>(acc + (uint32_t)txn * (uint32_t)sizeof(LeafT));
+  constexpr uint32_t LS = (uint32_t)sizeof(LeafT);
+  for (int b = 0; b < n; b += 8) {
+    const LeafT v0 = lds_load<LeafT>(buf + (ea.x >> 16) + i0 * LS), v1 = lds_load<LeafT>(buf + (ea.y >> 16) + i1 * LS),
+                v2 = lds_load<LeafT>(buf + (ea.z >> 16) + i2 * LS), v3 = lds_load<LeafT>(buf + (ea.w >> 16) + i3 * LS),
+                v4 = lds_load<LeafT>(buf + (eb.x >> 16) + i4 * LS), v5 = lds_load<LeafT>(buf + (eb.y >> 16) + i5 * LS),
+                v6 = lds_load<LeafT>(buf + (eb.z >> 16) + i6 * LS), v7 = lds_load<LeafT>(buf + (eb.w >> 16) + i7 * LS);
+    ea = na;
+    eb = nb;
+    i0 = lds_load<uint8_t>(tx + (ea.x & 0xFFFFu));
+    i1 = lds_load<uint8_t>(tx + (ea.y & 0xFFFFu));
+    i2 = lds_load<uint8_t>(tx + (ea.z & 0xFFFFu));
+    i3 = lds_load<uint8_t>(tx + (ea.w & 0xFFFFu));
+    i4 = lds_load<uint8_t>(tx + (eb.x & 0xFFFFu));
+    i5 = lds_load<uint8_t>(tx + (eb.y & 0xFFFFu));
+    i6 = lds_load<uint8_t>(tx + (eb.z & 0xFFFFu));
+    i7 = lds_load<uint8_t>(tx + (eb.w & 0xFFFFu));
+    na = lds_load<u32x4>(ent + (uint32_t)(b + 16) * 4u);
+    nb = lds_load<u32x4>(ent + (uint32_t)(b + 16) * 4u + 16u);
+    s = b + 0 < n ? s + v0 : s;
+    s = b + 1 < n ? s + v1 : s;
+    s = b + 2 < n ? s + v2 : s;
+    s = b + 3 < n ? s + v3 : s;
+    s = b + 4 < n ? s + v4 : s;
+    s = b + 5 < n ? s + v5 : s;
+    s = b + 6 < n ? s + v6 : s;
+    s = b + 7 < n ? s + v7 : s;
+  }
+  lds_store<LeafT>(acc + (uint32_t)txn * (uint32_t)sizeof(LeafT), s);
+}
+
 template <int D, int TPG, int CH, typename LeafT>
 __device__ __forceinline__ void owner_sum(uint32_t buf, uint32_t tile, uint32_t acc, int txn, const int NL = 1 << D) {
   unsigned long long w[4];
@@ -352,6 +459,23 @@
   for (int p = part; p < pieces; p += nparts) {
     const char* g = src + (p << 10) + lane * 16;
     const uint32_t m0 = __builtin_amdgcn_readfirstlane(dst + ((uint32_t)p << 10));
+    asm volatile(
+        "s_mov_b32 m0, %0\n\t"
+        "s_nop 0\n\t"
+        "global_load_lds_dwordx4 %1, off"
+        :
+        : "s"(m0), "v"(g)
+        : "memory", "m0");
+  }
+}
+
+__device__ __forceinline__ void stage_dense(const char* __restrict__ src, uint32_t dst, uint32_t tab, int bytes,
+                                            int nparts, int part) {
+  const int lane = threadIdx.x & 63;
+  const int pieces = bytes >> 10;
+  for (int p = part; p < pieces; p += nparts) {
+    const char* g = src + (p << 10) + lane * 16;
+    const uint32_t m0 = __builtin_amdgcn_readfirstlane(p + 1 < pieces ? dst + ((uint32_t)p << 10) : tab);
     asm volatile(
         "s_mov_b32 m0, %0\n\t"
         "s_nop 0\n\t"
@@ -515,7 +639,7 @@
   }
 }
 
-template <int Q, int L, bool LUT>
+template <int Q, int L, bool LUT, bool CS = false>
 __device__ __forceinline__ void bin_compact_pass(const EnsArgs& a, const float (&v)[16], uint16_t* Xs,
                                                  int txn, int f0, int f1, bool glob, uint32_t tl, int o0,
                                                  int& anynan, uint32_t lut) {
@@ -535,14 +659,16 @@
     } else if (x >= 0.f && x < (float)kLutN && x == truncf(x)) {
       bin = lds_load<uint16_t>(lut + (uint32_t)(ks * kLutN + (int)x) * 2u);
     } else {
-      const int o = a.thr_off[f], cnt = a.thr_off[f + 1] - o;
+      const int o = CS ? a.cthr[2 * (Q + 4 * i)] : a.thr_off[f];
+      const int cnt = (CS ? a.cthr[2 * (Q + 4 * i) + 1] : a.thr_off[f + 1]) - o;
       int pos = 0;
 #pragma unroll
       for (int st = 1 << 15; st > 0; st >>= 1)
         if (pos + st <= cnt && a.thr[o + pos + st - 1] <= x) pos += st;
       bin = (uint16_t)pos;
     }
-    Xs[(f >> 1) * 512 + txn * 2 + (f & 1)] = bin;
+    const int at = CS ? Q + 4 * i : f;
+    Xs[(at >> 1) * 512 + txn * 2 + (at & 1)] = bin;
   }
 #pragma unroll
   for (int g0 = 0; g0 < NS; g0 += L) {
@@ -556,8 +682,8 @@
       const int f = kCompactSlot[Q + 4 * i];
       act[k] = g0 + k < NS && f >= f0 && f < f1 && f < a.nf;
       vv[k] = act[k] ? v[i] : 0.f;
-      o[k] = act[k] ? a.thr_off[f] : o0;
-      cnt[k] = act[k] ? a.thr_off[f + 1] - o[k] : 0;
+      o[k] = act[k] ? (CS ? a.cthr[2 * (Q + 4 * i)] : a.thr_off[f]) : o0;
+      cnt[k] = act[k] ? (CS ? a.cthr[2 * (Q + 4 * i) + 1] : a.thr_off[f + 1]) - o[k] : 0;
       pos[k] = 0;
       steps = max(steps, lift_steps(cnt[k]));
     }
@@ -569,7 +695,8 @@
       if (act[k]) {
         const bool nan = vv[k] != vv[k];
         anynan |= nan ? 1 : 0;
-        Xs[(f >> 1) * 512 + txn * 2 + (f & 1)] = nan ? (uint16_t)0xFFFFu : (uint16_t)pos[k];
+        const int at = CS ? Q + 4 * i : f;
+        Xs[(at >> 1) * 512 + txn * 2 + (at & 1)] = nan ? (uint16_t)0xFFFFu : (uint16_t)pos[k];
       }
     }
   }
@@ -588,9 +715,11 @@
   const int gg = __builtin_amdgcn_readfirstlane(wave >> 2);
   const int txn = ((wave & 3) << 6) + lane;
   const uint32_t lane4 = s0 + (uint32_t)txn * 4u;
-  const uint32_t bufA = s0 + ens_xs_bytes(a.nf), bufB = bufA + kEnsBuf;
-  const uint32_t tile0 = bufB + kEnsBuf, tile1 = tile0 + kEnsTile;
-  const uint32_t accA = tile1 + kEnsTile, accB = accA + kTile * 4;
+  constexpr bool DENSE = VD == 3;
+  constexpr uint32_t kBufStep = kEnsBuf + (DENSE ? kDenseTab : 0u), kTileBytes = DENSE ? kDenseTile : kEnsTile;
+  const uint32_t bufA = s0 + (DENSE ? ens_xs_bytes(kCompactSlots) : ens_xs_bytes(a.nf)), bufB = bufA + kBufStep;
+  const uint32_t tile0 = bufB + kBufStep, tile1 = tile0 + kTileBytes;
+  const uint32_t accA = tile1 + kTileBytes, accB = accA + kTile * 4;
   const uint32_t flags = accB + kTile * 8, owner_cnt = flags + 64;
   const int64_t row = (int64_t)blockIdx.x * kTile + txn;
   const bool valid = row < a.n;
@@ -625,20 +754,20 @@
       const uint4* ra = reinterpret_cast<const uint4*>(a.X) + 2 * row;
       const uint4* rb = reinterpret_cast<const uint4*>(a.X) + 2 * (a.n + row);
       switch (q) {
-        case 0: load_split<0>(ra, rb, v); bin_compact_constants<0>(a, Xs, txn); break;
-        case 1: load_split<1>(ra, rb, v); bin_compact_constants<1>(a, Xs, txn); break;
-        case 2: load_split<2>(ra, rb, v); bin_compact_constants<2>(a, Xs, txn); break;
-        default: load_split<3>(ra, rb, v); bin_compact_constants<3>(a, Xs, txn); break;
+        case 0: load_split<0>(ra, rb, v); if (!DENSE) bin_compact_constants<0>(a, Xs, txn); break;
+        case 1: load_split<1>(ra, rb, v); if (!DENSE) bin_compact_constants<1>(a, Xs, txn); break;
+        case 2: load_split<2>(ra, rb, v); if (!DENSE) bin_compact_constants<2>(a, Xs, txn); break;
+        default: load_split<3>(ra, rb, v); if (!DENSE) bin_compact_constants<3>(a, Xs, txn); break;
       }
     } else if (valid && a.compact) {
       const float* xr = a.X + row * (int64_t)kCompactWidth;
       switch (q) {
-        case 0: load_compact<0>(xr, v); bin_compact_constants<0>(a, Xs, txn); break;
-        case 1: load_compact<1>(xr, v); bin_compact_constants<1>(a, Xs, txn); break;
-        case 2: load_compact<2>(xr, v); bin_compact_constants<2>(a, Xs, txn); break;
-        default: load_compact<3>(xr, v); bin_compact_constants<3>(a, Xs, txn); break;
-      }
-    } else if (valid) {
+        case 0: load_compact<0>(xr, v); if (!DENSE) bin_compact_constants<0>(a, Xs, txn); break;
+        case 1: load_compact<1>(xr, v); if (!DENSE) bin_compact_constants<1>(a, Xs, txn); break;
+        case 2: load_compact<2>(xr, v); if (!DENSE) bin_compact_constants<2>(a, Xs, txn); break;
+        default: load_compact<3>(xr, v); if (!DENSE) bin_compact_constants<3>(a, Xs, txn); break;
+      }
+    } else if (!DENSE && valid) {
       const float* xr = a.X + row * (int64_t)a.ld;
       const int ncopy = a.ld < a.nf ? a.ld : a.nf;
       if (a.vec4 && fq + 16 <= ncopy) {
@@ -658,7 +787,13 @@
     }
     if (a.n_pass > 0 && !(a.pass_global & 1ull))
       stage_pieces(a.img + a.img_off[0], bufA, a.img_off[1] - a.img_off[0], kEnsWG / 64, wave);
-    if (early0) stage_chunk_asm(nA > 0 ? a.nodes[0] : a.nodes[1], bufA, nA > 0 ? a.stride[0] : a.stride[1], kEnsWG / 64);
+    if (early0) {
+      if (DENSE)
+        stage_dense(nA > 0 ? a.nodes[0] : a.nodes[1], bufA, bufA + kEnsBuf, nA > 0 ? a.stride[0] : a.stride[1],
+                    kEnsWG / 64, wave);
+      else
+        stage_chunk_asm(nA > 0 ? a.nodes[0] : a.nodes[1], bufA, nA > 0 ? a.stride[0] : a.stride[1], kEnsWG / 64);
+    }
 #ifdef FD_FOREST_PROFILE
     pr_st[0] = __builtin_amdgcn_s_memtime();
 #endif
@@ -683,19 +818,19 @@
 #endif
       if (LUT && valid && a.compact) {
         switch (q) {
-          case 0: bin_compact_pass<0, kLock, true>(a, v, Xs, txn, f0, f1, glob, tl, o0, anynan, accA); break;
-          case 1: bin_compact_pass<1, kLock, true>(a, v, Xs, txn, f0, f1, glob, tl, o0, anynan, accA); break;
-          case 2: bin_compact_pass<2, kLock, true>(a, v, Xs, txn, f0, f1, glob, tl, o0, anynan, accA); break;
-          default: bin_compact_pass<3, kLock, true>(a, v, Xs, txn, f0, f1, glob, tl, o0, anynan, accA); break;
+          case 0: bin_compact_pass<0, kLock, true, DENSE>(a, v, Xs, txn, f0, f1, glob, tl, o0, anynan, accA); break;
+          case 1: bin_compact_pass<1, kLock, true, DENSE>(a, v, Xs, txn, f0, f1, glob, tl, o0, anynan, accA); break;
+          case 2: bin_compact_pass<2, kLock, true, DENSE>(a, v, Xs, txn, f0, f1, glob, tl, o0, anynan, accA); break;
+          default: bin_compact_pass<3, kLock, true, DENSE>(a, v, Xs, txn, f0, f1, glob, tl, o0, anynan, accA); break;
         }
       } else if (valid && a.compact) {
         switch (q) {
-          case 0: bin_compact_pass<0, kLock, false>(a, v, Xs, txn, f0, f1, glob, tl, o0, anynan, accA); break;
-          case 1: bin_compact_pass<1, kLock, false>(a, v, Xs, txn, f0, f1, glob, tl, o0, anynan, accA); break;
-          case 2: bin_compact_pass<2, kLock, false>(a, v, Xs, txn, f0, f1, glob, tl, o0, anynan, accA); break;
-          default: bin_compact_pass<3, kLock, false>(a, v, Xs, txn, f0, f1, glob, tl, o0, anynan, accA); break;
+          case 0: bin_compact_pass<0, kLock, false, DENSE>(a, v, Xs, txn, f0, f1, glob, tl, o0, anynan, accA); break;
+          case 1: bin_compact_pass<1, kLock, false, DENSE>(a, v, Xs, txn, f0, f1, glob, tl, o0, anynan, accA); break;
+          case 2: bin_compact_pass<2, kLock, false, DENSE>(a, v, Xs, txn, f0, f1, glob, tl, o0, anynan, accA); break;
+          default: bin_compact_pass<3, kLock, false, DENSE>(a, v, Xs, txn, f0, f1, glob, tl, o0, anynan, accA); break;
         }
-      } else if (valid) {
+      } else if (!DENSE && valid) {
 #pragma unroll
         for (int kk = 0; kk < 16; kk += kLock) {
           const int fb = fq + kk;
@@ -761,8 +896,13 @@
 #endif
     }
   }
-  if (G > 0 && !early0)
-    stage_pieces(nA > 0 ? a.nodes[0] : a.nodes[1], bufA, nA > 0 ? a.stride[0] : a.stride[1], kEnsWG / 64, wave);
+  if (G > 0 && !early0) {
+    if (DENSE)
+      stage_dense(nA > 0 ? a.nodes[0] : a.nodes[1], bufA, bufA + kEnsBuf, nA > 0 ? a.stride[0] : a.stride[1],
+                  kEnsWG / 64, wave);
+    else
+      stage_pieces(nA > 0 ? a.nodes[0] : a.nodes[1], bufA, nA > 0 ? a.stride[0] : a.stride[1], kEnsWG / 64, wave);
+  }
   if (gg == 0) {
     lds_store<float>(accA + txn * 4, a.base_margin);
     lds_store<double>(accB + txn * 8, 0.0);
@@ -775,11 +915,22 @@
   for (int g = 0; g < G; ++g) {
     FD_ESTAMP(q0);
     const bool owner = gg == (a.owner_fixed ? 0 : ((g - 1) & 3));
+    const uint32_t cur = (g & 1) ? bufB : bufA, tw = (g & 1) ? tile1 : tile0;
+    uint32_t th1 = 0, th2 = 0, th3 = 0;
+    if (DENSE) {
+      const u32x4 h = lds_load<u32x4>(cur + kEnsBuf);
+      th1 = __builtin_amdgcn_readfirstlane(h.y);
+      th2 = __builtin_amdgcn_readfirstlane(h.z);
+      th3 = __builtin_amdgcn_readfirstlane(h.w);
+    }
     if (owner) {
       if (g > 0) {
         const int c = g - 1;
         const uint32_t bp = (c & 1) ? bufB : bufA, tp = (c & 1) ? tile1 : tile0;
-        if (c < nA) owner_sum<D, TPGA, kCHA, float>(bp, tp, accA, txn, NL);
+        if (DENSE) {
+          if (c < nA) owner_sum_dense<float>(bp, bp + kEnsBuf, tp, accA, txn);
+          else owner_sum_dense<double>(bp, bp + kEnsBuf, tp, accB, txn);
+        } else if (c < nA) owner_sum<D, TPGA, kCHA, float>(bp, tp, accA, txn, NL);
         else owner_sum<D, TPGB, kCHB, double>(bp, tp, accB, txn, NL);
         if (lane == 0)
           __hip_atomic_fetch_add(reinterpret_cast<uint32_t*>(lbase + (owner_cnt - s0)), 1u, __ATOMIC_RELAXED,
@@ -790,18 +941,28 @@
       }
       if (g + 1 < G) {
         const int h = g + 1, fb = h >= nA ? 1 : 0;
-        stage_pieces(a.nodes[fb] + (size_t)(fb ? h - nA : h) * a.stride[fb], (g & 1) ? bufA : bufB, a.stride[fb], 4,
-                  wave & 3);
-      }
-    }
-    const uint32_t cur = (g & 1) ? bufB : bufA, tw = (g & 1) ? tile1 : tile0;
+        const uint32_t nb = (g & 1) ? bufA : bufB;
+        if (DENSE) {
+          if (h == nA) stage_dense(a.nodes[1], nb, nb + kEnsBuf, a.stride[1], 4, wave & 3);
+          else stage_dense(a.nodes[fb] + ((size_t)th1 << 10), nb, nb + kEnsBuf, (int)(th2 << 10), 4, wave & 3);
+        } else {
+          stage_pieces(a.nodes[fb] + (size_t)(fb ? h - nA : h) * a.stride[fb], nb, a.stride[fb], 4, wave & 3);
+        }
+      }
+    }
     FD_ESTAMP(q1);
-    unsigned long long w;
-    if (VD)
-      w = g < nA ? walk_pack_var<VD, TPGA>(cur, gg, lane4, tile_nan) : walk_pack_var<VD, TPGB>(cur, gg, lane4, tile_nan);
-    else
-      w = g < nA ? walk_pack<D, TPGA>(cur, gg, lane4, tile_nan) : walk_pack<D, TPGB>(cur, gg, lane4, tile_nan);
-    lds_store<unsigned long long>(tw + (uint32_t)(gg * kTile + txn) * 8u, w);
+    if (DENSE) {
+      if (g < nA) walk_dense<TPGA>(cur, cur + kEnsBuf, tw, gg, txn, lane4, tile_nan, th3);
+      else walk_dense<TPGB>(cur, cur + kEnsBuf, tw, gg, txn, lane4, tile_nan, th3);
+    } else {
+      unsigned long long w;
+      if (VD)
+        w = g < nA ? walk_pack_var<VD, TPGA>(cur, gg, lane4, tile_nan)
+                   : walk_pack_var<VD, TPGB>(cur, gg, lane4, tile_nan);
+      else
+        w = g < nA ? walk_pack<D, TPGA>(cur, gg, lane4, tile_nan) : walk_pack<D, TPGB>(cur, gg, lane4, tile_nan);
+      lds_store<unsigned long long>(tw + (uint32_t)(gg * kTile + txn) * 8u, w);
+    }
     FD_ESTAMP(q2);
     if (owner) dma_wait();
 #ifdef FD_FOREST_PROFILE
@@ -819,7 +980,10 @@
   if (G > 0 && gg == (a.owner_fixed ? 0 : ((G - 1) & 3))) {
     const int c = G - 1;
     const uint32_t bp = (c & 1) ? bufB : bufA, tp = (c & 1) ? tile1 : tile0;
-    if (c < nA) owner_sum<D, TPGA, kCHA, float>(bp, tp, accA, txn, NL);
+    if (DENSE) {
+      if (c < nA) owner_sum_dense<float>(bp, bp + kEnsBuf, tp, accA, txn);
+      else owner_sum_dense<double>(bp, bp + kEnsBuf, tp, accB, txn);
+    } else if (c < nA) owner_sum<D, TPGA, kCHA, float>(bp, tp, accA, txn, NL);
     else owner_sum<D, TPGB, kCHB, double>(bp, tp, accB, txn, NL);
   }
   __syncthreads();
@@ -917,6 +1081,10 @@
   if (vd == 2) {
     if (wide) return out == 1 ? (const void*)ensemble_kernel<8, 1, true, true, 2> : (const void*)ensemble_kernel<8, 0, true, true, 2>;
     return out == 1 ? (const void*)ensemble_kernel<8, 1, false, true, 2> : (const void*)ensemble_kernel<8, 0, false, true, 2>;
+  }
+  if (vd == 3) {
+    if (wide) return out == 1 ? (const void*)ensemble_kernel<8, 1, true, true, 3> : (const void*)ensemble_kernel<8, 0, true, true, 3>;
+    return out == 1 ? (const void*)ensemble_kernel<8, 1, false, true, 3> : (const void*)ensemble_kernel<8, 0, false, true, 3>;
   }
   if (wide) return out == 1 ? (const void*)ensemble_kernel<8, 1, true, true, 1> : (const void*)ensemble_kernel<8, 0, true, true, 1>;
   return out == 1 ? (const void*)ensemble_kernel<8, 1, false, true, 1> : (const void*)ensemble_kernel<8, 0, false, true, 1>;
@@ -1049,10 +1217,23 @@
   P.contracted = false;
   P.nodes_pruned = 0;
   P.steps_full = P.steps_c = 0;
+  P.dense_len0[0] = P.dense_len0[1] = P.dense_chunks[0] = P.dense_chunks[1] = 0;
   for (int k = 0; k < 2 && contract; ++k) {
     if (!F[k]) continue;
     const bool xgb = F[k]->params.kind == FD_FOREST_XGB_BINARY_LOGISTIC;
     const ContractedForest c = contract_forest_host(F[k]->params, arrays_of(*F[k]));
+    if (contract >= 3) {
+      FD_REQUIRE(ens_lds_dense(wide) <= ens_lds(kMaxFeatures, wide), FD_ERR_UNSUPPORTED,
+                 "dense layout: more LDS than the padded layout");
+      const DenseLayout L = dense_layout_host(c, xgb, merged, wide, contract, kDenseOwnerBias);
+      P.nodes_c[k].ensure(L.blob.size());
+      FD_HIP(hipMemcpy(P.nodes_c[k].ptr, L.blob.data(), L.blob.size(), hipMemcpyHostToDevice));
+      P.dense_len0[k] = L.chunk_len.empty() ? 0 : L.chunk_len[0];
+      P.dense_chunks[k] = (int)L.chunk_len.size();
+      P.steps_c += L.steps;
+      P.nodes_pruned += c.pruned;
+      continue;
+    }
     const int T = hp[k].n_trees, nc = P.n_chunks[k], ch = CH[k], tpg = ch / 4;
     const size_t nb = (size_t)nc * ch;
     std::vector<int> dw(nb, 1);
@@ -1160,6 +1341,177 @@
 
 bool want_wide(const Engine& e) { return e.ens_chunks == 1 || (e.ens_chunks == 0 && !e.comm.ready); }
 
+}
+
+DenseLayout dense_layout_host(const ContractedForest& c, bool xgb, const std::vector<std::vector<float>>& tables,
+                              bool wide, int mode, int owner_bias) {
+  FD_REQUIRE(mode == 3 || mode == 4, FD_ERR_INVALID_ARG, "dense layout: mode 3 or 4");
+  FD_REQUIRE(owner_bias >= 0 && owner_bias <= 64, FD_ERR_INVALID_ARG, "dense layout: owner_bias in [0, 64]");
+  DenseLayout L;
+  const int T = (int)c.off.size() - 1;
+  const int tpg = (xgb ? (wide ? EnsCfg<true>::CHA : EnsCfg<false>::CHA) : (wide ? EnsCfg<true>::CHB : EnsCfg<false>::CHB)) / 4;
+  const size_t lsz = xgb ? 4 : 8;
+  L.tpg = tpg;
+  L.buf = ens_buf(wide);
+  L.tree.assign((size_t)T, fd_dense_tree{});
+  for (int i = 0; i < T; ++i)
+    FD_REQUIRE(c.depth[i] >= 1 && c.depth[i] <= 8, FD_ERR_UNSUPPORTED, "dense layout: a tree deeper than 8 levels");
+  struct Bundle {
+    std::vector<int> trees;
+    int depth = 1;
+  };
+  auto bundle_up = [&](int i0, int n, std::vector<Bundle>& B) {
+    std::vector<int> order(n);
+    for (int k = 0; k < n; ++k) order[k] = i0 + k;
+    if (mode == 4)
+      std::stable_sort(order.begin(), order.end(), [&](int x, int y) { return c.depth[x] > c.depth[y]; });
+    B.clear();
+    size_t bytes = 0;
+    const int nbund = (n + tpg - 1) / tpg, part = n % tpg;
+    int where = nbund - 1;
+    if (mode == 4 && part) {
+      long long best = -1;
+      for (int w = 0; w < nbund; ++w) {
+        long long cost = 0;
+        for (int q = 0, k = 0; q < nbund; ++q) {
+          const int sz = q == w ? part : tpg;
+          cost += (long long)sz * c.depth[order[k]];
+          k += sz;
+        }
+        if (best < 0 || cost <= best) best = cost, where = w;
+      }
+    }
+    for (int q = 0, k = 0; q < nbund; ++q) {
+      const int sz = (part && q == where) ? part : tpg;
+      Bundle b;
+      b.trees.assign(order.begin() + k, order.begin() + k + sz);
+      k += sz;
+      for (int t : b.trees) b.depth = std::max(b.depth, (int)c.depth[t]);
+      bytes += b.trees.size() * ((4 + lsz) << b.depth);
+      B.push_back(std::move(b));
+    }
+    return bytes;
+  };
+  std::vector<Bundle> B, cand;
+  std::vector<int32_t> cur(2 * 256);
+  int i0 = 0;
+  while (i0 < T) {
+    int n = 0;
+    for (int m = tpg;; m += tpg) {
+      const int me = std::min(m, T - i0);
+      const size_t bytes = bundle_up(i0, me, cand);
+      if ((int)cand.size() > kDenseSMax || bytes > L.buf) break;
+      n = me;
+      B = cand;
+      if (i0 + m >= T) break;
+    }
+    FD_REQUIRE(n > 0, FD_ERR_UNSUPPORTED, "dense layout: one bundle exceeds the chunk buffer");
+    const int nb = (int)B.size(), ci = (int)L.chunk_off.size();
+    std::vector<int> by_size;
+    std::vector<int> bundle_of(n), place_of(n);
+    for (int b = 0; b < nb; ++b)
+      for (size_t j = 0; j < B[b].trees.size(); ++j) {
+        bundle_of[B[b].trees[j] - i0] = b;
+        place_of[B[b].trees[j] - i0] = (int)j;
+      }
+    for (int k = 0; k < n; ++k) by_size.push_back(k);
+    std::stable_sort(by_size.begin(), by_size.end(),
+                     [&](int x, int y) { return B[bundle_of[x]].depth > B[bundle_of[y]].depth; });
+    size_t at = 0;
+    for (int k : by_size) {
+      L.tree[i0 + k].node_offset = (int32_t)at;
+      at += (size_t)4 << B[bundle_of[k]].depth;
+    }
+    for (int k = 0; k < n; ++k) {
+      L.tree[i0 + k].leaf_offset = (int32_t)at;
+      at += lsz << B[bundle_of[k]].depth;
+    }
+    FD_REQUIRE(at <= L.buf, FD_ERR_UNSUPPORTED, "dense layout: chunk data exceed the buffer");
+    const size_t data = (at + 1023) / 1024 * 1024, base = L.blob.size();
+    L.blob.resize(base + data + 1024, 0);
+    L.chunk_off.push_back((int64_t)base);
+    L.chunk_len.push_back((int32_t)(data + 1024));
+    char* chunk = L.blob.data() + base;
+    std::vector<int> deal(nb);
+    for (int b = 0; b < nb; ++b) deal[b] = b;
+    std::stable_sort(deal.begin(), deal.end(), [&](int x, int y) { return B[x].depth > B[y].depth; });
+    long long load[4] = {(long long)owner_bias * n, 0, 0, 0};
+    std::vector<int> group_of(nb);
+    std::vector<std::vector<int>> of_group(4);
+    for (int b : deal) {
+      int g = 0;
+      for (int q = 1; q < 4; ++q)
+        if (load[q] < load[g]) g = q;
+      load[g] += 16ll * B[b].depth;
+      group_of[b] = g;
+      of_group[g].push_back(b);
+    }
+    for (int k = 0; k < n; ++k) {
+      const int i = i0 + k, dw = B[bundle_of[k]].depth, nl = 1 << dw;
+      fd_dense_tree& t = L.tree[i];
+      t.chunk = ci;
+      t.bundle = bundle_of[k];
+      t.group = group_of[bundle_of[k]];
+      t.depth = dw;
+      L.steps += dw;
+      uint32_t* dst = reinterpret_cast<uint32_t*>(chunk + t.node_offset);
+      const int64_t a = c.off[i];
+      cur[1] = 0;
+      for (int s = 1; s < nl; ++s) {
+        const int32_t o = cur[s];
+        const uint32_t link = s < (nl >> 1) ? (uint32_t)s : (uint32_t)(s - (nl >> 1));
+        if (c.left[a + o] < 0) {
+          dst[s] = link << 3;
+          cur[2 * s] = cur[2 * s + 1] = o;
+          continue;
+        }
+        const int f = c.feature[a + o];
+        FD_REQUIRE(f >= 0 && f < (int)tables.size() && compact_src(f) >= 0, FD_ERR_UNSUPPORTED,
+                   "dense layout: a split on a constant slot");
+        const uint32_t cs = (uint32_t)compact_src(f);
+        const float thr = xgb ? (float)c.threshold[a + o] : sklearn_threshold_to_lt(c.threshold[a + o]);
+        const std::vector<float>& tb = tables[(size_t)f];
+        const uint32_t jm = (uint32_t)(std::lower_bound(tb.begin(), tb.end(), thr) - tb.begin());
+        FD_REQUIRE(jm <= 0xFFFFu, FD_ERR_UNSUPPORTED, "dense layout: threshold index beyond 16 bits");
+        dst[s] = (jm << 16) | ((cs >> 1) << 10) | (link << 3) | ((cs & 1u) << 1) | (c.dleft[a + o] ? 1u : 0u);
+        cur[2 * s] = c.left[a + o];
+        cur[2 * s + 1] = c.right[a + o];
+      }
+      char* leaves = chunk + t.leaf_offset;
+      for (int s = 0; s < nl; ++s) {
+        const double v = c.leaf[a + cur[nl + s]];
+        if (xgb) {
+          const float vf = (float)v;
+          std::memcpy(leaves + (size_t)s * 4, &vf, 4);
+        } else {
+          std::memcpy(leaves + (size_t)s * 8, &v, 8);
+        }
+      }
+    }
+    uint32_t* tab = reinterpret_cast<uint32_t*>(chunk + data);
+    tab[0] = (uint32_t)n | ((uint32_t)nb << 8);
+    if (ci > 0) {
+      uint32_t* prev = reinterpret_cast<uint32_t*>(L.blob.data() + L.chunk_off[ci - 1] + L.chunk_len[ci - 1] - 1024);
+      prev[1] = (uint32_t)(base >> 10);
+      prev[2] = (uint32_t)((data + 1024) >> 10);
+    }
+    for (int g = 0; g < 4; ++g) {
+      tab[3] |= (uint32_t)of_group[g].size() << (8 * g);
+      for (size_t s = 0; s < of_group[g].size(); ++s) {
+        const int b = of_group[g][s];
+        uint32_t* e = tab + (64 + 128 * g + 16 * s) / 4;
+        e[0] = (uint32_t)B[b].depth | ((uint32_t)b << 8) | ((uint32_t)g << 16);
+        for (int j = 0; j < 6; ++j) {
+          const int t = B[b].trees[(size_t)j < B[b].trees.size() ? j : 0];
+          e[1 + j / 2] |= (uint32_t)L.tree[t].node_offset << (16 * (j & 1));
+        }
+      }
+    }
+    for (int k = 0; k < n; ++k)
+      tab[576 / 4 + k] = (uint32_t)(2048 * bundle_of[k] + place_of[k]) | ((uint32_t)L.tree[i0 + k].leaf_offset << 16);
+    i0 += n;
+  }
+  return L;
 }
 
 #ifdef FD_FOREST_PROFILE
@@ -1221,6 +1573,11 @@
   for (int f = 0; f <= P.nf; ++f) a.thr_off[f] = P.h_thr_off[f];
   a.owner_fixed = owner_fixed ? 1 : 0;
   for (int f = 0; f < kMaxFeatures; ++f) a.cbin[f] = f < (int)P.h_cbin.size() ? P.h_cbin[f] : 0;
+  for (int c = 0; c < kCompactSlots; ++c) {
+    const int f = kCompactSlot[c];
+    a.cthr[2 * c] = f < P.nf ? P.h_thr_off[f] : 0;
+    a.cthr[2 * c + 1] = f < P.nf ? P.h_thr_off[f + 1] : 0;
+  }
   for (size_t k = 0; k < P.h_lut.size() && k < sizeof(a.lut) / sizeof(a.lut[0]); ++k) a.lut[k] = P.h_lut[k];
   a.vec4 = (ld % 4 == 0 && (reinterpret_cast<uintptr_t>(dX) & 15u) == 0) ? 1 : 0;
   const EnsPassSet& ps = P.passes;
@@ -1244,7 +1601,7 @@
 bool run_plan(Engine& e, const EnsemblePlan& P, EnsArgs& a, int out, int timing_kind, int vd = 0) {
   const void* fn = vd && out != 2 ? pick_ensemble_var(out, P.wide, vd) : pick_ensemble(out, P.wide, P.D);
   if (!fn) return false;
-  const size_t lds = ens_lds(P.nf, P.wide);
+  const size_t lds = vd == 3 ? ens_lds_dense(P.wide) : ens_lds(P.nf, P.wide);
   FD_HIP(hipFuncSetAttribute(fn, hipFuncAttributeMaxDynamicSharedMemorySize, (int)lds));
   const int64_t blocks = (a.n + kTile - 1) / kTile;
   Engine::Timed* ev = e.timing ? e.next_event_pair(timing_kind) : nullptr;
@@ -1297,14 +1654,20 @@
   a.res = results;
   const int out = results ? 1 : 0;
   FD_REQUIRE(out == 1 || dfp != nullptr, FD_ERR_INVALID_ARG, "null output");
-  const int vd = (compact && e.ens.contracted) ? (e.ens.contract == 1 ? 2 : 1) : 0;
+  const int vd = (compact && e.ens.contracted) ? (e.ens.contract >= 3 ? 3 : e.ens.contract == 1 ? 2 : 1) : 0;
   if (vd) {
     for (int k = 0; k < 2; ++k) a.nodes[k] = e.ens.nodes_c[k].as<const char>();
     a.ldepth = e.ens.D;
   }
+  if (vd == 3)
+    for (int k = 0; k < 2; ++k) {
+      a.n_chunks[k] = e.ens.dense_chunks[k];
+      a.stride[k] = e.ens.dense_len0[k];
+    }
   if (!run_plan(e, e.ens, a, out, FD_TIMING_ENSEMBLE, vd)) return false;
   if (vd) ++e.ens_contract_total;
   e.ens_steps_last = vd ? e.ens.steps_c : e.ens.steps_full;
+  e.ens_dense_chunks_last = vd == 3 ? e.ens.dense_chunks[0] + e.ens.dense_chunks[1] : 0;
   return true;
 }
 
diff --git a/realtime-fraud-detection_amd/csrc/fd_internal.h b/realtime-fraud-detection_amd/csrc/fd_internal.h
--- a/realtime-fraud-detection_amd/csrc/fd_internal.h
+++ b/realtime-fraud-detection_amd/csrc/fd_internal.h
@@ -200,6 +200,7 @@
   bool contracted = false;
   long long nodes_pruned = 0;
   long long steps_full = 0, steps_c = 0;
+  int dense_len0[2] = {0, 0}, dense_chunks[2] = {0, 0};
 };
 
 struct ContractedForest {
@@ -222,6 +223,19 @@
   }
 };
 ContractedForest contract_forest_host(const fd_forest_params& p, const fd_tree_arrays& t);
+
+constexpr int kDenseSMax = 8;
+struct DenseLayout {
+  std::vector<char> blob;
+  std::vector<int64_t> chunk_off;
+  std::vector<int32_t> chunk_len;
+  std::vector<fd_dense_tree> tree;
+  int tpg = 0;
+  uint32_t buf = 0;
+  long long steps = 0;
+};
+DenseLayout dense_layout_host(const ContractedForest& c, bool xgb, const std::vector<std::vector<float>>& tables,
+                              bool wide, int mode, int owner_bias);
 
 struct __attribute__((aligned(16))) RouteRecord {
   unsigned long long key;
@@ -579,8 +593,9 @@
   int forest_variant = 0;
   bool ens_owner_fixed = true;
   int ens_chunks = 0;
-  int ens_contract = 1;
+  int ens_contract = 4;
   unsigned long long ens_contract_total = 0;
+  int ens_dense_chunks_last = 0;
   long long ens_steps_last = 0;
   int mlp_form = 0;
   int mlp_wgs_per_cu = 0;
diff --git a/realtime-fraud-detection_amd/fdengine/_native.py b/realtime-fraud-detection_amd/fdengine/_native.py
--- a/realtime-fraud-detection_amd/fdengine/_native.py
+++ b/realtime-fraud-detection_amd/fdengine/_native.py
@@ -63,6 +63,17 @@
         ("fraud_threshold", C.c_double),
         ("confidence_threshold", C.c_double),
     ]
+
+
+class fd_dense_tree(C.Structure):
+    _fields_ = [("chunk", C.c_int32), ("bundle", C.c_int32), ("group", C.c_int32), ("depth", C.c_int32),
+                ("node_offset", C.c_int32), ("leaf_offset", C.c_int32)]
+
+
+class fd_dense_info(C.Structure):
+    _fields_ = [("n_chunks", C.c_int32), ("s_max", C.c_int32), ("trees_per_bundle", C.c_int32),
+                ("buf_bytes", C.c_int32), ("blob_bytes", C.c_int64), ("n_thresholds", C.c_int64),
+                ("node_steps", C.c_int64)]
 
 
 class fd_pack_info(C.Structure):
@@ -399,6 +410,8 @@
                                       C.POINTER(fd_pack_info)]),
     "fd_contract_forest_host": (C.c_int, [C.POINTER(fd_forest_params), C.POINTER(fd_tree_arrays), C.POINTER(_i64),
                                           C.POINTER(fd_tree_arrays), C.POINTER(C.c_int32), C.POINTER(_i64)]),
+    "fd_dense_layout_host": (C.c_int, [C.POINTER(fd_forest_params), C.POINTER(fd_tree_arrays), _i32, _i32, _i32,
+                                       C.POINTER(fd_dense_info), _vp, _vp, _vp, _vp, _vp, _vp]),
     "fd_pack_forest_binned_host": (C.c_int, [C.POINTER(fd_forest_params), C.POINTER(fd_tree_arrays), _vp, _i64,
                                              _vp, _i64, _vp, C.POINTER(fd_pack_info)]),
     "fd_pack_forest_sparse_host": (C.c_int, [C.POINTER(fd_forest_params), C.POINTER(fd_tree_arrays), _vp, _i64,
diff --git a/realtime-fraud-detection_amd/fdengine/engine.py b/realtime-fraud-detection_amd/fdengine/engine.py
--- a/realtime-fraud-detection_amd/fdengine/engine.py
+++ b/realtime-fraud-detection_amd/fdengine/engine.py
@@ -727,6 +727,24 @@
     return out, depths, pruned.value
 
 
+def dense_layout_host(fa: ForestArrays, wide: bool = True, mode: int = 4, owner_bias: int = 0):
+    p, t, keep = fa.c_structs()
+    info = N.fd_dense_info()
+    args = (C.byref(p), C.byref(t), int(bool(wide)), int(mode), int(owner_bias), C.byref(info))
+    N.call("fd_dense_layout_host", *args, None, None, None, None, None, None)
+    blob = np.zeros(info.blob_bytes, np.uint8)
+    offs = np.zeros(info.n_chunks, np.int64)
+    lens = np.zeros(info.n_chunks, np.int32)
+    trees = np.zeros(fa.n_trees, np.dtype([(k, np.int32) for k in ("chunk", "bundle", "group", "depth", "node_offset",
+                                                                   "leaf_offset")]))
+    thr = np.zeros(info.n_thresholds, np.float32)
+    thr_off = np.zeros(fa.num_feature + 1, np.int32)
+    N.call("fd_dense_layout_host", *args, *[C.c_void_p(x.ctypes.data) for x in (blob, offs, lens, trees, thr, thr_off)])
+    del keep
+    return dict(blob=blob, chunk_offsets=offs, chunk_lengths=lens, trees=trees, thresholds=thr, thr_offsets=thr_off,
+                info=info)
+
+
 def pack_forest_binned_host(fa: ForestArrays):
     p, t, keep = fa.c_structs()
     info = N.fd_pack_info()
```
